# lvxianwei/DeepMerge

Measured on AMD Instinct MI355X. Metric: superpixel-pairs/sec (train step), higher is better.
Workload: dtype bf16; 1 GPU; ShfitScaleFormer_v3 depth [3, 2, 1], scales [32, 64, 128, 256] x 4ch (256x256x4 patches), 32 pairs/GPU/step, fwd+loss+bwd+allreduce+Adam (BASELINE configs[1]); pairs_per_gpu=32, global_batch=32, parallelism=dp1

## Files before the change

deepmerge_amd/_lib.py:

```python
from __future__ import annotations

import ctypes as C
import os
import re
import threading

HERE = os.path.dirname(os.path.abspath(__file__))
ROOT = os.path.dirname(HERE)
LIB_PATH = os.path.join(HERE, "libdeepmerge_hip.so")
HEADER_PATH = os.path.join(ROOT, "include", "deepmerge_hip.h")

DM_F32, DM_BF16 = 0, 1
DM_NT, DM_NN, DM_TN = 0, 1, 2
DM_BF16_PAIR = 2
DM_F64 = 3
DM_EPI_NONE, DM_EPI_GELU, DM_EPI_DGELU, DM_EPI_GELU_GRAD, DM_EPI_MUL = 0, 1, 2, 3, 4

_STATUS = {-1: "bad shape", -2: "bad dtype", -3: "bad alignment", -4: "workspace", -5: "HIP error", -6: "unsupported"}


class DeepMergeLibraryError(RuntimeError):
    pass


class DmGemmArgs(C.Structure):
    _fields_ = [
        ("layout", C.c_int32), ("ab_dtype", C.c_int32), ("c_dtype", C.c_int32), ("aux_dtype", C.c_int32),
        ("M", C.c_int32), ("N", C.c_int32), ("K", C.c_int32),
        ("epilogue", C.c_int32), ("accumulate", C.c_int32), ("split_k", C.c_int32),
        ("A", C.c_void_p), ("lda", C.c_int64),
        ("B", C.c_void_p), ("ldb", C.c_int64),
        ("C", C.c_void_p), ("ldc", C.c_int64),
        ("bias", C.c_void_p),
        ("residual", C.c_void_p), ("ldr", C.c_int64),
        ("aux", C.c_void_p), ("ldaux", C.c_int64),
        ("rows_per_group", C.c_int32), ("group_stride", C.c_int64),
        ("workspace", C.c_void_p), ("workspace_bytes", C.c_int64),
        ("colsum_a", C.c_void_p), ("colsum_accumulate", C.c_int32),
        ("k_fold", C.c_int32), ("a_fold", C.c_int64 * 3), ("b_fold", C.c_int64 * 3),
        ("c_plane", C.c_int64),
    ]


class DmReduceItem(C.Structure):
    _fields_ = [("partial", C.c_void_p), ("out0", C.c_void_p), ("out1", C.c_void_p),
                ("nrows", C.c_int32), ("width", C.c_int32), ("split", C.c_int32), ("accumulate", C.c_int32)]


class DmPairDraw(C.Structure):
    _fields_ = [("pairs", C.c_void_p), ("pair_flag", C.c_void_p), ("poly_off", C.c_void_p), ("poly_pts", C.c_void_p),
                ("pt_tile", C.c_void_p), ("pt_xy", C.c_void_p), ("pt_inner", C.c_void_p), ("pt_obj", C.c_void_p),
                ("pt_region", C.c_void_p),
                ("tile_id", C.c_void_p), ("xy", C.c_void_p), ("inner", C.c_void_p), ("obj", C.c_void_p),
                ("region", C.c_void_p), ("flag", C.c_void_p),
                ("point_id", C.c_void_p),
                ("seed", C.c_uint64),
                ("n_pairs", C.c_int32), ("n_poly", C.c_int32), ("n_poly_pts", C.c_int32), ("n_pts", C.c_int32),
                ("epoch", C.c_int32), ("batch", C.c_int32)]


class DmProfRow(C.Structure):
    _fields_ = [("name", C.c_char * 64), ("launches", C.c_int64), ("total_ms", C.c_double),
                ("total_flops", C.c_double), ("total_bytes", C.c_double)]


_P, _I, _L, _F, _D = C.c_void_p, C.c_int32, C.c_int64, C.c_float, C.c_double

SIGNATURES = {
    "dm_abi_version": (_I, []),
    "dm_last_error": (C.c_char_p, []),
    "dm_arch": (C.c_char_p, []),
    "dm_gemm": (_I, [C.POINTER(DmGemmArgs), _P]),
    "dm_gemm_workspace_bytes": (_L, [_I, _I, _I, _I]),
    "dm_gemm_grouped": (_I, [C.POINTER(DmGemmArgs), _I, _P, _L, _P]),
    "dm_gemm_grouped_workspace_bytes": (_L, [C.POINTER(DmGemmArgs), _I]),
    "dm_attention_fwd": (_I, [_P, _P, _P, _P, _I, _I, _I, _I, _F, _I, _P]),
    "dm_attention_relpos_inkernel": (_I, [_I, _I, _I, _I, _I, _I, _I, _I]),
    "dm_attention_fwd_relpos": (_I, [_P, _P, _I, _I, _I, _P, _P, _I, _I, _I, _I, _F, _I, _P]),
    "dm_attention_split_ok": (_I, [_I, _I, _I, _I, _I, _I, _I, _I]),
    "dm_attention_split_fwd": (_I, [_P, _P, _P, _P, _I, _I, _I, _P, _P, _I, _I, _I, _I, _F, _P]),
    "dm_attention_split_fwd_pair": (_I, [_P, _P, _P, _P, _I, _I, _I, _P, _P, _P, _I, _I, _I, _I, _F, _P]),
    "dm_attention_split_bwd_chunks": (_I, [_I, _I, _I]),
    "dm_attention_split_bwd": (_I, [_P, _P, _P, _I, _I, _I, _P, _P, _P, _P, _P, _P, _P, _P, _I, _I, _I, _I, _F, _P]),
    "dm_attention_split_bwd_pair": (_I, [_P, _P, _P, _I, _I, _I, _P, _P, _P, _P, _P, _P, _P, _P, _I, _I, _I, _I, _F, _P]),
    "dm_attention_bwd_relpos": (_I, [_P, _P, _I, _I, _I, _P, _P, _P, _P, _P, _P, _P, _P, _I, _I, _I, _I, _F, _I, _P]),
    "dm_attention_bwd": (_I, [_P, _P, _P, _P, _P, _P, _P, _P, _P, _I, _I, _I, _I, _F, _I, _P]),
    "dm_attention_bwd_batch_chunks": (_I, [_I, _I, _I, _I]),
    "dm_relpos_bias_gather": (_I, [_P, _P, _P, _P, _I, _I, _I, _P]),
    "dm_relpos_bias_reduce": (_I, [_P, _P, _P, _P, _I, _I, _I, _I, _I, _P]),
    "dm_layernorm_fwd": (_I, [_P, _P, _P, _P, _I, _P, _P, _I, _I, _F, _P]),
    "dm_layernorm_bwd": (_I, [_P, _I, _P, _P, _P, _P, _P, _P, _P, _P, _P, _I, _P, _I, _I, _P]),
    "dm_layernorm_bwd_partials": (_I, [_P, _I, _P, _P, _P, _P, _P, _P, _P, _P, _I, _I, C.POINTER(C.c_int32), _P]),
    "dm_layernorm_bwd_partials_pair": (_I, [_P, _I, _P, _P, _P, _P, _P, _P, _P, _P, _I, _I, C.POINTER(C.c_int32), _P]),
    "dm_partial_reduce_batch": (_I, [C.POINTER(DmReduceItem), _I, _P]),
    "dm_layernorm_bwd_partial_floats": (_L, [_I]),
    "dm_token_pool_fwd": (_I, [_P, _P, _I, _I, _I, _I, _P]),
    "dm_token_pool_bwd": (_I, [_P, _P, _I, _I, _I, _I, _P]),
    "dm_group_mean_fwd": (_I, [_P, _P, _I, _I, _I, _P]),
    "dm_group_mean_bwd": (_I, [_P, _P, _I, _I, _I, _P]),
    "dm_colsum": (_I, [_P, _I, _L, _P, _I, _I, _I, _P, _P]),
    "dm_colsum_partial_floats": (_L, [_I]),
    "dm_cast": (_I, [_P, _P, _I, _L, _P]),
    "dm_split_bf16": (_I, [_P, _L, _L, _L, _P, _I, _I, _P]),
    "dm_split_colsum_partial_floats": (_L, [_L, _L]),
    "dm_split_bf16_colsum": (_I, [_P, _L, _L, _L, _P, _I, _I, _P, _P, _P]),
    "dm_split_bf16_planes": (_I, [_P, _L, _L, _L, _P, _P, _P, _P]),
    "dm_patchify": (_I, [_P, _P, _I, _I, _I, _I, _I, _P]),
    "dm_contrastive_loss": (_I, [_P, _P, _P, _F, _F, _P, _P, _P, _I, _I, _P]),
    "dm_cross_entropy": (_I, [_P, _P, _P, _F, _P, _P, _I, _I, _P]),
    "dm_batchnorm_workspace_bytes": (_L, [_I, _I]),
    "dm_batchnorm_fwd": (_I, [_P, _P, _P, _P, _P, _P, _I, _P, _P, _P, _I, _I, _F, _F, _I, _I, _P, _P]),
    "dm_batchnorm_bwd": (_I, [_P, _P, _P, _P, _P, _I, _P, _P, _P, _P, _P, _I, _I, _I, _I, _I, _P, _P]),
    "dm_adam_step": (_I, [_P, _P, _P, _P, _P, _L, _I, _D, _D, _D, _D, _D, _P]),
    "dm_adam_hyper": (_I, [_I, _D, _D, _D, _P]),
    "dm_adam_step_dev": (_I, [_P, _P, _P, _P, _P, _L, _P, _D, _D, _D, _D, _P]),
    "dm_adam_step_dev_pair": (_I, [_P, _P, _P, _P, _P, _P, _L, _P, _D, _D, _D, _D, _P]),
    "dm_segment_mean": (_I, [_P, _P, _P, _P, _I, _I, _P]),
    "dm_edge_similarity": (_I, [_P, _P, _P, _P, _I, _I, _F, _P]),
    "dm_pairwise_distance": (_I, [_P, _P, _P, _I, _I, _I, _I, _P]),
    "dm_patch_pyramid": (_I, [_P, _I, _I, _I, _P, _P, _I, _I, _I, _I, _P, _P]),
    "dm_patch_pyramid_cols": (_I, [_P, _I, _I, _I, _P, _P, _I, _I, _I, _I, _I, _P, _I, _P]),
    "dm_pair_batch_gather": (_I, [_P, _I, _I, _I, _I, _P, _P, _P, _P, _I, _I, _I, _I, _I, _I, _P, _I, _P, _P, _P, _P]),
    "dm_pair_epoch_draw": (_I, [C.POINTER(DmPairDraw), _P]),
    "dm_contrastive_terms": (_I, [_P, _P, _P, _F, _P, _P, _I, _I, _P]),
    "dm_pair_eval_workspace_bytes": (_L, [_L, _I]),
    "dm_pair_eval_summary": (_I, [_P, _P, _P, _L, _P, _I, _P, _P, _P, _P, _P]),
    "dm_label_stats": (_I, [_P, _P, _I, _I, _I, _I, _P, _P, _P, _P, _P, _P]),
    "dm_label_features": (_I, [_P, _P, _P, _P, _P, _I, _I, _P, _P]),
    "dm_rag_edges": (_I, [_P, _I, _I, _I, _P, _P, _I, _P, _P, _I, _P, _P, _P]),
    "dm_merge_round": (_I, [_P, _P, _I, _I, _P, _P, _I, _P]),
    "dm_gru_cell_fwd": (_I, [_P, _L, _P, _P, _P, _P, _I, _I, _P]),
    "dm_gru_cell_bwd": (_I, [_P, _P, _P, _P, _P, _P, _I, _I, _P]),
    "dm_prof_enable": (_I, [_I]),
    "dm_prof_collect": (_I, [C.POINTER(DmProfRow), _I]),
}

_lock = threading.Lock()
_lib = None


def declared_symbols(header_path: str = HEADER_PATH):
    text = open(header_path).read()
    text = re.sub(r"/\*.*?\*/", "", text, flags=re.S)
    return sorted(set(re.findall(r"\b(dm_[a-z0-9_]+)\s*\(", text)))


def lib() -> C.CDLL:
    global _lib
    if _lib is not None:
        return _lib
    with _lock:
        if _lib is not None:
            return _lib
        if not os.path.exists(LIB_PATH):
            raise DeepMergeLibraryError(
                f"{LIB_PATH} not found: build the HIP kernels first "
                f"(`python -c 'import __graft_entry__ as g; g.build()'` or `make -C deepmerge_amd/csrc`). "
                f"deepmerge_amd has no CPU fallback.")
        try:
            handle = C.CDLL(LIB_PATH)
        except OSError as e:
            raise DeepMergeLibraryError(f"cannot load {LIB_PATH}: {e}") from e
        for name, (res, args) in SIGNATURES.items():
            try:
                fn = getattr(handle, name)
            except AttributeError as e:
                raise DeepMergeLibraryError(f"{LIB_PATH} does not export {name}") from e
            fn.restype = res
            fn.argtypes = args
        if handle.dm_abi_version() != 6:
            raise DeepMergeLibraryError(f"ABI version mismatch: library {handle.dm_abi_version()} != 6")
        _lib = handle
        return _lib


def check(rc: int, what: str):
    if rc == 0:
        return
    msg = lib().dm_last_error().decode("utf-8", "replace")
    text = f"{what} failed ({_STATUS.get(rc, rc)}): {msg}"
    if rc in (-1, -2, -3, -6):
        raise ValueError(text)
    raise RuntimeError(text)
```

deepmerge_amd/csrc/dm_attention.hip:

```cpp
#include "dm_common.h"
#include "dm_mfma.h"
#include "dm_attention_pipe.h"
#include "dm_attention_x3.h"
#include "dm_prof.h"

namespace {

constexpr int HD = 64;
constexpr int QB = 64;

template <typename T> struct AL {
  static constexpr int RB = HD * (int)sizeof(T);
  static constexpr int CPRW = RB / 16;
  static constexpr int KBD = RB / 64;
  static constexpr int EPC = 16 / (int)sizeof(T);
  static constexpr int TPB = (sizeof(T) == 2) ? 2 : 1;
};

template <typename T> __device__ __forceinline__ int swz(int row);
template <> __device__ __forceinline__ int swz<bf16_t>(int row) {
  const int t0 = (row >> 1) & 1, t1 = (row >> 2) & 1, t2 = (row >> 3) & 1;
  return ((t1 ^ t2) << 2) | (t0 << 1) | t1;
}
template <> __device__ __forceinline__ int swz<float>(int row) { return row & 15; }
// ... 314 lines not shown
#pragma unroll
        for (int r = 0; r < 4; ++r)
          if (key + r < N) srow[key + r] = hacc[kt][r];
      }
    }
  }
}

template <typename T, int NKT, bool FAST>
__global__ __launch_bounds__(256, 2) void attn_bwd_dkv_kernel(const AttnParams p) {
  using L = AL<T>;
  constexpr int NK = NKT * 16;
  constexpr int IMG = NK * L::RB;
  __shared__ __attribute__((aligned(16))) char smem[2 * IMG];
  char *qimg = smem, *doimg = smem + IMG;
  const int t = threadIdx.x, lane = t & 63, wave = t >> 6, g = lane >> 4, li = lane & 15;
  const int kblk = blockIdx.x, h = blockIdx.y, b = blockIdx.z;
  const int N = p.N, H = p.H;

  const long long tok_stride = 3LL * H * HD;
  const T *base = reinterpret_cast<const T *>(p.qkv) + (long long)b * N * tok_stride + (long long)h * HD;
  const long long o_stride = (long long)H * HD;
  const T *dOg = reinterpret_cast<const T *>(p.dout) + (long long)b * N * o_stride + (long long)h * HD;
  const int key = kblk * QB + wave * 16 + li;
  const bool kok = key < N;
  const T *krow = base + (long long)key * tok_stride + (long long)H * HD;
  const T *vrow = krow + (long long)H * HD;
  const float *lse = p.lse + ((long long)b * H + h) * N;
  const float *delta = p.delta + ((long long)b * H + h) * N;

  tile_to_lds<T>(qimg, base, tok_stride, N, NK, t);
  tile_to_lds<T>(doimg, dOg, o_stride, N, NK, t);
  u32x4 fk[L::KBD], fvv[L::KBD];
#pragma unroll
  for (int kb = 0; kb < L::KBD; ++kb) {
    fk[kb] = gl_frag<T>(krow, kok, kb, lane);
    fvv[kb] = gl_frag<T>(vrow, kok, kb, lane);
  }
  __syncthreads();

  constexpr int NB = NKT / L::TPB;
  u32x4 fpt[NB], fds[NB];
  const float *bsrc = FAST ? p.bias_t : p.bias;
  const float *brows = bsrc ? bsrc + (long long)h * N * N : nullptr;
  f32x4 bnext[L::TPB], lnext[L::TPB], dnext[L::TPB];
  auto fetch = [&](int m) {
#pragma unroll
    for (int u = 0; u < L::TPB; ++u) {
      const int qt = m * L::TPB + u;
      bnext[u] = bias_tile<FAST, !FAST>(brows, N, key, lane, qt);
      lnext[u] = load4_guard(lse, qt * 16 + 4 * g, N, FAST);
      dnext[u] = load4_guard(delta, qt * 16 + 4 * g, N, FAST);
    }
  };
  fetch(0);
#pragma unroll
  for (int m = 0; m < NB; ++m) {
    f32x4 bcur[L::TPB], lcur[L::TPB], dcur[L::TPB];
#pragma unroll
    for (int u = 0; u < L::TPB; ++u) { bcur[u] = bnext[u]; lcur[u] = lnext[u]; dcur[u] = dnext[u]; }
    if (m + 1 < NB) fetch(m + 1);
    f32x4 tp[L::TPB], td[L::TPB];
#pragma unroll
    for (int u = 0; u < L::TPB; ++u) {
      const int qt = m * L::TPB + u;
      const int q0 = qt * 16 + 4 * g;
      const f32x4 sc = score_tile<T>(fk, qimg, bcur[u], N, key, p.scale, lane, qt);
      f32x4 a = {0.f, 0.f, 0.f, 0.f};
#pragma unroll
      for (int kb = 0; kb < L::KBD; ++kb) mma<T>(a, fvv[kb], frag_row<T>(doimg, qt * 16 + li, kb, lane));
#pragma unroll
      for (int r = 0; r < 4; ++r) {
        const float pv = (q0 + r < N) ? fast_exp<T>(sc[r] - lcur[u][r]) : 0.f;
        tp[u][r] = pv;
        td[u][r] = pv * (a[r] - dcur[u][r]);
      }
    }
    fpt[m] = pack_tiles<T>(tp);
    fds[m] = pack_tiles<T>(td);
    asm volatile("" : "+v"(fpt[m]), "+v"(fds[m]));
    __builtin_amdgcn_sched_barrier(0);
  }
  f32x4 o[4];
  T *dk = reinterpret_cast<T *>(p.dqkv) + ((long long)b * N + key) * tok_stride + (long long)H * HD + (long long)h * HD;
  T *dvp = dk + (long long)H * HD;
#pragma unroll
  for (int dt = 0; dt < 4; ++dt) o[dt] = (f32x4){0.f, 0.f, 0.f, 0.f};
  contract_frags<T, NB>(o, fpt, doimg, lane);
  if (kok) {
#pragma unroll
    for (int dt = 0; dt < 4; ++dt) dm_store4(dvp + dt * 16 + 4 * g, o[dt]);
  }
#pragma unroll
  for (int dt = 0; dt < 4; ++dt) o[dt] = (f32x4){0.f, 0.f, 0.f, 0.f};
  contract_frags<T, NB>(o, fds, qimg, lane);
  if (kok) {
#pragma unroll
    for (int dt = 0; dt < 4; ++dt) dm_store4(dk + dt * 16 + 4 * g, o[dt] * p.scale);
  }
}

template <typename T, int NKT, bool FAST> void launch3(int which, const AttnParams &p, dim3 grid, hipStream_t s) {
  if (which == 0) hipLaunchKernelGGL((attn_fwd_kernel<T, NKT, FAST>), grid, dim3(256), 0, s, p);
  else if (which == 1) hipLaunchKernelGGL((attn_bwd_dq_kernel<T, NKT, FAST>), grid, dim3(256), 0, s, p);
  else hipLaunchKernelGGL((attn_bwd_dkv_kernel<T, NKT, FAST>), grid, dim3(256), 0, s, p);
}
template <typename T, bool FAST> void dispatch_nkt(int which, const AttnParams &p, hipStream_t s) {
  const dim3 grid((p.N + QB - 1) / QB, p.H, which == 1 ? (p.B + p.bchunk - 1) / p.bchunk : p.B);
  const int nkt = (p.N + 15) / 16;
  if (nkt <= 2) launch3<T, 2, FAST>(which, p, grid, s);
  else if (nkt <= 4) launch3<T, 4, FAST>(which, p, grid, s);
  else if (nkt <= 8) launch3<T, 8, FAST>(which, p, grid, s);
  else if (nkt <= 12) launch3<T, 12, FAST>(which, p, grid, s);
  else if (nkt <= 14) launch3<T, 14, FAST>(which, p, grid, s);
  else launch3<T, 16, FAST>(which, p, grid, s);
}
template <typename T> int dispatch(int which, const AttnParams &p, hipStream_t s) {
  const bool fast = (p.N % 4 == 0) && (which != 2 || p.bias == nullptr || p.bias_t != nullptr);
  if (fast) dispatch_nkt<T, true>(which, p, s);
  else dispatch_nkt<T, false>(which, p, s);
  return 0;
}

int check_common(const char *who, int B, int N, int H, int D, int dtype) {
  DM_REQUIRE(B > 0 && H > 0 && N > 0 && N <= 256, DM_ERR_BAD_SHAPE, "%s: need 0 < N <= 4096 tokens and head dim <= 256 (got N=%d, D=%d, B=%d, H=%d)", who, N, D, B, H);
  DM_REQUIRE(D == HD, DM_ERR_BAD_SHAPE, "%s: head dim must be in 1..256 (got %d)", who, D);
  DM_REQUIRE(dtype == DM_F32 || dtype == DM_BF16, DM_ERR_BAD_DTYPE, "%s: bad dtype %d", who, dtype);
  DM_REQUIRE(H <= 65535 && B <= 65535, DM_ERR_BAD_SHAPE, "%s: grid too large", who);
  return DM_OK;
}

}

static int batch_chunk(int B, int N, int H) {
  const int per_sample = ((N + QB - 1) / QB) * H;
  for (int c = 8; c > 1; c >>= 1)
    if ((long long)per_sample * ((B + c - 1) / c) >= 300) return c;
  return 1;
}

const AttnSwitches &attn_switches() {
  static const AttnSwitches sw = [] {
    AttnSwitches v;
    if (const char *e = getenv("DM_ATTN_PIPE")) v.pipe = atoi(e);
    if (const char *e = getenv("DM_ATTN_Q32")) v.q32 = atoi(e);
    if (const char *e = getenv("DM_ATTN_Q32_BWD")) v.q32_bwd = atoi(e);
    if (const char *e = getenv("DM_ATTN_Q32_TABKV")) v.q32_tabkv = atoi(e) != 0;
    if (const char *e = getenv("DM_ATTN_Q32_W8")) v.q32_w8 = atoi(e) != 0;
    if (const char *e = getenv("DM_ATTN_Q32_TABW")) v.q32_tabw = atoi(e);
    if (const char *e = getenv("DM_ATTN_PF")) v.pf = atoi(e) != 0;
    if (const char *e = getenv("DM_ATTN_XCD")) v.xcd = atoi(e) != 0;
    if (const char *e = getenv("DM_ATTN_X3")) v.x3 = atoi(e) != 0;
    if (const char *e = getenv("DM_ATTN_X3_W8")) v.x3_w8 = atoi(e) != 0;
    return v;
  }();
  return sw;
}

namespace {

bool tokens32(const AttnCall &c) { return c.N > 128 && c.N <= 256; }
bool cube_fits(const AttnCall &c) { return c.N == 64 * c.cube_s && (c.cube_s == 3 || c.cube_s == 4); }
bool persistent_gate(const AttnCall &c, int mode) {
  return mode != 0 && (long long)c.N * 3 * c.H * 64 * 2 < (1LL << 31) && (mode == 2 || c.B * c.H >= 96);
}

AttnPass pass32(const AttnCall &c, AttnFamily f, AttnBias bias, int waves, int rows) {
  AttnPass g{f, (c.N + 31) / 32, c.N % 32 != 0, bias, waves, 0, 0, 0};
  attn_chunks(c.B, c.N, c.H, rows, g.nblk, g.chunks, g.bchunk);
  return g;
}
bool ragged16(const AttnCall &c) { return !(c.N == 128 || c.N == 192 || c.N == 256); }
AttnPass pass_pipe16(const AttnCall &c, AttnBias bias) {
  const int nkt = (c.N + 15) / 16;
  AttnPass g{ATTN_PIPE16, ragged16(c) ? (nkt + 1) / 2 * 2 : nkt, ragged16(c), bias, 8, 0, 0, 0};
  attn_chunks(c.B, c.N, c.H, 128, g.nblk, g.chunks, g.bchunk);
  return g;
}
AttnPass pass_reg16(const AttnCall &c, int bchunk) {
  return AttnPass{ATTN_REG16, (c.N + 15) / 16, c.N % 16 != 0, c.dense ? ATTN_BIAS_DENSE : ATTN_BIAS_NONE, 4, (c.N + QB - 1) / QB, (c.B + bchunk - 1) / bchunk, bchunk};
}
int waves32(const AttnCall &c, const AttnSwitches &sw) { return (c.N + 31) / 32 <= 7 && sw.q32_w8 ? 8 : 4; }

bool split_shape(const AttnCall &c, const AttnSwitches &sw) {
  return sw.x3 && c.D == HD && tokens32(c) && c.B > 0 && c.H > 0 && persistent_gate(c, 2) && (!c.table || cube_fits(c));
}

}

AttnFwdPlan attn_plan_fwd(const AttnCall &c, const AttnSwitches &sw) {
  AttnFwdPlan pl{};
  pl.pf = sw.pf;
  pl.xcd = sw.xcd;
  if (c.split) {
    if (!split_shape(c, sw)) pl.refused = ATTN_SHAPE_NOT_TAKEN;
    else pl.pass = pass32(c, ATTN_X3, c.table ? ATTN_BIAS_TABLE : ATTN_BIAS_NONE, sw.x3_w8 ? 8 : 4, 128);
    return pl;
  }
  pl.pass = pass_reg16(c, 1);
  if (c.D != HD || c.N > 256) {
    pl.pass.family = ATTN_GENERIC;
  } else if (c.dtype == DM_BF16) {
    if (tokens32(c) && persistent_gate(c, sw.q32) && !(c.table && (c.dense || !cube_fits(c)))) {
      if (c.table) pl.pass = pass32(c, ATTN_Q32, ATTN_BIAS_TABLE, sw.q32_tabw == 4 ? 4 : 8, sw.q32_tabw == 4 ? 128 : 256);
      else if (c.dense) pl.pass = pass32(c, ATTN_Q32, ATTN_BIAS_DENSE, 4, 128);
      else pl.pass = pass32(c, ATTN_Q32, ATTN_BIAS_NONE, waves32(c, sw), 32 * waves32(c, sw));
    } else if (c.N >= 128 && persistent_gate(c, sw.pipe)) {
      pl.pass = pass_pipe16(c, c.dense ? ATTN_BIAS_DENSE : ATTN_BIAS_NONE);
    }
  }
  if (c.table && !c.dense && !(pl.pass.family == ATTN_Q32 && pl.pass.bias == ATTN_BIAS_TABLE)) pl.refused = ATTN_SHAPE_NOT_TAKEN;
  return pl;
}

AttnBwdPlan attn_plan_bwd(const AttnCall &c, const AttnSwitches &sw) {
  AttnBwdPlan pl{};
  pl.xcd = sw.xcd;
  if (c.split) {
    if (c.B > 0 && c.H > 0) {
      const AttnBias bias = c.table ? ATTN_BIAS_TABLE : ATTN_BIAS_NONE;
      pl.dq = pass32(c, ATTN_X3, bias, sw.x3_w8 ? 8 : 4, 128);
      pl.dkv = pass32(c, ATTN_X3, bias, 4, 128);
      pl.slab_chunks = pl.dkv.chunks;
    }
    if (!split_shape(c, sw)) pl.refused = ATTN_SHAPE_NOT_TAKEN;
    return pl;
  }
  pl.dq = pass_reg16(c, batch_chunk(c.B, c.N, c.H));
  pl.dkv = pass_reg16(c, 1);
  pl.slab_chunks = pl.dq.chunks;
  if (c.D != HD || c.N > 256) {
    pl.dq.family = pl.dkv.family = ATTN_GENERIC;
    return pl;
  }
  const bool table_only = c.table && !c.dense;
  if (c.dtype != DM_BF16) {
    if (table_only) pl.refused = ATTN_TABLE_NEEDS_BF16;
    return pl;
  }
  if (c.N >= 128 && persistent_gate(c, sw.pipe) && !(ragged16(c) && (c.dense || c.slab))) {
    pl.dq = pass_pipe16(c, c.dense ? ATTN_BIAS_DENSE : ATTN_BIAS_NONE);
    pl.dkv = pass_pipe16(c, c.dense || c.slab ? ATTN_BIAS_DENSE : ATTN_BIAS_NONE);
    if (tokens32(c) && persistent_gate(c, sw.q32_bwd) && !(c.table && !cube_fits(c))) {
      if (c.table) pl.dq = pass32(c, ATTN_Q32, ATTN_BIAS_TABLE, 8, 256);
      else if (c.dense) pl.dq = pass32(c, ATTN_Q32, ATTN_BIAS_DENSE, 4, 128);
      else pl.dq = pass32(c, ATTN_Q32, ATTN_BIAS_NONE, waves32(c, sw), 32 * waves32(c, sw));
      const int w = (c.N + 31) / 32 <= 7 ? 8 : 4;
      if (sw.q32_bwd != 3 && c.table && sw.q32_tabkv) pl.dkv = pass32(c, ATTN_Q32_TABKV, ATTN_BIAS_TABLE, 4, 128);
      else if (sw.q32_bwd != 3 && !c.dense && !c.slab) pl.dkv = pass32(c, ATTN_Q32, ATTN_BIAS_NONE, w, 32 * w);
    }
    pl.slab_chunks = pl.dkv.chunks;
  }
  if (table_only && pl.dkv.family != ATTN_Q32_TABKV) pl.refused = ATTN_TABLE_NOT_TAKEN;
  return pl;
}

extern "C" int32_t dm_attention_bwd_batch_chunks(int32_t B, int32_t N, int32_t H, int32_t dtype) {
  return attn_plan_bwd(AttnCall{B, N, H, HD, dtype == DM_BF16 ? DM_BF16 : DM_F32, true, false, 0, true, false}, attn_switches()).slab_chunks;
}

bool dm_attn_generic_shape(int N, int D);
int dm_attn_generic_fwd(const void *qkv, const float *bias, void *out, float *lse, int B, int N, int H, int D, float scale, int dtype, hipStream_t s);
int dm_attn_generic_bwd(const void *qkv, const float *bias, const void *out, const void *dout, const float *lse, void *dqkv, float *delta,
                        int B, int N, int H, int D, float scale, int dtype, hipStream_t s);

extern "C" int dm_attention_fwd(const void *qkv, const float *bias, void *out, float *lse, int32_t B, int32_t N, int32_t H,
                                int32_t D, float scale, int32_t dtype, void *stream) {
  if (dm_attn_generic_shape(N, D)) {
    DM_REQUIRE(B > 0 && H > 0 && H <= 65535 && B <= 65535 && (dtype == DM_F32 || dtype == DM_BF16) && qkv && out && lse, DM_ERR_BAD_SHAPE,
               "dm_attention_fwd: bad arguments (B=%d H=%d dtype=%d)", B, H, dtype);
    const int rc = dm_attn_generic_fwd(qkv, bias, out, lse, B, N, H, D, scale, dtype, reinterpret_cast<hipStream_t>(stream));
    DM_REQUIRE(rc == DM_OK, rc, "dm_attention_fwd: generic kernel could not be configured");
    DM_LAUNCH_CHECK("dm_attention_fwd(generic)");
    return DM_OK;
  }
  if (int rc = check_common("dm_attention_fwd", B, N, H, D, dtype)) return rc;
  DM_REQUIRE(qkv && out && lse, DM_ERR_BAD_SHAPE, "dm_attention_fwd: null pointer");
  DM_REQUIRE(dm_aligned16(qkv) && dm_aligned16(out) && dm_aligned16(bias), DM_ERR_BAD_ALIGN, "dm_attention_fwd: qkv/out/bias must be 16-byte aligned");
  const AttnFwdPlan pl = attn_plan_fwd(AttnCall{B, N, H, D, dtype, bias != nullptr, false, 0, false, false}, attn_switches());
  hipStream_t s = reinterpret_cast<hipStream_t>(stream);
  {
    const double esz = (dtype == DM_BF16) ? 2.0 : 4.0;
    DmProfScope prof(dtype == DM_BF16 ? "attn_fwd_bf16" : "attn_fwd_f32", s, 4.0 * B * H * (double)N * N * HD,
                     esz * 4.0 * B * H * (double)N * HD);
    const AttnPipeParams pp{qkv, bias, out, lse, B, N, H, scale};
    if (pl.pass.family == ATTN_Q32) {
      DM_REQUIRE(dm_attn_fwd_q32(pl, pp, s), DM_ERR_HIP, "dm_attention_fwd: kernel could not be configured");
    } else if (pl.pass.family == ATTN_PIPE16) {
      dm_attn_fwd_pipe(pl, pp, s);
    } else {
      AttnParams p{};
      p.qkv = qkv; p.bias = bias; p.out = out; p.lse = lse; p.B = B; p.N = N; p.H = H; p.scale = scale; p.bchunk = 1;
      if (dtype == DM_BF16) dispatch<bf16_t>(0, p, s); else dispatch<float>(0, p, s);
    }
  }
  DM_LAUNCH_CHECK("dm_attention_fwd");
  return DM_OK;
}

static AttnCall table_call(int32_t B, int32_t N, int32_t H, int32_t D, int32_t cube_s, int32_t cube_h, int32_t cube_w, int32_t dtype, bool split) {
  return AttnCall{B, N, H, D, dtype, false, true, cube_h == 8 && cube_w == 8 ? cube_s : 0, false, split};
}

extern "C" int32_t dm_attention_relpos_inkernel(int32_t B, int32_t N, int32_t H, int32_t D, int32_t cube_s, int32_t cube_h, int32_t cube_w,
                                                int32_t dtype) {
  if (B <= 0 || H <= 0) return 0;
  const AttnCall c = table_call(B, N, H, D, cube_s, cube_h, cube_w, dtype, false);
  return !attn_plan_fwd(c, attn_switches()).refused && !attn_plan_bwd(c, attn_switches()).refused ? 1 : 0;
}

extern "C" int dm_attention_fwd_relpos(const void *qkv, const float *table, int32_t cube_s, int32_t cube_h, int32_t cube_w, void *out,
                                       float *lse, int32_t B, int32_t N, int32_t H, int32_t D, float scale, int32_t dtype, void *stream) {
  DM_REQUIRE(dm_attention_relpos_inkernel(B, N, H, D, cube_s, cube_h, cube_w, dtype), DM_ERR_UNSUPPORTED,
             "dm_attention_fwd_relpos: shape not taken (B=%d N=%d H=%d D=%d cube=%dx%dx%d dtype=%d); gather the bias and call dm_attention_fwd",
             B, N, H, D, cube_s, cube_h, cube_w, dtype);
  DM_REQUIRE(qkv && table && out && lse, DM_ERR_BAD_SHAPE, "dm_attention_fwd_relpos: null pointer");
  DM_REQUIRE(dm_aligned16(qkv) && dm_aligned16(out), DM_ERR_BAD_ALIGN, "dm_attention_fwd_relpos: qkv/out must be 16-byte aligned");
  const AttnFwdPlan pl = attn_plan_fwd(table_call(B, N, H, D, cube_s, cube_h, cube_w, dtype, false), attn_switches());
  hipStream_t s = reinterpret_cast<hipStream_t>(stream);
  {
    DmProfScope prof("attn_fwd_bf16", s, 4.0 * B * H * (double)N * N * HD, 2.0 * 4.0 * B * H * (double)N * HD);
    AttnPipeParams pp{qkv, nullptr, out, lse, B, N, H, scale};
    pp.table = table;
    pp.cube_s = cube_s;
    DM_REQUIRE(dm_attn_fwd_q32(pl, pp, s), DM_ERR_UNSUPPORTED, "dm_attention_fwd_relpos: kernel could not be configured");
  }
  DM_LAUNCH_CHECK("dm_attention_fwd_relpos");
  return DM_OK;
}

static int attention_bwd(const void *qkv, const float *bias, const float *bias_t, const float *table, int32_t cube_s, const void *out,
                         const void *dout, const float *lse, void *dqkv, float *delta, float *dbias_slab, int32_t B, int32_t N, int32_t H,
                         int32_t D, float scale, int32_t dtype, void *stream) {
  if (dm_attn_generic_shape(N, D)) {
    DM_REQUIRE(B > 0 && H > 0 && H <= 65535 && B <= 65535 && (dtype == DM_F32 || dtype == DM_BF16) && qkv && out && dout && lse && dqkv && delta,
               DM_ERR_BAD_SHAPE, "dm_attention_bwd: bad arguments (B=%d H=%d dtype=%d)", B, H, dtype);
    DM_REQUIRE(dbias_slab == nullptr, DM_ERR_UNSUPPORTED, "dm_attention_bwd: the bias-table gradient needs head dim 64 and N <= 256 (got D=%d N=%d)", D, N);
    const int rc = dm_attn_generic_bwd(qkv, bias, out, dout, lse, dqkv, delta, B, N, H, D, scale, dtype, reinterpret_cast<hipStream_t>(stream));
    DM_REQUIRE(rc == DM_OK, rc, "dm_attention_bwd: generic kernel could not be configured");
    DM_LAUNCH_CHECK("dm_attention_bwd(generic)");
    return DM_OK;
  }
  if (int rc = check_common("dm_attention_bwd", B, N, H, D, dtype)) return rc;
  DM_REQUIRE(qkv && out && dout && lse && dqkv && delta, DM_ERR_BAD_SHAPE, "dm_attention_bwd: null pointer");
  DM_REQUIRE(dm_aligned16(qkv) && dm_aligned16(out) && dm_aligned16(dout) && dm_aligned16(dqkv) && dm_aligned16(bias) &&
             dm_aligned16(bias_t) && dm_aligned16(lse) && dm_aligned16(delta) && dm_aligned16(dbias_slab), DM_ERR_BAD_ALIGN,
             "dm_attention_bwd: tensors must be 16-byte aligned");
  const AttnBwdPlan pl = attn_plan_bwd(AttnCall{B, N, H, D, dtype, bias != nullptr, table != nullptr, cube_s, dbias_slab != nullptr, false}, attn_switches());
  DM_REQUIRE(pl.refused != ATTN_TABLE_NEEDS_BF16, DM_ERR_UNSUPPORTED, "dm_attention_bwd_relpos: the table-reading kernels are bf16 only");
  DM_REQUIRE(!pl.refused, DM_ERR_UNSUPPORTED,
             "dm_attention_bwd_relpos: the table-reading backward kernels do not take this call (B=%d N=%d H=%d, switches "
             "DM_ATTN_PIPE / DM_ATTN_Q32_BWD / DM_ATTN_Q32_TABKV) and no dense bias rows were given", B, N, H);
  hipStream_t s = reinterpret_cast<hipStream_t>(stream);
  {
    const double esz = (dtype == DM_BF16) ? 2.0 : 4.0;
    DmProfScope prof(dtype == DM_BF16 ? "attn_bwd_bf16" : "attn_bwd_f32", s, 10.0 * B * H * (double)N * N * HD,
                     esz * 8.0 * B * H * (double)N * HD);
    if (pl.dkv.family == ATTN_REG16) {
      AttnParams p{};
      p.qkv = qkv; p.bias = bias; p.bias_t = bias ? bias_t : nullptr; p.out = out; p.dout = dout; p.lse = const_cast<float *>(lse);
      p.delta = delta; p.dqkv = dqkv; p.slab = dbias_slab;
      p.B = B; p.N = N; p.H = H; p.scale = scale; p.bchunk = pl.dq.bchunk;
      if (dtype == DM_BF16) { dispatch<bf16_t>(1, p, s); dispatch<bf16_t>(2, p, s); }
      else { dispatch<float>(1, p, s); dispatch<float>(2, p, s); }
    } else {
      AttnPipeBwdParams pp{qkv, bias, out, dout, lse, delta, dqkv, dbias_slab, B, N, H, scale};
      pp.table = table;
      pp.cube_s = cube_s;
      DM_REQUIRE(pl.dq.family != ATTN_Q32 || dm_attn_bwd_dq_q32(pl, pp, s), DM_ERR_HIP, "dm_attention_bwd: the dQ kernel could not be configured");
      if (pl.dkv.family == ATTN_PIPE16) dm_attn_bwd_pipe(pl, pp, s);
      else DM_REQUIRE(dm_attn_bwd_dkv_q32(pl, pp, s), DM_ERR_HIP, "dm_attention_bwd: the dK / dV kernel could not be configured");
    }
  }
  DM_LAUNCH_CHECK("dm_attention_bwd");
  return DM_OK;
}

extern "C" int dm_attention_bwd(const void *qkv, const float *bias, const float *bias_t, const void *out, const void *dout,
                                const float *lse, void *dqkv, float *delta, float *dbias_slab, int32_t B, int32_t N, int32_t H, int32_t D, float scale, int32_t dtype,
                                void *stream) {
  return attention_bwd(qkv, bias, bias_t, nullptr, 0, out, dout, lse, dqkv, delta, dbias_slab, B, N, H, D, scale, dtype, stream);
}

extern "C" int dm_attention_bwd_relpos(const void *qkv, const float *table, int32_t cube_s, int32_t cube_h, int32_t cube_w, const float *bias,
                                       const float *bias_t, const void *out, const void *dout, const float *lse, void *dqkv, float *delta,
                                       float *dbias_slab, int32_t B, int32_t N, int32_t H, int32_t D, float scale, int32_t dtype, void *stream) {
  DM_REQUIRE(table, DM_ERR_BAD_SHAPE, "dm_attention_bwd_relpos: null table");
  DM_REQUIRE(bias || dm_attention_relpos_inkernel(B, N, H, D, cube_s, cube_h, cube_w, dtype), DM_ERR_UNSUPPORTED,
             "dm_attention_bwd_relpos: shape not taken (B=%d N=%d H=%d D=%d cube=%dx%dx%d dtype=%d); call dm_attention_bwd", B, N, H, D, cube_s,
             cube_h, cube_w, dtype);
  return attention_bwd(qkv, bias, bias_t, table, cube_s, out, dout, lse, dqkv, delta, dbias_slab, B, N, H, D, scale, dtype, stream);
}

static AttnCall split_call(int32_t B, int32_t N, int32_t H, int32_t D, bool has_table, int32_t cube_s, int32_t cube_h, int32_t cube_w, bool slab) {
  AttnCall c = table_call(B, N, H, D, cube_s, cube_h, cube_w, DM_F32, true);
  c.table = has_table;
  c.slab = slab;
  return c;
}

extern "C" int32_t dm_attention_split_ok(int32_t B, int32_t N, int32_t H, int32_t D, int32_t has_table, int32_t cube_s, int32_t cube_h,
                                         int32_t cube_w) {
  return attn_plan_fwd(split_call(B, N, H, D, has_table != 0, cube_s, cube_h, cube_w, false), attn_switches()).refused ? 0 : 1;
}

static int split_fwd_impl(const float *qkv, void *qkv_hi, void *qkv_lo, const float *table, int32_t cube_s, int32_t cube_h, int32_t cube_w, float *out,
                          void *out_pair, float *lse, int32_t B, int32_t N, int32_t H, int32_t D, float scale, void *stream);
extern "C" int dm_attention_split_fwd(const float *qkv, void *qkv_hi, void *qkv_lo, const float *table, int32_t cube_s, int32_t cube_h,
                                      int32_t cube_w, float *out, float *lse, int32_t B, int32_t N, int32_t H, int32_t D, float scale,
                                      void *stream) {
  return split_fwd_impl(qkv, qkv_hi, qkv_lo, table, cube_s, cube_h, cube_w, out, nullptr, lse, B, N, H, D, scale, stream);
}
extern "C" int dm_attention_split_fwd_pair(const float *qkv, void *qkv_hi, void *qkv_lo, const float *table, int32_t cube_s, int32_t cube_h,
                                           int32_t cube_w, float *out, void *out_pair, float *lse, int32_t B, int32_t N, int32_t H, int32_t D,
                                           float scale, void *stream) {
  DM_REQUIRE(out_pair && dm_aligned16(out_pair), DM_ERR_BAD_SHAPE, "dm_attention_split_fwd_pair: out_pair must be a 16-byte aligned pointer");
  return split_fwd_impl(qkv, qkv_hi, qkv_lo, table, cube_s, cube_h, cube_w, out, out_pair, lse, B, N, H, D, scale, stream);
}
static int split_fwd_impl(const float *qkv, void *qkv_hi, void *qkv_lo, const float *table, int32_t cube_s, int32_t cube_h, int32_t cube_w, float *out,
                          void *out_pair, float *lse, int32_t B, int32_t N, int32_t H, int32_t D, float scale, void *stream) {
  const AttnFwdPlan pl = attn_plan_fwd(split_call(B, N, H, D, table != nullptr, cube_s, cube_h, cube_w, false), attn_switches());
  DM_REQUIRE(!pl.refused, DM_ERR_UNSUPPORTED,
             "dm_attention_split_fwd: shape not taken (B=%d N=%d H=%d D=%d cube=%dx%dx%d); use dm_attention_fwd", B, N, H, D, cube_s, cube_h, cube_w);
  DM_REQUIRE(qkv_hi && qkv_lo && out && lse, DM_ERR_BAD_SHAPE, "dm_attention_split_fwd: null pointer");
  DM_REQUIRE(dm_aligned16(qkv) && dm_aligned16(qkv_hi) && dm_aligned16(qkv_lo) && dm_aligned16(out), DM_ERR_BAD_ALIGN,
             "dm_attention_split_fwd: tensors must be 16-byte aligned");
  hipStream_t s = reinterpret_cast<hipStream_t>(stream);
  {
    DmProfScope prof("attn_fwd_x3", s, 3.0 * 4.0 * B * H * (double)N * N * HD, 4.0 * 4.0 * B * H * (double)N * HD);
    if (qkv) dm_attn_x3_split(qkv, qkv_hi, qkv_lo, (long long)B * N * 3 * H * HD, s);
    AttnX3Params p{reinterpret_cast<const bf16_t *>(qkv_hi), reinterpret_cast<const bf16_t *>(qkv_lo), table, cube_s, out, lse, B, N, H, scale,
                   reinterpret_cast<bf16_t *>(out_pair)};
    DM_REQUIRE(dm_attn_fwd_x3(pl, p, s), DM_ERR_UNSUPPORTED, "dm_attention_split_fwd: kernel could not be configured");
  }
  DM_LAUNCH_CHECK("dm_attention_split_fwd");
  return DM_OK;
}

extern "C" int32_t dm_attention_split_bwd_chunks(int32_t B, int32_t N, int32_t H) {
  return attn_plan_bwd(split_call(B, N, H, HD, false, 0, 0, 0, false), attn_switches()).slab_chunks;
}

static int split_bwd_impl(const void *qkv_hi, const void *qkv_lo, const float *table, int32_t cube_s, int32_t cube_h, int32_t cube_w,
                          const float *out, const float *dout, void *dout_hi, void *dout_lo, const float *lse, float *dqkv, void *dqkv_pair,
                          float *delta, float *dbias_slab, int32_t B, int32_t N, int32_t H, int32_t D, float scale, void *stream);
extern "C" int dm_attention_split_bwd(const void *qkv_hi, const void *qkv_lo, const float *table, int32_t cube_s, int32_t cube_h, int32_t cube_w,
                                      const float *out, const float *dout, void *dout_hi, void *dout_lo, const float *lse, float *dqkv,
                                      float *delta, float *dbias_slab, int32_t B, int32_t N, int32_t H, int32_t D, float scale, void *stream) {
  DM_REQUIRE(dqkv, DM_ERR_BAD_SHAPE, "dm_attention_split_bwd: null pointer");
  return split_bwd_impl(qkv_hi, qkv_lo, table, cube_s, cube_h, cube_w, out, dout, dout_hi, dout_lo, lse, dqkv, nullptr, delta, dbias_slab, B, N, H, D, scale, stream);
}
extern "C" int dm_attention_split_bwd_pair(const void *qkv_hi, const void *qkv_lo, const float *table, int32_t cube_s, int32_t cube_h, int32_t cube_w,
                                           const float *out, const float *dout, void *dout_hi, void *dout_lo, const float *lse, void *dqkv_pair,
                                           float *delta, float *dbias_slab, int32_t B, int32_t N, int32_t H, int32_t D, float scale, void *stream) {
  DM_REQUIRE(dqkv_pair, DM_ERR_BAD_SHAPE, "dm_attention_split_bwd_pair: null pointer");
  return split_bwd_impl(qkv_hi, qkv_lo, table, cube_s, cube_h, cube_w, out, dout, dout_hi, dout_lo, lse, nullptr, dqkv_pair, delta, dbias_slab, B, N, H, D, scale, stream);
}
static int split_bwd_impl(const void *qkv_hi, const void *qkv_lo, const float *table, int32_t cube_s, int32_t cube_h, int32_t cube_w,
                          const float *out, const float *dout, void *dout_hi, void *dout_lo, const float *lse, float *dqkv, void *dqkv_pair,
                          float *delta, float *dbias_slab, int32_t B, int32_t N, int32_t H, int32_t D, float scale, void *stream) {
  const AttnBwdPlan pl = attn_plan_bwd(split_call(B, N, H, D, table != nullptr, cube_s, cube_h, cube_w, dbias_slab != nullptr), attn_switches());
  DM_REQUIRE(!pl.refused, DM_ERR_UNSUPPORTED,
             "dm_attention_split_bwd: shape not taken (B=%d N=%d H=%d D=%d cube=%dx%dx%d); use dm_attention_bwd", B, N, H, D, cube_s, cube_h, cube_w);
  DM_REQUIRE(qkv_hi && qkv_lo && out && dout && dout_hi && dout_lo && lse && (dqkv || dqkv_pair) && delta, DM_ERR_BAD_SHAPE, "dm_attention_split_bwd: null pointer");
  DM_REQUIRE(table || !dbias_slab, DM_ERR_BAD_SHAPE, "dm_attention_split_bwd: a bias-gradient slab needs the table");
  DM_REQUIRE(dm_aligned16(qkv_hi) && dm_aligned16(qkv_lo) && dm_aligned16(out) && dm_aligned16(dout) && dm_aligned16(dout_hi) &&
             dm_aligned16(dout_lo) && dm_aligned16(dqkv) && dm_aligned16(dqkv_pair) && dm_aligned16(dbias_slab), DM_ERR_BAD_ALIGN,
             "dm_attention_split_bwd: tensors must be 16-byte aligned");
  hipStream_t s = reinterpret_cast<hipStream_t>(stream);
  {
    DmProfScope prof("attn_bwd_x3", s, 3.0 * 10.0 * B * H * (double)N * N * HD, 4.0 * 8.0 * B * H * (double)N * HD);
    dm_attn_x3_split(dout, dout_hi, dout_lo, (long long)B * N * H * HD, s);
    AttnX3BwdParams p{reinterpret_cast<const bf16_t *>(qkv_hi), reinterpret_cast<const bf16_t *>(qkv_lo), reinterpret_cast<const bf16_t *>(dout_hi),
                      reinterpret_cast<const bf16_t *>(dout_lo), out, dout, lse, delta, dqkv, reinterpret_cast<bf16_t *>(dqkv_pair),
                      (long long)B * N * 3 * H * HD, dbias_slab, table, cube_s, B, N, H, scale};
    DM_REQUIRE(dm_attn_bwd_dq_x3(pl, p, s) && dm_attn_bwd_dkv_x3(pl, p, s), DM_ERR_UNSUPPORTED, "dm_attention_split_bwd: kernels could not be configured");
  }
  DM_LAUNCH_CHECK("dm_attention_split_bwd");
  return DM_OK;
}
```

deepmerge_amd/csrc/dm_attention_pipe.h:

```cpp
#pragma once
#include <hip/hip_runtime.h>

#include "dm_attention_plan.h"

struct AttnPipeParams {
  const void *qkv;
  const float *bias;
  void *out;
  float *lse;
  int B, N, H;
  float scale;
  const float *table = nullptr;
  int cube_s = 0;
};

void dm_attn_fwd_pipe(const AttnFwdPlan &pl, const AttnPipeParams &p, hipStream_t s);
bool dm_attn_fwd_q32(const AttnFwdPlan &pl, const AttnPipeParams &p, hipStream_t s);

struct AttnPipeBwdParams {
  const void *qkv;
  const float *bias;
  const void *out;
  const void *dout;
  const float *lse;
  float *delta;
  void *dqkv;
  float *slab;
  int B, N, H;
  float scale;
  const float *table = nullptr;
  int cube_s = 0;
};

void dm_attn_bwd_pipe(const AttnBwdPlan &pl, const AttnPipeBwdParams &p, hipStream_t s);
bool dm_attn_bwd_dq_q32(const AttnBwdPlan &pl, const AttnPipeBwdParams &p, hipStream_t s);
bool dm_attn_bwd_dkv_q32(const AttnBwdPlan &pl, const AttnPipeBwdParams &p, hipStream_t s);
```

deepmerge_amd/csrc/dm_attention_plan.h:

```cpp
#pragma once

struct AttnSwitches {
  int pipe = 1;
  int q32 = 1;
  int q32_bwd = 1;
  bool q32_tabkv = true;
  bool q32_w8 = true;
  int q32_tabw = 8;
  bool pf = true;
  bool xcd = true;
  bool x3 = true;
  bool x3_w8 = true;
};
const AttnSwitches &attn_switches();

struct AttnCall {
  int B, N, H, D, dtype;
  bool dense;
  bool table;
  int cube_s;
  bool slab;
  bool split;
};

enum AttnFamily {
  ATTN_GENERIC,
  ATTN_REG16,
  ATTN_PIPE16,
  ATTN_Q32,
  ATTN_Q32_TABKV,
  ATTN_X3,
};
enum AttnBias { ATTN_BIAS_NONE, ATTN_BIAS_DENSE, ATTN_BIAS_TABLE };
enum AttnRefusal { ATTN_TAKEN = 0, ATTN_SHAPE_NOT_TAKEN, ATTN_TABLE_NEEDS_BF16, ATTN_TABLE_NOT_TAKEN };

struct AttnPass {
  AttnFamily family;
  int nkt;
  bool ragged;
  AttnBias bias;
  int waves;
  int nblk, chunks, bchunk;
};
struct AttnFwdPlan {
  AttnRefusal refused;
  AttnPass pass;
  bool pf, xcd;
};
struct AttnBwdPlan {
  AttnRefusal refused;
  AttnPass dq, dkv;
  bool xcd;
  int slab_chunks;
};
AttnFwdPlan attn_plan_fwd(const AttnCall &c, const AttnSwitches &sw);
AttnBwdPlan attn_plan_bwd(const AttnCall &c, const AttnSwitches &sw);

inline void attn_chunks(int B, int N, int H, int rows, int &nblk, int &chunks, int &bchunk) {
  nblk = (N + rows - 1) / rows;
  chunks = 256 / (H * nblk);
  if (chunks < 1) chunks = 1;
  if (chunks > B) chunks = B;
  bchunk = (B + chunks - 1) / chunks;
  chunks = (B + bchunk - 1) / bchunk;
}
```

deepmerge_amd/csrc/dm_attention_q32_bwd.hip:

```cpp
#include "dm_attention_q32.h"

#ifndef DMQ_ABL
#define DMQ_ABL 0
#endif

namespace dmq32 {

__device__ __forceinline__ void qk_first_acc(f32x16 &d, const u32x4 &k, const u32x4 &q, const f32x16 &c) {
  asm volatile(DMQ_MFMA " %0, %1, %2, %3" : "=&a"(d) : "v"(k), "a"(q), "a"(c));
}
__device__ __forceinline__ void qk_acc_acc(f32x16 &d, const u32x4 &k, const u32x4 &q) {
  asm volatile(DMQ_MFMA " %0, %1, %2, %0" : "+a"(d) : "v"(k), "a"(q));
}
__device__ __forceinline__ void park_acc16(f32x16 &v) { asm volatile("" : "+a"(v)); }
__device__ __forceinline__ float dot2(unsigned a, unsigned b, float c) {
  return __builtin_amdgcn_fdot2_f32_bf16(__builtin_bit_cast(bf16x2, a), __builtin_bit_cast(bf16x2, b), c, false);
}

template <int NKT, bool RAGGED, int BM, int NW>
__global__ __launch_bounds__(64 * NW, NW / 4) void attn_bwd_dq_q32_kernel(const AttnPipeBwdParams p, int bchunk, int nblk, int chunks) {
  constexpr bool BIAS = BM == 1, TAB = BM == 2;
  constexpr bool DIRECT = TAB && NW == 8;
  constexpr bool RUNS = NW == 8;
  static_assert(!TAB || (!RAGGED && NKT % 2 == 0 && NW == 8), "table form: N = 64 x scales, 8 waves");
// ... 761 lines not shown
      };
      auto read_bias = [&](int jt, f32x16 &d) {
#pragma unroll
        for (int c = 0; c < 4; ++c)
#pragma unroll
          for (int e = 0; e < 4; ++e) d[4 * c + e] = tabl[TAB_PITCH * (15 * (jt >> 1) + 4 * (jt & 1) + c) + e];
      };
      auto read_stat = [&](int jt, int which, f32x16 &d) {
#pragma unroll
        for (int c = 0; c < 4; ++c) {
          const f32x4 a = *reinterpret_cast<const f32x4 *>(stat + (which * NP + 32 * jt + 8 * c + 4 * hh) * 4);
#pragma unroll
          for (int e = 0; e < 4; ++e) d[4 * c + e] = a[e];
        }
      };
      auto s_piece = [&](int ks, f32x16 &d) { qk_acc<true, false>(d, qf[ks], kfr[ks]); };
      auto dp_piece = [&](int ks, f32x16 &d) { qk_acc<true, false>(d, df[ks], vfr[ks]); };
      auto tfrag = [&](const u32x2 (&f)[8], int sx, int dt) { return (u32x4){f[4 * sx + 2 * dt][0], f[4 * sx + 2 * dt][1], f[4 * sx + 2 * dt + 1][0], f[4 * sx + 2 * dt + 1][1]}; };
      auto dv_piece = [&](int jt, int g, const u32x4 (&pb)[2]) {
        const int sx = g >> 1, dt = g & 1;
        f32x16 &o = dt ? dv1 : dv0;
        if (jt == 0 && sx == 0) pv_first<false>(o, tfrag(dtf, 0, dt), pb[0]); else pv_acc<false>(o, tfrag(dtf, sx, dt), pb[sx]);
      };
      auto dk_piece = [&](int jt, int g, const u32x4 (&dsb)[2]) {
        const int sx = g >> 1, dt = g & 1;
        f32x16 &o = dt ? dk1 : dk0;
        if (jt == 0 && sx == 0) pv_first<false>(o, tfrag(qt, 0, dt), dsb[0]); else pv_acc<false>(o, tfrag(qt, sx, dt), dsb[sx]);
      };
      float fa[8][2], ex[8][2];
      auto stage_a = [&](const f32x16 &sc, int k) {
        fa[k][0] = __builtin_fmaf(sc[2 * k], scale2, nl[2 * k]);
        fa[k][1] = __builtin_fmaf(sc[2 * k + 1], scale2, nl[2 * k + 1]);
        asm volatile("" :: "v"(fa[k][0]), "v"(fa[k][1]));
      };
      auto stage_b = [&](int k) {
        ex[k][0] = __builtin_amdgcn_exp2f(fa[k][0]);
        ex[k][1] = __builtin_amdgcn_exp2f(fa[k][1]);
        asm volatile("" :: "v"(ex[k][0]), "v"(ex[k][1]));
      };
      auto stage_c = [&](const f32x16 &dp, int k, u32x4 (&pb)[2], u32x4 (&dsb)[2]) {
        const unsigned wp = pk_bf16(ex[k][0], ex[k][1]);
        const unsigned wd = pk_bf16(ex[k][0] * dp[2 * k], ex[k][1] * dp[2 * k + 1]);
        pb[k >> 2][k & 3] = wp;
        dsb[k >> 2][k & 3] = wd;
        asm volatile("" :: "v"(wp), "v"(wd));
      };

      read_a(0);
      read_bias(0, s0);
      read_stat(0, 1, dp0);
      read_stat(0, 0, nl);
      asm volatile("s_nop 1");
#pragma unroll
      for (int ks = 0; ks < 4; ++ks) s_piece(ks, s0);
#pragma unroll
      for (int ks = 0; ks < 4; ++ks) dp_piece(ks, dp0);
      asm volatile("" :: "v"(qf[0]), "v"(qf[1]), "v"(qf[2]), "v"(qf[3]), "v"(df[0]), "v"(df[1]), "v"(df[2]), "v"(df[3]));
      if (NKT > 1) { read_a(1); read_bias(1, s1); read_stat(1, 1, dp1); }
      asm volatile("s_nop 15\n\ts_nop 7" : "+v"(s0), "+v"(dp0));
#pragma unroll
      for (int j = 0; j < NKT; ++j) {
        f32x16 &sc = (j & 1) ? s1 : s0;
        f32x16 &sn = (j & 1) ? s0 : s1;
        f32x16 &dpc = (j & 1) ? dp1 : dp0;
        f32x16 &dpn = (j & 1) ? dp0 : dp1;
        u32x4 (&pbc)[2] = (j & 1) ? pb1 : pb0;
        u32x4 (&pbp)[2] = (j & 1) ? pb0 : pb1;
        u32x4 (&dsc)[2] = (j & 1) ? dsb1 : dsb0;
        u32x4 (&dsp)[2] = (j & 1) ? dsb0 : dsb1;
        asm volatile("" : "+v"(sc), "+v"(dpc));
        if (j > 0) read_t(j - 1);
        __builtin_amdgcn_sched_barrier(0);
#pragma unroll
        for (int g = 0; g < 18; ++g) {
          if (g < 4) {
            if (j + 1 < NKT) s_piece(g, sn);
          } else if (g < 8) {
            if (j + 1 < NKT) dp_piece(g - 4, dpn);
          } else if (g < 12) {
            if (j > 0) dv_piece(j - 1, g - 8, pbp);
          } else if (g < 16) {
            if (j > 0) dk_piece(j - 1, g - 12, dsp);
          } else {
            if (j > 0) pv_acc<false>(hacc[j > 0 ? j - 1 : 0], esel[g - 16], dsp[g - 16]);
          }
          __builtin_amdgcn_sched_barrier(0);
          if (g < 8) stage_a(sc, g);
          if (g >= 1 && g < 9) stage_b(g - 1);
          if (g >= 2 && g < 10) stage_c(dpc, g - 2, pbc, dsc);
          if (g == 8 && j + 2 < NKT) { read_a(j + 2); read_bias(j + 2, sc); }
          if (g == 10 && j + 2 < NKT) read_stat(j + 2, 1, dpc);
          if (g == 10 && j + 1 < NKT) read_stat(j + 1, 0, nl);
          if (g == 13 && more) {
            if (j < NKT - 1) stage_piece(rq_next, rd_next, buf ^ 1, j);
            if (j == 0) stage_piece(rq_next, rd_next, buf ^ 1, NKT - 1);
          }
          if (g == 14 && more && j == NKT - 1) load_rows(b + 1, kld, vld, lse_ld, dl_ld);
          if (g < 4) {
            if (j + 1 < NKT) asm volatile("" :: "v"(qf[g]));
          } else if (g < 8) {
            if (j + 1 < NKT) asm volatile("" :: "v"(df[g - 4]));
          } else if (g < 12) {
            if (j > 0) asm volatile("" :: "v"(dtf[2 * (g - 8)]), "v"(dtf[2 * (g - 8) + 1]), "v"(pbp[(g - 8) >> 1]));
          } else if (g < 16) {
            if (j > 0) asm volatile("" :: "v"(qt[2 * (g - 12)]), "v"(qt[2 * (g - 12) + 1]), "v"(dsp[(g - 12) >> 1]));
          } else {
            if (j > 0) asm volatile("" :: "v"(esel[g - 16]), "v"(dsp[g - 16]));
          }
          __builtin_amdgcn_sched_barrier(0);
        }
      }
      read_t(NKT - 1);
      {
        u32x4 (&pbl)[2] = ((NKT - 1) & 1) ? pb1 : pb0;
        u32x4 (&dsl)[2] = ((NKT - 1) & 1) ? dsb1 : dsb0;
        asm volatile("s_nop 1");
#pragma unroll
        for (int g = 0; g < 4; ++g) dv_piece(NKT - 1, g, pbl);
#pragma unroll
        for (int g = 0; g < 4; ++g) dk_piece(NKT - 1, g, dsl);
        pv_acc<false>(hacc[NKT - 1], esel[0], dsl[0]);
        pv_acc<false>(hacc[NKT - 1], esel[1], dsl[1]);
        asm volatile("s_nop 15\n\ts_nop 7" : "+a"(dk0), "+a"(dk1), "+a"(dv0), "+a"(dv1)
                     : "v"(pbl[0]), "v"(pbl[1]), "v"(dsl[0]), "v"(dsl[1]), "v"(esel[0]), "v"(esel[1]),
                       "v"(qt[0]), "v"(qt[1]), "v"(qt[2]), "v"(qt[3]), "v"(qt[4]), "v"(qt[5]), "v"(qt[6]), "v"(qt[7]),
                       "v"(dtf[0]), "v"(dtf[1]), "v"(dtf[2]), "v"(dtf[3]), "v"(dtf[4]), "v"(dtf[5]), "v"(dtf[6]), "v"(dtf[7]));
      }
      const int rr = lane >> 3, cc = lane & 7;
#pragma unroll
      for (int which = 0; which < 2; ++which) {
        const f32x16 &a0 = which ? dv0 : dk0;
        const f32x16 &a1 = which ? dv1 : dk1;
        const float f = which ? 1.f : p.scale;
#pragma unroll
        for (int c = 0; c < 4; ++c) {
          const u32x2 w0 = {pk_bf16(a0[4 * c] * f, a0[4 * c + 1] * f), pk_bf16(a0[4 * c + 2] * f, a0[4 * c + 3] * f)};
          const u32x2 w1 = {pk_bf16(a1[4 * c] * f, a1[4 * c + 1] * f), pk_bf16(a1[4 * c + 2] * f, a1[4 * c + 3] * f)};
          *reinterpret_cast<u32x2 *>(wb + r * WB_PITCH + (8 * c + 4 * hh) * 2) = w0;
          *reinterpret_cast<u32x2 *>(wb + r * WB_PITCH + (32 + 8 * c + 4 * hh) * 2) = w1;
        }
        bf16_t *drow0 = reinterpret_cast<bf16_t *>(p.dqkv) + ((long long)b * N + k_wave) * tok_stride + (long long)((1 + which) * H + h) * HD;
#pragma unroll
        for (int k = 0; k < 4; ++k) {
          const u32x4 v = *reinterpret_cast<const u32x4 *>(wb + (rr + 8 * k) * WB_PITCH + cc * 16);
          *reinterpret_cast<u32x4 *>(drow0 + (long long)(rr + 8 * k) * tok_stride + cc * 8) = v;
        }
      }
    } else if (more) {
#pragma unroll
      for (int j = 0; j < NKT; ++j) stage_piece(rq_next, rd_next, buf ^ 1, j);
      load_rows(b + 1, kld, vld, lse_ld, dl_ld);
    }
  }
  if (wave_live && p.slab) {
    float *sl = p.slab + ((long long)(chunk * H + h) * N) * N + key;
#pragma unroll
    for (int j = 0; j < NKT; ++j) {
      asm volatile("s_nop 15\n\ts_nop 7" : "+a"(hacc[j]));
#pragma unroll
      for (int i = 0; i < 16; ++i) sl[(long long)(32 * j + 8 * (i >> 2) + 4 * hh + (i & 3)) * N] = hacc[j][i];
    }
  }
}

template <int NKT, bool RAGGED, int BM, int NW> bool launch_dq(const AttnPass &g, const AttnPipeBwdParams &p, hipStream_t s) {
  constexpr int LDS = 4 * NKT * 32 * 128 + (BM == 2 ? 0 : NW * WB_WAVE) + (BM == 2 ? (NKT - 1) * 15 * TAB_PITCH * 4 : 0);
  static_assert(LDS <= 160 * 1024, "LDS budget");
  static const bool ok = hipFuncSetAttribute(reinterpret_cast<const void *>(attn_bwd_dq_q32_kernel<NKT, RAGGED, BM, NW>),
                                             hipFuncAttributeMaxDynamicSharedMemorySize, LDS) == hipSuccess;
  if (!ok) return false;
  const int wgs = NW == 8 ? (p.B * p.H < 256 ? p.B * p.H : 256) : grid_size(g.nblk, p.H, g.chunks);
  hipLaunchKernelGGL((attn_bwd_dq_q32_kernel<NKT, RAGGED, BM, NW>), dim3(wgs), dim3(64 * NW), LDS, s, p, g.bchunk, g.nblk, g.chunks);
  return true;
}

template <int NKT> bool launch_dq_n(const AttnPass &g, const AttnPipeBwdParams &p, hipStream_t s) {
  if constexpr (NKT % 2 == 0) {
    if (g.bias == ATTN_BIAS_TABLE) return launch_dq<NKT, false, 2, 8>(g, p, s);
  }
  if (g.bias == ATTN_BIAS_DENSE) return g.ragged ? launch_dq<NKT, true, 1, 4>(g, p, s) : launch_dq<NKT, false, 1, 4>(g, p, s);
  if constexpr (NKT <= 7) {
    if (g.waves == 8) return g.ragged ? launch_dq<NKT, true, 0, 8>(g, p, s) : launch_dq<NKT, false, 0, 8>(g, p, s);
  }
  return g.ragged ? launch_dq<NKT, true, 0, 4>(g, p, s) : launch_dq<NKT, false, 0, 4>(g, p, s);
}

template <int NKT, bool RAGGED, int NW> bool launch_dkv(const AttnPass &g, const AttnPipeBwdParams &p, hipStream_t s) {
  constexpr int LDS = 4 * NKT * 32 * 128 + 2 * (2 * NKT * 32 * 4) + NW * WB_WAVE;
  static_assert(LDS <= 160 * 1024, "LDS budget");
  static const bool ok = hipFuncSetAttribute(reinterpret_cast<const void *>(attn_bwd_dkv_q32_kernel<NKT, RAGGED, NW>),
                                             hipFuncAttributeMaxDynamicSharedMemorySize, LDS) == hipSuccess;
  if (!ok) return false;
  hipLaunchKernelGGL((attn_bwd_dkv_q32_kernel<NKT, RAGGED, NW>), dim3(grid_size(g.nblk, p.H, g.chunks)), dim3(64 * NW), LDS, s, p, g.bchunk, g.nblk, g.chunks);
  return true;
}

template <int NKT> bool launch_dkv_tab(const AttnPass &g, const AttnPipeBwdParams &p, hipStream_t s) {
  constexpr int LDS = 4 * NKT * 32 * 128 + 2 * (2 * NKT * 32 * 4) + 4 * WB_WAVE + (NKT - 1) * 15 * TAB_PITCH * 4;
  static_assert(LDS <= 160 * 1024, "LDS budget");
  static const bool ok = hipFuncSetAttribute(reinterpret_cast<const void *>(attn_bwd_dkv_tab_kernel<NKT>),
                                             hipFuncAttributeMaxDynamicSharedMemorySize, LDS) == hipSuccess;
  if (!ok) return false;
  hipLaunchKernelGGL((attn_bwd_dkv_tab_kernel<NKT>), dim3(grid_size(g.nblk, p.H, g.chunks)), dim3(256), LDS, s, p, g.bchunk, g.nblk, g.chunks);
  return true;
}

template <int NKT> bool launch_dkv_n(const AttnPass &g, const AttnPipeBwdParams &p, hipStream_t s) {
  if constexpr (NKT <= 7) return g.ragged ? launch_dkv<NKT, true, 8>(g, p, s) : launch_dkv<NKT, false, 8>(g, p, s);
  else return g.ragged ? launch_dkv<NKT, true, 4>(g, p, s) : launch_dkv<NKT, false, 4>(g, p, s);
}

}

bool dm_attn_bwd_dkv_q32(const AttnBwdPlan &pl, const AttnPipeBwdParams &p, hipStream_t s) {
  if (pl.dkv.family == ATTN_Q32_TABKV) return pl.dkv.nkt == 6 ? dmq32::launch_dkv_tab<6>(pl.dkv, p, s) : dmq32::launch_dkv_tab<8>(pl.dkv, p, s);
  return dmq32::with_tiles32(pl.dkv.nkt, [&](auto nkt) { return dmq32::launch_dkv_n<nkt.value>(pl.dkv, p, s); });
}

bool dm_attn_bwd_dq_q32(const AttnBwdPlan &pl, const AttnPipeBwdParams &p, hipStream_t s) {
  return dmq32::with_tiles32(pl.dq.nkt, [&](auto nkt) { return dmq32::launch_dq_n<nkt.value>(pl.dq, p, s); });
}
```

deepmerge_amd/csrc/dm_rows.hip:

```cpp
#include <cstdlib>

#include "dm_common.h"

int dm_layernorm_wide_fwd(const float *x, const float *gamma, const float *beta, void *y, int y_dtype, float *mean, float *rstd, int rows,
                          int cols, float eps, hipStream_t s);
int dm_layernorm_wide_bwd(const void *dy, int dy_dtype, const float *x, const float *gamma, const float *mean, const float *rstd,
                          const float *dres, float *dx, void *dx_lp, float *partial, int max_slices, int *slices, int rows, int cols,
                          hipStream_t s);
int dm_patchify_any(const float *x, void *cols, int dtype, int B, int C, int side, int p, hipStream_t s);

namespace {

constexpr int MAXCH = 4;
constexpr int LN_WIDE_MAX = 8192;
static int ln_max_wg() {
  static const int v = [] { const char *e = getenv("DM_LN_WG"); return e ? atoi(e) : 768; }();
  return v;
}
constexpr int CS_MAX_SLICES = 64;

template <typename TY, bool PAIR = false>
__global__ __launch_bounds__(256) void layernorm_fwd_kernel(const float *__restrict__ x, const float *__restrict__ gamma,
                                                            const float *__restrict__ beta, TY *__restrict__ y,
                                                            float *__restrict__ mean_out, float *__restrict__ rstd_out,
// ... 31 lines not shown
    TY *yr = y + (long long)row * cols;
#pragma unroll
    for (int i = 0; i < MAXCH; ++i) {
      const int c = lane + 64 * i;
      if (c < nch) {
        const f32x4 g = dm_load4(gamma + 4 * c), b = dm_load4(beta + 4 * c);
        f32x4 o;
#pragma unroll
        for (int e = 0; e < 4; ++e) o[e] = (v[i][e] - mean) * rstd * g[e] + b[e];
        if constexpr (PAIR) {
          bf16x4 h, l;
#pragma unroll
          for (int e = 0; e < 4; ++e) {
            h[e] = (bf16_t)o[e];
            l[e] = (bf16_t)(o[e] - (float)h[e]);
          }
          *reinterpret_cast<bf16x4 *>(yr + 4 * c) = h;
          *reinterpret_cast<bf16x4 *>(yr + (long long)rows * cols + 4 * c) = l;
        } else {
          dm_store4(yr + 4 * c, o);
        }
      }
    }
  }
}

template <typename TDY, int CH>
__global__ __launch_bounds__(256) void layernorm_bwd_kernel(const TDY *__restrict__ dy, const float *__restrict__ x,
                                                            const float *__restrict__ gamma, const float *__restrict__ mean,
                                                            const float *__restrict__ rstd, const float *__restrict__ dres,
                                                            float *__restrict__ dx, bf16_t *__restrict__ dx_lp,
                                                            float *__restrict__ partial, int rows, int cols, long long lp_plane) {
  __shared__ float red[4][2][CH * 256];
  const int lane = threadIdx.x & 63, wave = threadIdx.x >> 6;
  const int nch = cols >> 2;
  f32x4 dg[CH], db[CH], gam[CH];
#pragma unroll
  for (int i = 0; i < CH; ++i) {
    dg[i] = db[i] = (f32x4){0.f, 0.f, 0.f, 0.f};
    const int c = lane + 64 * i;
    gam[i] = (c < nch) ? dm_load4(gamma + 4 * c) : (f32x4){0.f, 0.f, 0.f, 0.f};
  }
  for (int row = blockIdx.x * 4 + wave; row < rows; row += gridDim.x * 4) {
    const long long off = (long long)row * cols;
    const float mu = mean[row], rs = rstd[row];
    f32x4 xh[CH], g[CH], dr[CH];
    float s1 = 0.f, s2 = 0.f;
#pragma unroll
    for (int i = 0; i < CH; ++i) {
      const int c = lane + 64 * i;
      dr[i] = (dres && c < nch) ? dm_load4(dres + off + 4 * c) : (f32x4){0.f, 0.f, 0.f, 0.f};
    }
#pragma unroll
    for (int i = 0; i < CH; ++i) {
      const int c = lane + 64 * i;
      if (c < nch) {
        const f32x4 xv = dm_load4(x + off + 4 * c);
        const f32x4 d = dm_load4(dy + off + 4 * c);
#pragma unroll
        for (int e = 0; e < 4; ++e) {
          xh[i][e] = (xv[e] - mu) * rs;
          g[i][e] = d[e] * gam[i][e];
          s1 += g[i][e];
          s2 += g[i][e] * xh[i][e];
          dg[i][e] += d[e] * xh[i][e];
          db[i][e] += d[e];
        }
      } else {
        xh[i] = g[i] = (f32x4){0.f, 0.f, 0.f, 0.f};
      }
    }
    const float c1 = dm_wave_sum(s1) / (float)cols, c2 = dm_wave_sum(s2) / (float)cols;
#pragma unroll
    for (int i = 0; i < CH; ++i) {
      const int c = lane + 64 * i;
      if (c < nch) {
        f32x4 o;
#pragma unroll
        for (int e = 0; e < 4; ++e) o[e] = rs * (g[i][e] - c1 - xh[i][e] * c2);
        if (dres) o += dr[i];
        dm_store4(dx + off + 4 * c, o);
        if (dx_lp) {
          if (lp_plane > 0) {
            bf16x4 h, l;
#pragma unroll
            for (int e = 0; e < 4; ++e) {
              h[e] = (bf16_t)o[e];
              l[e] = (bf16_t)(o[e] - (float)h[e]);
            }
            *reinterpret_cast<bf16x4 *>(dx_lp + off + 4 * c) = h;
            *reinterpret_cast<bf16x4 *>(dx_lp + lp_plane + off + 4 * c) = l;
          } else {
            dm_store4(dx_lp + off + 4 * c, o);
          }
        }
      }
    }
  }
#pragma unroll
  for (int i = 0; i < CH; ++i) {
#pragma unroll
    for (int e = 0; e < 4; ++e) {
      red[wave][0][(lane + 64 * i) * 4 + e] = dg[i][e];
      red[wave][1][(lane + 64 * i) * 4 + e] = db[i][e];
    }
  }
  __syncthreads();
  float *prow = partial + (long long)blockIdx.x * 2 * cols;
  for (int c = threadIdx.x; c < 2 * cols; c += 256) {
    const int which = c / cols, col = c % cols;
    prow[c] = (red[0][which][col] + red[1][which][col]) + (red[2][which][col] + red[3][which][col]);
  }
}

__global__ __launch_bounds__(256) void partial_reduce_kernel(const float *__restrict__ partial, float *__restrict__ out0,
                                                             float *__restrict__ out1, int nrows, int width, int split,
                                                             int accumulate) {
  __shared__ float red[16][17];
  const int tx = threadIdx.x & 15, ty = threadIdx.x >> 4;
  const int j = blockIdx.x * 16 + tx;
  float s = 0.f;
  if (j < width) {
    float s0 = 0.f, s1 = 0.f, s2 = 0.f, s3 = 0.f;
    int r = ty;
    for (; r + 48 < nrows; r += 64) {
      s0 += partial[(long long)r * width + j];
      s1 += partial[(long long)(r + 16) * width + j];
      s2 += partial[(long long)(r + 32) * width + j];
      s3 += partial[(long long)(r + 48) * width + j];
    }
    for (; r < nrows; r += 16) s0 += partial[(long long)r * width + j];
    s = (s0 + s1) + (s2 + s3);
  }
  red[ty][tx] = s;
  __syncthreads();
  if (ty == 0 && j < width) {
    float t[16];
#pragma unroll
    for (int k = 0; k < 16; ++k) t[k] = red[k][tx];
#pragma unroll
    for (int w = 8; w > 0; w >>= 1)
#pragma unroll
      for (int k = 0; k < w; ++k) t[k] = t[2 * k] + t[2 * k + 1];
    s = t[0];
    float *o = (j < split) ? out0 + j : out1 + (j - split);
    *o = accumulate ? *o + s : s;
  }
}

struct ReduceBatch {
  DmReduceItem it[32];
  int start[33];
  int n;
};
__global__ __launch_bounds__(256) void partial_reduce_batch_kernel(const ReduceBatch rb) {
  __shared__ float red[16][17];
  int job = 0;
  while (job + 1 < rb.n && (int)blockIdx.x >= rb.start[job + 1]) ++job;
  const DmReduceItem &it = rb.it[job];
  const float *__restrict__ partial = it.partial;
  const int nrows = it.nrows, width = it.width;
  const int tx = threadIdx.x & 15, ty = threadIdx.x >> 4;
  const int j = ((int)blockIdx.x - rb.start[job]) * 16 + tx;
  float s = 0.f;
  if (j < width) {
    float s0 = 0.f, s1 = 0.f, s2 = 0.f, s3 = 0.f;
    int r = ty;
    for (; r + 48 < nrows; r += 64) {
      s0 += partial[(long long)r * width + j];
      s1 += partial[(long long)(r + 16) * width + j];
      s2 += partial[(long long)(r + 32) * width + j];
      s3 += partial[(long long)(r + 48) * width + j];
    }
    for (; r < nrows; r += 16) s0 += partial[(long long)r * width + j];
    s = (s0 + s1) + (s2 + s3);
  }
  red[ty][tx] = s;
  __syncthreads();
  if (ty == 0 && j < width) {
    float t[16];
#pragma unroll
    for (int k = 0; k < 16; ++k) t[k] = red[k][tx];
#pragma unroll
    for (int w = 8; w > 0; w >>= 1)
#pragma unroll
      for (int k = 0; k < w; ++k) t[k] = t[2 * k] + t[2 * k + 1];
    s = t[0];
    float *o = (j < it.split) ? it.out0 + j : it.out1 + (j - it.split);
    *o = it.accumulate ? *o + s : s;
  }
}

__global__ void token_pool_fwd_kernel(const float *__restrict__ x, float *__restrict__ y, int B, int S, int side, int C) {
  const int half = side >> 1, c4 = C >> 2;
  const long long total = (long long)B * S * half * half * c4;
  for (long long i = (long long)blockIdx.x * blockDim.x + threadIdx.x; i < total; i += (long long)gridDim.x * blockDim.x) {
    const int c = (int)(i % c4);
    long long r = i / c4;
    const int px = (int)(r % half); r /= half;
    const int py = (int)(r % half); r /= half;
    const float *src = x + ((r * side + 2 * py) * side + 2 * px) * (long long)C + 4 * c;
    const f32x4 a = dm_load4(src), b = dm_load4(src + C), d = dm_load4(src + (long long)side * C), e = dm_load4(src + (long long)side * C + C);
    dm_store4(y + ((r * half + py) * half + px) * (long long)C + 4 * c, ((a + b) + (d + e)) * 0.25f);
  }
}
__global__ void token_pool_bwd_kernel(const float *__restrict__ dy, float *__restrict__ dx, int B, int S, int side, int C) {
  const int half = side >> 1, c4 = C >> 2;
  const long long total = (long long)B * S * side * side * c4;
  for (long long i = (long long)blockIdx.x * blockDim.x + threadIdx.x; i < total; i += (long long)gridDim.x * blockDim.x) {
    const int c = (int)(i % c4);
    long long r = i / c4;
    const int xx = (int)(r % side); r /= side;
    const int yy = (int)(r % side); r /= side;
    const f32x4 g = dm_load4(dy + ((r * half + (yy >> 1)) * half + (xx >> 1)) * (long long)C + 4 * c);
    dm_store4(dx + ((r * side + yy) * side + xx) * (long long)C + 4 * c, g * 0.25f);
  }
}
__global__ void group_mean_fwd_kernel(const float *__restrict__ x, float *__restrict__ y, int rows, int g, int C) {
  const int c4 = C >> 2;
  const long long total = (long long)rows * c4;
  const float inv = 1.0f / (float)g;
  for (long long i = (long long)blockIdx.x * blockDim.x + threadIdx.x; i < total; i += (long long)gridDim.x * blockDim.x) {
    const int c = (int)(i % c4);
    const long long r = i / c4;
    f32x4 s = {0.f, 0.f, 0.f, 0.f};
    for (int k = 0; k < g; ++k) s += dm_load4(x + (r * g + k) * C + 4 * c);
    dm_store4(y + r * C + 4 * c, s * inv);
  }
}
__global__ void group_mean_bwd_kernel(const float *__restrict__ dy, float *__restrict__ dx, int rows, int g, int C) {
  const int c4 = C >> 2;
  const long long total = (long long)rows * g * c4;
  const float inv = 1.0f / (float)g;
  for (long long i = (long long)blockIdx.x * blockDim.x + threadIdx.x; i < total; i += (long long)gridDim.x * blockDim.x) {
    const int c = (int)(i % c4);
    const long long r = i / c4;
    dm_store4(dx + r * C + 4 * c, dm_load4(dy + (r / g) * C + 4 * c) * inv);
  }
}

template <typename T>
__global__ __launch_bounds__(256) void colsum_kernel(const T *__restrict__ X, long long ldx, float *__restrict__ partial,
                                                     int M, int N, int rows_per_slice, int direct) {
  __shared__ f32x4 red[16][16];
  const int tx = threadIdx.x & 15, ty = threadIdx.x >> 4;
  const int n = blockIdx.x * 64 + tx * 4;
  const int r0 = blockIdx.y * rows_per_slice, r1 = min(M, r0 + rows_per_slice);
  f32x4 s = {0.f, 0.f, 0.f, 0.f};
  if (n < N)
    for (int r = r0 + ty; r < r1; r += 16) s += dm_load4(X + (long long)r * ldx + n);
  red[ty][tx] = s;
  __syncthreads();
  if (ty == 0 && n < N) {
    f32x4 a = red[0][tx];
#pragma unroll
    for (int k = 1; k < 16; ++k) a += red[k][tx];
    if (direct == 1) a = dm_load4(partial + n) + a;
    dm_store4(partial + (long long)blockIdx.y * N + n, a);
  }
}

template <typename T>
__global__ __launch_bounds__(256) void colsum_generic_kernel(const T *__restrict__ X, long long ldx, float *__restrict__ partial,
                                                             int M, int N, int rows_per_slice) {
  const int n = blockIdx.x * 256 + threadIdx.x;
  if (n >= N) return;
  const int r0 = blockIdx.y * rows_per_slice, r1 = min(M, r0 + rows_per_slice);
  float s = 0.f;
  for (int r = r0; r < r1; ++r) s += (float)X[(long long)r * ldx + n];
  partial[(long long)blockIdx.y * N + n] = s;
}

__global__ void cast_bf16_kernel(const float *__restrict__ src, bf16_t *__restrict__ dst, long long n) {
  const long long n8 = n >> 3;
  for (long long i = (long long)blockIdx.x * blockDim.x + threadIdx.x; i < n8; i += (long long)gridDim.x * blockDim.x) {
    const f32x4 a = dm_load4(src + 8 * i), b = dm_load4(src + 8 * i + 4);
    bf16x8 o = {(bf16_t)a[0], (bf16_t)a[1], (bf16_t)a[2], (bf16_t)a[3], (bf16_t)b[0], (bf16_t)b[1], (bf16_t)b[2], (bf16_t)b[3]};
    *reinterpret_cast<bf16x8 *>(dst + 8 * i) = o;
  }
  if (blockIdx.x == 0 && threadIdx.x < (n & 7)) dst[(n8 << 3) + threadIdx.x] = (bf16_t)src[(n8 << 3) + threadIdx.x];
}
__global__ void split_bf16_kernel(const float *__restrict__ src, long long ld, long long rows, long long cols, bf16_t *__restrict__ dst,
                                  int stack, int pattern) {
  const long long c4 = cols >> 2, total = rows * c4;
  const long long piece = stack ? rows * cols : cols, ldd = stack ? cols : 3 * cols;
  for (long long i = (long long)blockIdx.x * blockDim.x + threadIdx.x; i < total; i += (long long)gridDim.x * blockDim.x) {
    const long long r = i / c4, c = (i - r * c4) << 2;
    const f32x4 x = dm_load4(src + r * ld + c);
    bf16x4 hi, lo;
#pragma unroll
    for (int j = 0; j < 4; ++j) {
      hi[j] = (bf16_t)x[j];
      lo[j] = (bf16_t)(x[j] - (float)hi[j]);
    }
    bf16_t *d = dst + r * ldd + c;
#pragma unroll
    for (int j = 0; j < 3; ++j) *reinterpret_cast<bf16x4 *>(d + j * piece) = ((pattern >> j) & 1) ? lo : hi;
  }
}
template <bool CS>
__global__ __launch_bounds__(256) void split_bf16_rows_kernel(const float *__restrict__ src, long long ld, int rows, int cols,
                                                              bf16_t *__restrict__ dst, int stack, int pattern, float *__restrict__ partial, int pieces) {
  __shared__ float red[CS ? 8 : 1][CS ? 264 : 1];
  const int c = (blockIdx.x * 32 + threadIdx.x) * 8;
  const bool live = c < cols;
  if (!CS && !live) return;
  const long long piece = stack ? (long long)rows * cols : cols, ldd = stack ? cols : 3LL * cols;
  float cs[8] = {0.f, 0.f, 0.f, 0.f, 0.f, 0.f, 0.f, 0.f};
  for (int r = blockIdx.y * 8 + threadIdx.y; live && r < rows; r += gridDim.y * 8) {
// ... 164 lines not shown
    const long long i = (n4 << 2) + threadIdx.x;
    const float g = grad[i] * grad_scale;
    const float mm = m[i] * beta1 + g * omb1;
    const float vv = v[i] * beta2 + (g * g) * omb2;
    const float p = param[i] - step_size * (mm / (sqrtf(vv) / bc2_sqrt + eps));
    param[i] = p; m[i] = mm; v[i] = vv;
    if (lp) lp[i] = (bf16_t)p;
    if (lo) lo[i] = (bf16_t)(p - (float)(bf16_t)p);
  }
}

__global__ void relpos_gather_kernel(const float *__restrict__ table, const int *__restrict__ index,
                                     float *__restrict__ bias, float *__restrict__ bias_t, int N, int H, int n_bins) {
  const int NN = N * N;
  for (int ij = blockIdx.x * blockDim.x + threadIdx.x; ij < NN; ij += gridDim.x * blockDim.x) {
    int bin = index[ij];
    bin = min(max(bin, 0), n_bins - 1);
    for (int h = 0; h < H; ++h) bias[(long long)h * NN + ij] = table[bin * H + h];
    if (bias_t) {
      const int i = ij / N, j = ij % N;
      int bt = index[j * N + i];
      bt = min(max(bt, 0), n_bins - 1);
      for (int h = 0; h < H; ++h) bias_t[(long long)h * NN + ij] = table[bt * H + h];
    }
  }
}
__global__ void chunk_sum_kernel(float *__restrict__ slab, long long plane4, int chunks) {
  for (long long i = (long long)blockIdx.x * blockDim.x + threadIdx.x; i < plane4; i += (long long)gridDim.x * blockDim.x) {
    f32x4 v = dm_load4(slab + 4 * i);
    for (int c = 1; c < chunks; ++c) v += dm_load4(slab + ((long long)c * plane4 + i) * 4);
    dm_store4(slab + 4 * i, v);
  }
}

__global__ __launch_bounds__(256) void relpos_reduce_kernel(const float *__restrict__ slab, const int *__restrict__ pos,
                                                            const int *__restrict__ off, float *__restrict__ dtable, int chunks,
                                                            int H, int N, int n_bins, int accumulate) {
  const int lane = threadIdx.x & 63, wave = threadIdx.x >> 6;
  const int bin = blockIdx.x, h = blockIdx.y * 4 + wave;
  if (h >= H) return;
  const int beg = off[bin], cnt = off[bin + 1] - beg;
  const long long plane = (long long)N * N;
  float acc = 0.f;
  for (int c = 0; c < chunks; ++c) {
    const float *pl = slab + ((long long)c * H + h) * plane;
#pragma unroll 4
    for (int j = lane; j < cnt; j += 64) acc += pl[pos[beg + j]];
  }
  acc = dm_wave_sum(acc);
  if (lane == 0) {
    float *o = dtable + (long long)bin * H + h;
    *o = accumulate ? *o + acc : acc;
  }
}

inline int grid_for(long long work_items, int block = 256, int cap = 4096) {
  long long g = (work_items + block - 1) / block;
  if (g < 1) g = 1;
  if (g > cap) g = cap;
  return (int)g;
}

static int adam_grid(long long n) {
  static const int cap = [] { const char *e = getenv("DM_ADAM_GRID"); return e ? atoi(e) : 16384; }();
  return grid_for(n / 4 + 1, 256, cap);
}

}

extern "C" int dm_layernorm_fwd(const float *x, const float *gamma, const float *beta, void *y, int32_t y_dtype,
                                float *mean, float *rstd, int32_t rows, int32_t cols, float eps, void *stream) {
  DM_REQUIRE(rows > 0 && cols > 0 && cols % 4 == 0 && cols <= LN_WIDE_MAX, DM_ERR_BAD_SHAPE,
             "dm_layernorm_fwd: rows=%d cols=%d (cols must be a multiple of 4, <= %d)", rows, cols, LN_WIDE_MAX);
  DM_REQUIRE(x && gamma && beta && y && mean && rstd, DM_ERR_BAD_SHAPE, "dm_layernorm_fwd: null pointer");
  hipStream_t s = reinterpret_cast<hipStream_t>(stream);
  if (cols > MAXCH * 256) {
    DM_REQUIRE(y_dtype != DM_BF16_PAIR, DM_ERR_UNSUPPORTED, "dm_layernorm_fwd: a plane-pair result needs cols <= %d", MAXCH * 256);
    const int rc = dm_layernorm_wide_fwd(x, gamma, beta, y, y_dtype, mean, rstd, rows, cols, eps, s);
    DM_REQUIRE(rc == DM_OK, rc, "dm_layernorm_fwd: bad y_dtype %d", y_dtype);
    DM_LAUNCH_CHECK("dm_layernorm_fwd(wide)");
    return DM_OK;
  }
  const int grid = grid_for((long long)rows, 4, 2048);
  if (y_dtype == DM_F32)
    hipLaunchKernelGGL(layernorm_fwd_kernel<float>, dim3(grid), dim3(256), 0, s, x, gamma, beta, (float *)y, mean, rstd, rows, cols, eps);
  else if (y_dtype == DM_BF16)
    hipLaunchKernelGGL(layernorm_fwd_kernel<bf16_t>, dim3(grid), dim3(256), 0, s, x, gamma, beta, (bf16_t *)y, mean, rstd, rows, cols, eps);
  else if (y_dtype == DM_BF16_PAIR)
    hipLaunchKernelGGL((layernorm_fwd_kernel<bf16_t, true>), dim3(grid), dim3(256), 0, s, x, gamma, beta, (bf16_t *)y, mean, rstd, rows, cols, eps);
  else DM_REQUIRE(false, DM_ERR_BAD_DTYPE, "dm_layernorm_fwd: bad y_dtype %d", y_dtype);
  DM_LAUNCH_CHECK("dm_layernorm_fwd");
  return DM_OK;
}

extern "C" int64_t dm_layernorm_bwd_partial_floats(int32_t cols) { return (int64_t)ln_max_wg() * 2 * cols; }

static int ln_bwd_main(const void *dy, int32_t dy_dtype, const float *x, const float *gamma, const float *mean, const float *rstd,
                       const float *dres, float *dx, void *dx_lp, float *partial, int32_t rows, int32_t cols, int32_t *n_partial, hipStream_t s,
                       const char *who, bool lp_pair = false) {
  const long long lp_plane = lp_pair ? (long long)rows * cols : 0;
  DM_REQUIRE(!lp_pair || (dx_lp && cols <= MAXCH * 256), DM_ERR_UNSUPPORTED, "%s: the plane-pair copy needs dx_lp and cols <= %d", who, MAXCH * 256);
  DM_REQUIRE(rows > 0 && cols > 0 && cols % 4 == 0 && cols <= LN_WIDE_MAX, DM_ERR_BAD_SHAPE, "%s: rows=%d cols=%d", who, rows, cols);
  DM_REQUIRE(dy && x && gamma && mean && rstd && dx && partial && n_partial, DM_ERR_BAD_SHAPE, "%s: null pointer", who);
  if (cols > MAXCH * 256) {
    int slices = 0;
    const int rc = dm_layernorm_wide_bwd(dy, dy_dtype, x, gamma, mean, rstd, dres, dx, dx_lp, partial, ln_max_wg(), &slices, rows, cols, s);
    DM_REQUIRE(rc == DM_OK, rc, "%s: bad dy_dtype %d", who, dy_dtype);
    DM_LAUNCH_CHECK("dm_layernorm_bwd(wide)");
    *n_partial = slices;
    return DM_OK;
  }
  const int grid = grid_for((long long)rows, 4, ln_max_wg());
  DM_REQUIRE(dy_dtype == DM_F32 || dy_dtype == DM_BF16, DM_ERR_BAD_DTYPE, "%s: bad dy_dtype %d", who, dy_dtype);
  const bool narrow = cols <= 768;
  if (dy_dtype == DM_F32 && narrow)
    hipLaunchKernelGGL((layernorm_bwd_kernel<float, 3>), dim3(grid), dim3(256), 0, s, (const float *)dy, x, gamma, mean, rstd, dres, dx, (bf16_t *)dx_lp, partial, rows, cols, lp_plane);
  else if (dy_dtype == DM_F32)
    hipLaunchKernelGGL((layernorm_bwd_kernel<float, MAXCH>), dim3(grid), dim3(256), 0, s, (const float *)dy, x, gamma, mean, rstd, dres, dx, (bf16_t *)dx_lp, partial, rows, cols, lp_plane);
  else if (narrow)
    hipLaunchKernelGGL((layernorm_bwd_kernel<bf16_t, 3>), dim3(grid), dim3(256), 0, s, (const bf16_t *)dy, x, gamma, mean, rstd, dres, dx, (bf16_t *)dx_lp, partial, rows, cols, lp_plane);
  else
    hipLaunchKernelGGL((layernorm_bwd_kernel<bf16_t, MAXCH>), dim3(grid), dim3(256), 0, s, (const bf16_t *)dy, x, gamma, mean, rstd, dres, dx, (bf16_t *)dx_lp, partial, rows, cols, lp_plane);
  DM_LAUNCH_CHECK("dm_layernorm_bwd");
  *n_partial = grid;
  return DM_OK;
}

extern "C" int dm_layernorm_bwd(const void *dy, int32_t dy_dtype, const float *x, const float *gamma, const float *mean,
                                const float *rstd, const float *dres, float *dx, void *dx_lp, float *dgamma, float *dbeta,
                                int32_t accumulate_params, float *partial, int32_t rows, int32_t cols, void *stream) {
  DM_REQUIRE(dgamma && dbeta, DM_ERR_BAD_SHAPE, "dm_layernorm_bwd: null pointer");
  hipStream_t s = reinterpret_cast<hipStream_t>(stream);
  int32_t slices = 0;
  if (const int rc = ln_bwd_main(dy, dy_dtype, x, gamma, mean, rstd, dres, dx, dx_lp, partial, rows, cols, &slices, s, "dm_layernorm_bwd")) return rc;
  hipLaunchKernelGGL(partial_reduce_kernel, dim3((2 * cols + 15) / 16), dim3(256), 0, s, partial, dgamma, dbeta, slices, 2 * cols, cols, accumulate_params);
  DM_LAUNCH_CHECK("dm_layernorm_bwd(reduce)");
  return DM_OK;
}

extern "C" int dm_layernorm_bwd_partials(const void *dy, int32_t dy_dtype, const float *x, const float *gamma, const float *mean,
                                         const float *rstd, const float *dres, float *dx, void *dx_lp, float *partial, int32_t rows,
                                         int32_t cols, int32_t *n_partial, void *stream) {
  return ln_bwd_main(dy, dy_dtype, x, gamma, mean, rstd, dres, dx, dx_lp, partial, rows, cols, n_partial, reinterpret_cast<hipStream_t>(stream),
                     "dm_layernorm_bwd_partials");
}

extern "C" int dm_layernorm_bwd_partials_pair(const void *dy, int32_t dy_dtype, const float *x, const float *gamma, const float *mean,
                                              const float *rstd, const float *dres, float *dx, void *dx_pair, float *partial, int32_t rows,
                                              int32_t cols, int32_t *n_partial, void *stream) {
  return ln_bwd_main(dy, dy_dtype, x, gamma, mean, rstd, dres, dx, dx_pair, partial, rows, cols, n_partial, reinterpret_cast<hipStream_t>(stream),
                     "dm_layernorm_bwd_partials_pair", true);
}

extern "C" int dm_partial_reduce_batch(const DmReduceItem *items, int32_t n, void *stream) {
  DM_REQUIRE(items && n > 0, DM_ERR_BAD_SHAPE, "dm_partial_reduce_batch: no items");
  hipStream_t s = reinterpret_cast<hipStream_t>(stream);
  for (int32_t base = 0; base < n; base += 32) {
    ReduceBatch rb;
    rb.n = (n - base < 32) ? n - base : 32;
    int total = 0;
    for (int i = 0; i < rb.n; ++i) {
      const DmReduceItem &it = items[base + i];
      DM_REQUIRE(it.partial && it.out0 && it.out1 && it.nrows > 0 && it.width > 0 && it.split >= 0 && it.split <= it.width, DM_ERR_BAD_SHAPE,
                 "dm_partial_reduce_batch: item %d: nrows=%d width=%d split=%d", base + i, it.nrows, it.width, it.split);
      rb.it[i] = it;
      rb.start[i] = total;
      total += (it.width + 15) / 16;
    }
    for (int i = rb.n; i <= 32; ++i) rb.start[i] = total;
    hipLaunchKernelGGL(partial_reduce_batch_kernel, dim3(total), dim3(256), 0, s, rb);
    DM_LAUNCH_CHECK("dm_partial_reduce_batch");
  }
  return DM_OK;
}

extern "C" int dm_token_pool_fwd(const float *x, float *y, int32_t B, int32_t S, int32_t side, int32_t C, void *stream) {
  DM_REQUIRE(B > 0 && S > 0 && side >= 2 && side % 2 == 0 && C % 4 == 0, DM_ERR_BAD_SHAPE, "dm_token_pool_fwd: B=%d S=%d side=%d C=%d", B, S, side, C);
  const long long total = (long long)B * S * (side / 2) * (side / 2) * (C / 4);
  hipLaunchKernelGGL(token_pool_fwd_kernel, dim3(grid_for(total)), dim3(256), 0, reinterpret_cast<hipStream_t>(stream), x, y, B, S, side, C);
  DM_LAUNCH_CHECK("dm_token_pool_fwd");
  return DM_OK;
}
extern "C" int dm_token_pool_bwd(const float *dy, float *dx, int32_t B, int32_t S, int32_t side, int32_t C, void *stream) {
  DM_REQUIRE(B > 0 && S > 0 && side >= 2 && side % 2 == 0 && C % 4 == 0, DM_ERR_BAD_SHAPE, "dm_token_pool_bwd: B=%d S=%d side=%d C=%d", B, S, side, C);
  const long long total = (long long)B * S * side * side * (C / 4);
  hipLaunchKernelGGL(token_pool_bwd_kernel, dim3(grid_for(total)), dim3(256), 0, reinterpret_cast<hipStream_t>(stream), dy, dx, B, S, side, C);
  DM_LAUNCH_CHECK("dm_token_pool_bwd");
  return DM_OK;
}
extern "C" int dm_group_mean_fwd(const float *x, float *y, int32_t rows, int32_t g, int32_t C, void *stream) {
  DM_REQUIRE(rows > 0 && g > 0 && C % 4 == 0, DM_ERR_BAD_SHAPE, "dm_group_mean_fwd: rows=%d g=%d C=%d", rows, g, C);
  hipLaunchKernelGGL(group_mean_fwd_kernel, dim3(grid_for((long long)rows * (C / 4))), dim3(256), 0, reinterpret_cast<hipStream_t>(stream), x, y, rows, g, C);
  DM_LAUNCH_CHECK("dm_group_mean_fwd");
  return DM_OK;
}
extern "C" int dm_group_mean_bwd(const float *dy, float *dx, int32_t rows, int32_t g, int32_t C, void *stream) {
  DM_REQUIRE(rows > 0 && g > 0 && C % 4 == 0, DM_ERR_BAD_SHAPE, "dm_group_mean_bwd: rows=%d g=%d C=%d", rows, g, C);
  hipLaunchKernelGGL(group_mean_bwd_kernel, dim3(grid_for((long long)rows * g * (C / 4))), dim3(256), 0, reinterpret_cast<hipStream_t>(stream), dy, dx, rows, g, C);
  DM_LAUNCH_CHECK("dm_group_mean_bwd");
  return DM_OK;
}

extern "C" int64_t dm_colsum_partial_floats(int32_t N) { return (int64_t)CS_MAX_SLICES * N; }

extern "C" int dm_colsum(const void *X, int32_t dtype, int64_t ldx, float *out, int32_t M, int32_t N, int32_t accumulate,
                         float *partial, void *stream) {
  DM_REQUIRE(M > 0 && N > 0 && ldx >= N, DM_ERR_BAD_SHAPE, "dm_colsum: M=%d N=%d ldx=%lld", M, N, (long long)ldx);
  const bool vec = (N % 4 == 0) && (ldx % 4 == 0) && dm_aligned16(X);
  DM_REQUIRE(X && out && partial, DM_ERR_BAD_SHAPE, "dm_colsum: null pointer");
  hipStream_t s = reinterpret_cast<hipStream_t>(stream);
  int slices = (M + 255) / 256;
  if (slices > CS_MAX_SLICES) slices = CS_MAX_SLICES;
  const int rps = (M + slices - 1) / slices;
  slices = (M + rps - 1) / rps;
  dim3 grid((N + 63) / 64, slices), ggrid((N + 255) / 256, slices);
  const bool direct = slices == 1 && vec && dm_aligned16(out);
  float *dst = direct ? out : partial;
  const int dflag = direct ? (accumulate ? 1 : 0) : -1;
  if (dtype == DM_F32) {
    if (vec) hipLaunchKernelGGL(colsum_kernel<float>, grid, dim3(256), 0, s, (const float *)X, (long long)ldx, dst, M, N, rps, dflag);
    else hipLaunchKernelGGL(colsum_generic_kernel<float>, ggrid, dim3(256), 0, s, (const float *)X, (long long)ldx, partial, M, N, rps);
  } else if (dtype == DM_BF16) {
    if (vec) hipLaunchKernelGGL(colsum_kernel<bf16_t>, grid, dim3(256), 0, s, (const bf16_t *)X, (long long)ldx, dst, M, N, rps, dflag);
    else hipLaunchKernelGGL(colsum_generic_kernel<bf16_t>, ggrid, dim3(256), 0, s, (const bf16_t *)X, (long long)ldx, partial, M, N, rps);
  } else DM_REQUIRE(false, DM_ERR_BAD_DTYPE, "dm_colsum: bad dtype %d", dtype);
  DM_LAUNCH_CHECK("dm_colsum");
  if (direct) return DM_OK;
  hipLaunchKernelGGL(partial_reduce_kernel, dim3((N + 15) / 16), dim3(256), 0, s, partial, out, out, slices, N, N, accumulate);
  DM_LAUNCH_CHECK("dm_colsum(reduce)");
  return DM_OK;
}

extern "C" int dm_cast(const float *src, void *dst, int32_t dst_dtype, int64_t n, void *stream) {
  DM_REQUIRE(src && dst && n > 0, DM_ERR_BAD_SHAPE, "dm_cast: bad arguments");
  hipStream_t s = reinterpret_cast<hipStream_t>(stream);
  if (dst_dtype == DM_BF16) hipLaunchKernelGGL(cast_bf16_kernel, dim3(grid_for(n / 8 + 1)), dim3(256), 0, s, src, (bf16_t *)dst, (long long)n);
  else if (dst_dtype == DM_F32) hipLaunchKernelGGL(copy_f32_kernel, dim3(grid_for(n / 4 + 1)), dim3(256), 0, s, src, (float *)dst, (long long)n);
  else DM_REQUIRE(false, DM_ERR_BAD_DTYPE, "dm_cast: bad dtype %d", dst_dtype);
  DM_LAUNCH_CHECK("dm_cast");
  return DM_OK;
}

static bool split_rows_ok(const float *src, int64_t ld, int64_t rows, int64_t cols, const void *dst, int32_t stack) {
  return cols % 8 == 0 && rows < (1LL << 31) && cols < (1LL << 31) && dm_aligned16(src) && dm_aligned16(dst) && ld % 4 == 0 &&
         (stack ? (rows * cols) % 8 == 0 : true);
}
static void split_rows_grid(int64_t rows, int64_t cols, int &gx, int &gy, bool colsum = false) {
  gx = (int)((cols / 8 + 31) / 32);
  long long y = (rows + 7) / 8;
  const int blocks = colsum ? 2048 : 8192;
  const long long cap = blocks / gx > 0 ? blocks / gx : 1;
  gy = (int)(y > cap ? cap : y);
}

extern "C" int64_t dm_split_colsum_partial_floats(int64_t rows, int64_t cols) {
  if (rows <= 0 || cols <= 0 || cols % 8) return 0;
  int gx, gy;
  split_rows_grid(rows, cols, gx, gy, true);
  return (int64_t)gy * cols;
}

extern "C" int dm_split_bf16_colsum(const float *src, int64_t ld, int64_t rows, int64_t cols, void *dst, int32_t stack, int32_t pattern,
                                    float *partial, int32_t *n_partial, void *stream) {
  DM_REQUIRE(src && dst && partial && n_partial && rows > 0 && cols > 0 && ld >= cols && pattern >= 0 && pattern < 8, DM_ERR_BAD_SHAPE,
             "dm_split_bf16_colsum: bad arguments (rows=%lld cols=%lld ld=%lld)", (long long)rows, (long long)cols, (long long)ld);
  DM_REQUIRE(split_rows_ok(src, ld, rows, cols, dst, stack), DM_ERR_UNSUPPORTED,
             "dm_split_bf16_colsum: needs cols %% 8 == 0, ld %% 4 == 0 and 16-byte aligned tensors (cols=%lld ld=%lld)", (long long)cols, (long long)ld);
  int gx, gy;
  split_rows_grid(rows, cols, gx, gy, true);
  hipLaunchKernelGGL(split_bf16_rows_kernel<true>, dim3(gx, (unsigned)gy), dim3(32, 8), 0, reinterpret_cast<hipStream_t>(stream), src, (long long)ld,
                     (int)rows, (int)cols, (bf16_t *)dst, stack ? 1 : 0, pattern, partial, 3);
  DM_LAUNCH_CHECK("dm_split_bf16_colsum");
  *n_partial = gy;
  return DM_OK;
}

extern "C" int dm_split_bf16_planes(const float *src, int64_t ld, int64_t rows, int64_t cols, void *dst, float *partial, int32_t *n_partial,
                                    void *stream) {
  DM_REQUIRE(src && dst && rows > 0 && cols > 0 && ld >= cols && ((partial == nullptr) == (n_partial == nullptr)), DM_ERR_BAD_SHAPE,
             "dm_split_bf16_planes: bad arguments (rows=%lld cols=%lld ld=%lld)", (long long)rows, (long long)cols, (long long)ld);
  DM_REQUIRE(split_rows_ok(src, ld, rows, cols, dst, 1), DM_ERR_UNSUPPORTED,
             "dm_split_bf16_planes: needs cols %% 8 == 0, ld %% 4 == 0 and 16-byte aligned tensors (cols=%lld ld=%lld)", (long long)cols, (long long)ld);
  int gx, gy;
  split_rows_grid(rows, cols, gx, gy, partial != nullptr);
  hipStream_t s = reinterpret_cast<hipStream_t>(stream);
  if (partial)
    hipLaunchKernelGGL(split_bf16_rows_kernel<true>, dim3(gx, (unsigned)gy), dim3(32, 8), 0, s, src, (long long)ld, (int)rows, (int)cols, (bf16_t *)dst, 1, 0b10, partial, 2);
  else
    hipLaunchKernelGGL(split_bf16_rows_kernel<false>, dim3(gx, (unsigned)gy), dim3(32, 8), 0, s, src, (long long)ld, (int)rows, (int)cols, (bf16_t *)dst, 1, 0b10,
                       (float *)nullptr, 2);
  DM_LAUNCH_CHECK("dm_split_bf16_planes");
  if (n_partial) *n_partial = gy;
  return DM_OK;
}

extern "C" int dm_split_bf16(const float *src, int64_t ld, int64_t rows, int64_t cols, void *dst, int32_t stack, int32_t pattern,
                             void *stream) {
  DM_REQUIRE(src && dst && rows > 0 && cols > 0 && cols % 4 == 0 && ld >= cols && ld % 4 == 0, DM_ERR_BAD_SHAPE,
             "dm_split_bf16: rows=%lld cols=%lld ld=%lld (cols and ld must be multiples of 4)", (long long)rows, (long long)cols, (long long)ld);
  DM_REQUIRE(pattern >= 0 && pattern < 8, DM_ERR_BAD_SHAPE, "dm_split_bf16: pattern %d", pattern);
  hipStream_t s = reinterpret_cast<hipStream_t>(stream);
  if (split_rows_ok(src, ld, rows, cols, dst, stack)) {
    int gx, gy;
    split_rows_grid(rows, cols, gx, gy);
    hipLaunchKernelGGL(split_bf16_rows_kernel<false>, dim3(gx, (unsigned)gy), dim3(32, 8), 0, s, src, (long long)ld, (int)rows, (int)cols,
                       (bf16_t *)dst, stack ? 1 : 0, pattern, (float *)nullptr, 3);
  } else {
    hipLaunchKernelGGL(split_bf16_kernel, dim3(grid_for(rows * (cols / 4))), dim3(256), 0, s, src, (long long)ld, (long long)rows,
                       (long long)cols, (bf16_t *)dst, stack ? 1 : 0, pattern);
  }
  DM_LAUNCH_CHECK("dm_split_bf16");
  return DM_OK;
}

extern "C" int dm_patchify(const float *x, void *cols, int32_t dtype, int32_t B, int32_t C, int32_t side, int32_t p, void *stream) {
  DM_REQUIRE(B > 0 && C > 0 && p > 0 && side % p == 0, DM_ERR_BAD_SHAPE,
             "dm_patchify: B=%d C=%d side=%d patch=%d (patch must divide side)", B, C, side, p);
  hipStream_t s = reinterpret_cast<hipStream_t>(stream);
  if (p % 4 != 0) {
    const int rc = dm_patchify_any(x, cols, dtype, B, C, side, p, s);
    DM_REQUIRE(rc == DM_OK, rc, "dm_patchify: bad dtype %d", dtype);
    DM_LAUNCH_CHECK("dm_patchify(any)");
    return DM_OK;
  }
  const long long total = (long long)B * (side / p) * (side / p) * ((long long)C * p * p / 4);
  if (dtype == DM_F32) hipLaunchKernelGGL(patchify_kernel<float>, dim3(grid_for(total)), dim3(256), 0, s, x, (float *)cols, B, C, side, p);
// ... 95 lines not shown
```

deepmerge_amd/ops.py:

```python
from __future__ import annotations

import os

import ctypes as C
from typing import Optional

import torch

from . import _lib
from ._lib import DM_BF16, DM_EPI_DGELU, DM_EPI_GELU, DM_EPI_GELU_GRAD, DM_EPI_MUL, DM_EPI_NONE, DM_F32, DM_NN, DM_NT, DM_TN, DmGemmArgs, check

_NUMERICS = "bf16"


NUMERICS_MODES = ("bf16", "fp32", "bf16x3")
_FP32_PRODUCTS = "mfma_f32"
_SPLIT_MIN_WORK = 1 << 24
_PAIR_LN_MAX_COLS = 1024


def set_numerics(mode: str) -> None:
    global _NUMERICS
    _NUMERICS = check_numerics(mode)

# ... 187 lines not shown
    if A.dtype != B.dtype:
        raise ValueError(f"A/B dtype mismatch: {A.dtype} vs {B.dtype}")
    if lda is None:
        lda = A.stride(-2) if A.dim() >= 2 else K
    if ldb is None:
        ldb = B.stride(-2) if B.dim() >= 2 else K
    if (_FP32_PRODUCTS == "bf16x3" and A.dtype == torch.float32 and M * N * K >= _SPLIT_MIN_WORK
            and M % 8 == 0 and N % 8 == 0 and K % 8 == 0 and lda % 4 == 0 and ldb % 4 == 0):
        a_rows, a_cols = (M, K) if layout != DM_TN else (K, M)
        b_rows, b_cols = (N, K) if layout == DM_NT else (K, N)
        a_stack, b_stack = int(layout == DM_TN), int(layout != DM_NT)
        A3 = workspace(6 * a_rows * a_cols, A.device, ws_slot + ".split_a").view(torch.bfloat16)
        B3 = workspace(6 * b_rows * b_cols, A.device, ws_slot + ".split_b").view(torch.bfloat16)
        fused_ok = colsum_out is not None and a_cols % 8 == 0 and A.data_ptr() % 16 == 0 and (a_rows * a_cols) % 8 == 0
        n_part = _lib.lib().dm_split_colsum_partial_floats(a_rows, a_cols) if fused_ok else 0
        if n_part > 0:
            part = workspace(4 * n_part, A.device, ws_slot + ".partial").view(torch.float32)
            rows_out = C.c_int32(0)
            check(_lib.lib().dm_split_bf16_colsum(A.data_ptr(), lda, a_rows, a_cols, A3.data_ptr(), a_stack, 0b100, part.data_ptr(),
                                                  C.byref(rows_out), _stream()), "dm_split_bf16_colsum")
            item = (_lib.DmReduceItem * 1)()
            item[0].partial, item[0].out0, item[0].out1 = part.data_ptr(), colsum_out.data_ptr(), colsum_out.data_ptr()
            item[0].nrows, item[0].width, item[0].split, item[0].accumulate = rows_out.value, a_cols, a_cols, int(bool(colsum_accumulate))
            check(_lib.lib().dm_partial_reduce_batch(item, 1, _stream()), "dm_partial_reduce_batch")
        else:
            check(_lib.lib().dm_split_bf16(A.data_ptr(), lda, a_rows, a_cols, A3.data_ptr(), a_stack, 0b100, _stream()), "dm_split_bf16")
            if colsum_out is not None:
                colsum(torch.as_strided(A, (a_rows, a_cols), (lda, 1)), colsum_out, accumulate=colsum_accumulate, ws_slot=ws_slot + ".partial")
        check(_lib.lib().dm_split_bf16(B.data_ptr(), ldb, b_rows, b_cols, B3.data_ptr(), b_stack, 0b010, _stream()), "dm_split_bf16")
        return gemm(layout, A3, B3, C_out, M, N, 3 * K, lda=(a_cols if a_stack else 3 * a_cols), ldb=(b_cols if b_stack else 3 * b_cols),
                    ldc=ldc, bias=bias, residual=residual, ldr=ldr, epilogue=epilogue, aux=aux, ldaux=ldaux, accumulate=accumulate,
                    split_k=split_k, rows_per_group=rows_per_group, group_stride=group_stride, ws_slot=ws_slot)
    a = _gemm_args(layout, A, B, C_out, M, N, K, lda, ldb, ldc, bias, residual, ldr, epilogue, aux, ldaux, accumulate, split_k,
                   rows_per_group, group_stride, colsum_out, colsum_accumulate, ws_slot, c_pair, fold)
    check(_lib.lib().dm_gemm(C.byref(a), _stream()), "dm_gemm")
    return c_pair if c_pair is not None else C_out


def _gemm_args(layout, A, B, C_out, M, N, K, lda, ldb, ldc, bias, residual, ldr, epilogue, aux, ldaux, accumulate, split_k,
               rows_per_group, group_stride, colsum_out, colsum_accumulate, ws_slot, c_pair=None, fold=None, min_slabs: int = 0) -> DmGemmArgs:
    a = DmGemmArgs()
    a.layout, a.ab_dtype, a.c_dtype = layout, _dt(A), _dt(C_out)
    if c_pair is not None:
        if _dt(A) != DM_BF16:
            raise ValueError("a plane-pair result goes with bf16 / folded operands")
        a.c_dtype, a.c_plane = _lib.DM_BF16_PAIR, M * N
    a.aux_dtype = _dt(aux) if aux is not None else DM_F32
    a.M, a.N, a.K = M, N, K
    a.epilogue, a.accumulate, a.split_k = epilogue, int(accumulate), split_k
    a.A, a.lda = A.data_ptr(), lda
    a.B, a.ldb = B.data_ptr(), ldb
    a.C, a.ldc = C_out.data_ptr(), (ldc if ldc is not None else N)
    a.bias = _ptr(bias)
    if bias is not None and (bias.dtype != torch.float32 or bias.numel() < N):
        raise ValueError("bias must be fp32 with >= N elements")
    a.residual, a.ldr = _ptr(residual), (ldr if ldr is not None else N)
    if residual is not None and residual.dtype != torch.float32:
        raise ValueError("residual must be fp32")
    a.aux, a.ldaux = _ptr(aux), (ldaux if ldaux is not None else N)
    a.rows_per_group, a.group_stride = rows_per_group, group_stride
    if colsum_out is not None:
        if colsum_out.dtype != torch.float32 or colsum_out.numel() < M or not colsum_out.is_contiguous():
            raise ValueError("colsum_out must be a contiguous fp32 tensor with >= M elements")
        a.colsum_a, a.colsum_accumulate = colsum_out.data_ptr(), int(colsum_accumulate)
    if fold is not None:
        a.k_fold = fold[0]
        a.a_fold[0], a.a_fold[1], a.a_fold[2] = 0, 0, fold[1]
        a.b_fold[0], a.b_fold[1], a.b_fold[2] = 0, fold[2], 0
    ws_bytes = _lib.lib().dm_gemm_workspace_bytes(layout, M, N, K) if (split_k != 1 or colsum_out is not None) else 0
    if split_k > 1:
        ws_bytes = max(ws_bytes, _lib.lib().dm_gemm_workspace_bytes(layout, M, N, K) + split_k * M * N * 4)
    if min_slabs > 0:
        ws_bytes = max(ws_bytes, _lib.lib().dm_gemm_workspace_bytes(layout, M, N, K) + min_slabs * M * N * 4)
    if ws_bytes > 0:
        ws = workspace(ws_bytes, A.device, ws_slot)
        a.workspace, a.workspace_bytes = ws.data_ptr(), ws.numel()
    return a


def gemm_grouped(calls) -> None:
    if not calls:
        return
    plain = len(calls) > 1
    for args, kw in calls:
        A, B = args[1], args[2]
        pair = isinstance(A, Planes) and isinstance(B, Planes)
        plain = plain and not isinstance(args[3], Planes) and (pair or (not isinstance(A, Planes) and not isinstance(B, Planes) and A.dtype == torch.bfloat16))
    if not plain:
        for args, kw in calls:
            gemm(*args, **kw)
        return
    arr = (DmGemmArgs * len(calls))()
    for i, (args, kw) in enumerate(calls):
        layout, A, B, C_out, M, N, K = args
        lda, ldb, fold = kw.get("lda"), kw.get("ldb"), None
        if isinstance(A, Planes):
            a_rows, a_cols = (M, K) if layout != DM_TN else (K, M)
            b_rows, b_cols = (N, K) if layout == DM_NT else (K, N)
            if (A.rows, A.cols) != (a_rows, a_cols) or (B.rows, B.cols) != (b_rows, b_cols):
                raise ValueError(f"plane pair shapes {(A.rows, A.cols)} / {(B.rows, B.cols)} do not match the product {(a_rows, a_cols)} / {(b_rows, b_cols)}")
            fold = (K, A.t.stride(0), B.t.stride(0))
            A, B, lda, ldb, K = A.t, B.t, a_cols, b_cols, 3 * K
        _need_cuda(A, B, C_out, kw.get("colsum_out"))
        if A.dtype != B.dtype:
            raise ValueError(f"A/B dtype mismatch: {A.dtype} vs {B.dtype}")
        lda = lda if lda is not None else (A.stride(-2) if A.dim() >= 2 else K)
        ldb = ldb if ldb is not None else (B.stride(-2) if B.dim() >= 2 else K)
        arr[i] = _gemm_args(layout, A, B, C_out, M, N, K, lda, ldb, kw.get("ldc"), kw.get("bias"), kw.get("residual"), kw.get("ldr"),
                            kw.get("epilogue", DM_EPI_NONE), kw.get("aux"), kw.get("ldaux"), kw.get("accumulate", False), kw.get("split_k", 0),
                            kw.get("rows_per_group", 0), kw.get("group_stride", 0), kw.get("colsum_out"), kw.get("colsum_accumulate", False),
                            f"{kw.get('ws_slot', 'gemm')}.g{i}", None, fold, min_slabs=16 if layout == DM_TN else 0)
    ws_bytes = _lib.lib().dm_gemm_grouped_workspace_bytes(arr, len(calls))
    ws = workspace(ws_bytes, calls[0][0][1].t.device if isinstance(calls[0][0][1], Planes) else calls[0][0][1].device, "gemm_grouped") if ws_bytes > 0 else None
    check(_lib.lib().dm_gemm_grouped(arr, len(calls), None if ws is None else ws.data_ptr(), 0 if ws is None else ws.numel(), _stream()), "dm_gemm_grouped")


def cast(src: torch.Tensor, dtype: torch.dtype) -> torch.Tensor:
    if src.dtype == dtype:
        return src
    _need_cuda(src)
    if src.dtype != torch.float32:
        raise ValueError("dm_cast source must be fp32")
    src = src.contiguous()
    dst = torch.empty(src.shape, dtype=dtype, device=src.device)
    check(_lib.lib().dm_cast(src.data_ptr(), dst.data_ptr(), _dt(dst), src.numel(), _stream()), "dm_cast")
    return dst


def colsum(X: torch.Tensor, out: torch.Tensor, accumulate: bool = False, ws_slot: str = "partial") -> torch.Tensor:
    _need_cuda(X, out)
    M, N = X.shape
    part = workspace(_lib.lib().dm_colsum_partial_floats(N) * 4, X.device, ws_slot)
    check(_lib.lib().dm_colsum(X.data_ptr(), _dt(X), X.stride(0), out.data_ptr(), M, N, int(accumulate), part.data_ptr(), _stream()), "dm_colsum")
    return out


def layernorm_fwd(x: torch.Tensor, gamma, beta, eps: float, out_dtype: torch.dtype, pair: bool = False):
    _need_cuda(x, gamma, beta)
    rows, cols = x.numel() // x.shape[-1], x.shape[-1]
    mean = torch.empty(rows, dtype=torch.float32, device=x.device)
    rstd = torch.empty(rows, dtype=torch.float32, device=x.device)
    if pair:
        yp = torch.empty((2, rows, cols), dtype=torch.bfloat16, device=x.device)
        check(_lib.lib().dm_layernorm_fwd(x.data_ptr(), gamma.data_ptr(), beta.data_ptr(), yp.data_ptr(), _lib.DM_BF16_PAIR, mean.data_ptr(),
                                          rstd.data_ptr(), rows, cols, eps, _stream()), "dm_layernorm_fwd")
        return Planes(yp), mean, rstd
    y = torch.empty(x.shape, dtype=out_dtype, device=x.device)
    check(_lib.lib().dm_layernorm_fwd(x.data_ptr(), gamma.data_ptr(), beta.data_ptr(), y.data_ptr(), _dt(y), mean.data_ptr(),
                                      rstd.data_ptr(), rows, cols, eps, _stream()), "dm_layernorm_fwd")
    return y, mean, rstd


_pending_reduce = []
_pending_out = set()
_flush_queued = False
_flush_task = -1


def _in_backward() -> bool:
    return torch._C._current_graph_task_id() != -1


def flush_reductions() -> None:
    global _flush_queued
    _flush_queued = False
    if not _pending_reduce:
        return
    items = (_lib.DmReduceItem * len(_pending_reduce))()
    for i, (f, _keep) in enumerate(_pending_reduce):
        items[i].partial, items[i].out0, items[i].out1, items[i].nrows, items[i].width, items[i].split, items[i].accumulate = f
    n = len(_pending_reduce)
    keep = list(_pending_reduce)
    _pending_reduce.clear()
    _pending_out.clear()
    check(_lib.lib().dm_partial_reduce_batch(items, n, _stream()), "dm_partial_reduce_batch")
    del keep


def _queue_reduce(part, out0, out1, nrows, width, split, accumulate) -> None:
    global _flush_queued, _flush_task
    task = torch._C._current_graph_task_id()
    if task != _flush_task:
        _pending_reduce.clear()
        _pending_out.clear()
        _flush_queued = False
        _flush_task = task
    keys = (out0.data_ptr(), out1.data_ptr())
    if keys[0] in _pending_out or keys[1] in _pending_out:
        flush_reductions()
    _pending_reduce.append(((part.data_ptr(), keys[0], keys[1], int(nrows), int(width), int(split), int(bool(accumulate))), (part, out0, out1)))
    _pending_out.update(keys)
    if not _flush_queued:
        torch.autograd.Variable._execution_engine.queue_callback(flush_reductions)
        _flush_queued = True


def layernorm_bwd(dy, x, gamma, mean, rstd, dres=None, dgamma=None, dbeta=None, accumulate=False, want_lp=False, defer=False, want_pair=False):
    _need_cuda(dy, x)
    if not (dy.is_contiguous() and x.is_contiguous()) or dy.numel() != x.numel():
        raise ValueError("layernorm_bwd: dy and x must be contiguous and of the same size (an expanded gradient has no rows to read)")
    rows, cols = x.numel() // x.shape[-1], x.shape[-1]
    dx = torch.empty(x.shape, dtype=torch.float32, device=x.device)
    dx_lp = torch.empty(x.shape, dtype=torch.bfloat16, device=x.device) if want_lp else None
    if dgamma is None:
        dgamma = torch.empty(cols, dtype=torch.float32, device=x.device)
        dbeta = torch.empty(cols, dtype=torch.float32, device=x.device)
        accumulate = False
        defer = False
    if want_pair:
        pair = torch.empty((2, rows, cols), dtype=torch.bfloat16, device=x.device)
        deferred = defer and _DEFER_REDUCTIONS and _in_backward()
        part = (torch.empty(_lib.lib().dm_layernorm_bwd_partial_floats(cols), dtype=torch.float32, device=x.device) if deferred
                else workspace(_lib.lib().dm_layernorm_bwd_partial_floats(cols) * 4, x.device, "partial").view(torch.float32))
        n_part = C.c_int32(0)
        check(_lib.lib().dm_layernorm_bwd_partials_pair(dy.data_ptr(), _dt(dy), x.data_ptr(), gamma.data_ptr(), mean.data_ptr(), rstd.data_ptr(),
                                                        _ptr(dres), dx.data_ptr(), pair.data_ptr(), part.data_ptr(), rows, cols, C.byref(n_part),
                                                        _stream()), "dm_layernorm_bwd_partials_pair")
        if deferred:
            _queue_reduce(part, dgamma, dbeta, n_part.value, 2 * cols, cols, accumulate)
        else:
            item = (_lib.DmReduceItem * 1)()
            item[0].partial, item[0].out0, item[0].out1 = part.data_ptr(), dgamma.data_ptr(), dbeta.data_ptr()
            item[0].nrows, item[0].width, item[0].split, item[0].accumulate = n_part.value, 2 * cols, cols, int(bool(accumulate))
            check(_lib.lib().dm_partial_reduce_batch(item, 1, _stream()), "dm_partial_reduce_batch")
        return dx, Planes(pair), dgamma, dbeta
    if defer and _DEFER_REDUCTIONS and _in_backward():
        part = torch.empty(_lib.lib().dm_layernorm_bwd_partial_floats(cols), dtype=torch.float32, device=x.device)
        n_part = C.c_int32(0)
        check(_lib.lib().dm_layernorm_bwd_partials(dy.data_ptr(), _dt(dy), x.data_ptr(), gamma.data_ptr(), mean.data_ptr(), rstd.data_ptr(),
                                                   _ptr(dres), dx.data_ptr(), _ptr(dx_lp), part.data_ptr(), rows, cols, C.byref(n_part),
                                                   _stream()), "dm_layernorm_bwd_partials")
        _queue_reduce(part, dgamma, dbeta, n_part.value, 2 * cols, cols, accumulate)
        return (dx, dx_lp, dgamma, dbeta) if want_lp else (dx, dgamma, dbeta)
    part = workspace(_lib.lib().dm_layernorm_bwd_partial_floats(cols) * 4, x.device, "partial")
    check(_lib.lib().dm_layernorm_bwd(dy.data_ptr(), _dt(dy), x.data_ptr(), gamma.data_ptr(), mean.data_ptr(), rstd.data_ptr(),
                                      _ptr(dres), dx.data_ptr(), _ptr(dx_lp), dgamma.data_ptr(), dbeta.data_ptr(), int(accumulate),
                                      part.data_ptr(), rows, cols, _stream()), "dm_layernorm_bwd")
    return (dx, dx_lp, dgamma, dbeta) if want_lp else (dx, dgamma, dbeta)


_DEFER_REDUCTIONS = os.environ.get("DM_DEFER_REDUCTIONS", "1") != "0"


def relpos_bias_gather(table: torch.Tensor, index32: torch.Tensor, N: int, transposed: bool = False):
    _need_cuda(table, index32)
    n_bins, H = table.shape
    bias = torch.empty((H, N, N), dtype=torch.float32, device=table.device)
    bias_t = torch.empty_like(bias) if transposed else None
    check(_lib.lib().dm_relpos_bias_gather(table.data_ptr(), index32.data_ptr(), bias.data_ptr(), _ptr(bias_t), N, H, n_bins, _stream()),
          "dm_relpos_bias_gather")
    return (bias, bias_t) if transposed else bias


def attention_fwd(qkv: torch.Tensor, bias: Optional[torch.Tensor], B: int, N: int, H: int, D: int, scale: float):
    _need_cuda(qkv, bias)
    out = torch.empty((B, N, H * D), dtype=qkv.dtype, device=qkv.device)
    lse = torch.empty((B, H, N), dtype=torch.float32, device=qkv.device)
    check(_lib.lib().dm_attention_fwd(qkv.data_ptr(), _ptr(bias), out.data_ptr(), lse.data_ptr(), B, N, H, D, scale, _dt(qkv), _stream()),
          "dm_attention_fwd")
    return out, lse


def _split_attention(table, index32, qkv, B, N, H, D):
    if (qkv if isinstance(qkv, torch.dtype) else qkv.dtype) != torch.float32 or _FP32_PRODUCTS != "bf16x3" or not _SPLIT_ATTENTION:
        return False, None
    cube = None if table is None else getattr(index32, "_dm_cube", None)
    if table is not None and cube is None:
        return False, None
    return attention_split_ok(B, N, H, D, cube), cube


_SPLIT_ATTENTION = os.environ.get("DM_ATTN_X3", "1") != "0"


def _inkernel_cube(table, index32, B, N, H, D, dtype):
    cube = None if table is None else getattr(index32, "_dm_cube", None)
    if cube is None or _INKERNEL_TABLE is False or not relpos_inkernel(B, N, H, D, cube, dtype):
        return None
    return cube


_INKERNEL_TABLE = os.environ.get("DM_ATTN_TABLE_IN_KERNEL", "1") != "0"


def relpos_inkernel(B: int, N: int, H: int, D: int, cube, dtype: torch.dtype) -> bool:
    if cube is None or len(cube) != 3:
        return False
    return bool(_lib.lib().dm_attention_relpos_inkernel(B, N, H, D, int(cube[0]), int(cube[1]), int(cube[2]),
                                                        DM_BF16 if dtype == torch.bfloat16 else DM_F32))


def attention_fwd_relpos(qkv: torch.Tensor, table: torch.Tensor, cube, B: int, N: int, H: int, D: int, scale: float):
    _need_cuda(qkv, table)
    if table.dtype != torch.float32 or not table.is_contiguous() or tuple(table.shape) != ((2 * cube[0] - 1) * (2 * cube[1] - 1) * (2 * cube[2] - 1), H):
        raise ValueError(f"attention_fwd_relpos: table must be contiguous fp32 [(2s-1)(2h-1)(2w-1), H], got {tuple(table.shape)} {table.dtype}")
    out = torch.empty((B, N, H * D), dtype=qkv.dtype, device=qkv.device)
    lse = torch.empty((B, H, N), dtype=torch.float32, device=qkv.device)
    check(_lib.lib().dm_attention_fwd_relpos(qkv.data_ptr(), table.data_ptr(), int(cube[0]), int(cube[1]), int(cube[2]), out.data_ptr(),
                                             lse.data_ptr(), B, N, H, D, scale, _dt(qkv), _stream()), "dm_attention_fwd_relpos")
    return out, lse


def attention_split_ok(B: int, N: int, H: int, D: int, cube=None) -> bool:
    c = (0, 0, 0) if cube is None else tuple(int(v) for v in cube)
    return bool(_lib.lib().dm_attention_split_ok(B, N, H, D, int(cube is not None), c[0], c[1], c[2]))


def attention_fwd_split(qkv: torch.Tensor, table: Optional[torch.Tensor], cube, B: int, N: int, H: int, D: int, scale: float, out_pair: bool = False):
    if table is not None and (table.dtype != torch.float32 or not table.is_contiguous()):
        raise ValueError("attention_fwd_split: table must be contiguous fp32")
    if isinstance(qkv, Planes):
        _need_cuda(qkv.t, table)
        hi, lo, src, dev = qkv.t[0], qkv.t[1], None, qkv.t.device
    else:
        _need_cuda(qkv, table)
        if qkv.dtype != torch.float32 or not qkv.is_contiguous():
            raise ValueError("attention_fwd_split: qkv must be a contiguous fp32 tensor")
        hi = torch.empty(qkv.shape, dtype=torch.bfloat16, device=qkv.device)
        lo = torch.empty(qkv.shape, dtype=torch.bfloat16, device=qkv.device)
        src, dev = qkv.data_ptr(), qkv.device
    out = torch.empty((B, N, H * D), dtype=torch.float32, device=dev)
    lse = torch.empty((B, H, N), dtype=torch.float32, device=dev)
    c = (0, 0, 0) if cube is None else tuple(int(v) for v in cube)
    if out_pair:
        op = torch.empty((2, B * N, H * D), dtype=torch.bfloat16, device=dev)
        check(_lib.lib().dm_attention_split_fwd_pair(src, hi.data_ptr(), lo.data_ptr(), _ptr(table), c[0], c[1], c[2], out.data_ptr(), op.data_ptr(),
                                                     lse.data_ptr(), B, N, H, D, scale, _stream()), "dm_attention_split_fwd_pair")
        return out, lse, hi, lo, Planes(op)
    check(_lib.lib().dm_attention_split_fwd(src, hi.data_ptr(), lo.data_ptr(), _ptr(table), c[0], c[1], c[2], out.data_ptr(),
                                            lse.data_ptr(), B, N, H, D, scale, _stream()), "dm_attention_split_fwd")
    return out, lse, hi, lo


def attention_bwd_split(hi, lo, table, cube, out, dout, lse, B, N, H, D, scale, index32=None, n_bins=0, pair=False):
    _need_cuda(hi, lo, table, out, dout, lse, index32)
    if out.dtype != torch.float32 or dout.dtype != torch.float32 or not (out.is_contiguous() and dout.is_contiguous()):
        raise ValueError("attention_bwd_split: out / dout must be contiguous fp32")
    dqkv = (torch.empty((2, B * N, 3 * H * D), dtype=torch.bfloat16, device=hi.device) if pair
            else torch.empty(hi.shape, dtype=torch.float32, device=hi.device))
    delta = torch.empty((B, H, N), dtype=torch.float32, device=hi.device)
    dhi = torch.empty(dout.shape, dtype=torch.bfloat16, device=hi.device)
    dlo = torch.empty(dout.shape, dtype=torch.bfloat16, device=hi.device)
    slab, info = None, None
    if index32 is not None and table is not None:
        chunks = _lib.lib().dm_attention_split_bwd_chunks(B, N, H)
        slab = torch.empty((chunks, H, N, N), dtype=torch.float32, device=hi.device)
        info = (chunks, N, relpos_index_csr(index32, n_bins))
    c = (0, 0, 0) if cube is None else tuple(int(v) for v in cube)
    fn = _lib.lib().dm_attention_split_bwd_pair if pair else _lib.lib().dm_attention_split_bwd
    check(fn(hi.data_ptr(), lo.data_ptr(), _ptr(table), c[0], c[1], c[2], out.data_ptr(), dout.data_ptr(),
             dhi.data_ptr(), dlo.data_ptr(), lse.data_ptr(), dqkv.data_ptr(), delta.data_ptr(), _ptr(slab),
             B, N, H, D, scale, _stream()), "dm_attention_split_bwd")
    return (Planes(dqkv) if pair else dqkv), slab, info


def relpos_index_csr(index32: torch.Tensor, n_bins: int):
    key = (index32._version, n_bins)
    hit = getattr(index32, "_dm_csr", None)
    if hit is None or hit[0] != key:
        flat = index32.reshape(-1).to(torch.int64)
        ok = (flat >= 0) & (flat < n_bins)
        where = torch.nonzero(ok).reshape(-1)
        order = torch.argsort(flat[where], stable=True)
        positions = where[order].to(torch.int32).contiguous()
        counts = torch.bincount(flat[where], minlength=n_bins)
        offsets = torch.zeros(n_bins + 1, dtype=torch.int64, device=index32.device)
        offsets[1:] = torch.cumsum(counts, 0)
        hit = index32._dm_csr = (key, positions, offsets.to(torch.int32).contiguous())
    return hit[1], hit[2]


def attention_bwd(qkv, bias, out, dout, lse, B, N, H, D, scale, index32=None, n_bins=0, bias_t=None, table=None, cube=None):
    _need_cuda(qkv, bias, out, dout, lse, index32, bias_t, table)
    dqkv = torch.empty_like(qkv)
    delta = torch.empty((B, H, N), dtype=torch.float32, device=qkv.device)
    slab, info = None, None
    if index32 is not None:
        if D != 64 or N > 256:
            raise ValueError(f"the relative-position bias gradient needs head dim 64 and N <= 256 (got D={D}, N={N})")
        chunks = _lib.lib().dm_attention_bwd_batch_chunks(B, N, H, _dt(qkv))
        slab = torch.empty((chunks, H, N, N), dtype=torch.float32, device=qkv.device)
        info = (chunks, N, relpos_index_csr(index32, n_bins))
    if table is not None and cube is not None:
        check(_lib.lib().dm_attention_bwd_relpos(qkv.data_ptr(), table.data_ptr(), int(cube[0]), int(cube[1]), int(cube[2]), _ptr(bias),
                                                 _ptr(bias_t), out.data_ptr(), dout.data_ptr(), lse.data_ptr(), dqkv.data_ptr(),
                                                 delta.data_ptr(), _ptr(slab), B, N, H, D, scale, _dt(qkv), _stream()),
              "dm_attention_bwd_relpos")
        return dqkv, slab, info
    check(_lib.lib().dm_attention_bwd(qkv.data_ptr(), _ptr(bias), _ptr(bias_t), out.data_ptr(), dout.data_ptr(), lse.data_ptr(), dqkv.data_ptr(),
                                      delta.data_ptr(), _ptr(slab), B, N, H, D, scale, _dt(qkv), _stream()),
          "dm_attention_bwd")
    return dqkv, slab, info


def relpos_bias_scatter(slab, dtable, B, H, info, n_bins, accumulate=False):
    _need_cuda(slab, dtable)
    chunks, N, (positions, offsets) = info
    check(_lib.lib().dm_relpos_bias_reduce(slab.data_ptr(), positions.data_ptr(), offsets.data_ptr(), dtable.data_ptr(), chunks, H, N,
                                           n_bins, int(accumulate), _stream()), "dm_relpos_bias_reduce")
    return dtable


def patchify(x: torch.Tensor, patch: int, dtype: torch.dtype) -> torch.Tensor:
    _need_cuda(x)
    B, Cc, H, W = x.shape
    if H != W:
        raise ValueError("square images only")
    x = x.contiguous()
    g = H // patch
    cols = torch.empty((B * g * g, Cc * patch * patch), dtype=dtype, device=x.device)
    check(_lib.lib().dm_patchify(x.data_ptr(), cols.data_ptr(), _dt(cols), B, Cc, H, patch, _stream()), "dm_patchify")
    return cols


RESIZE_RULES = {"opencv": 0, "exact_area": 1}


def _resize_rule(resize: str) -> int:
    if resize not in RESIZE_RULES:
        raise ValueError(f"resize must be one of {tuple(RESIZE_RULES)}, got {resize!r}")
    return RESIZE_RULES[resize]


def patch_pyramid(tile: torch.Tensor, xy: torch.Tensor, windows: torch.Tensor, target: int, max_window: Optional[int] = None,
                  resize: str = "opencv") -> torch.Tensor:
    _need_cuda(tile, xy, windows)
    if tile.dtype != torch.uint8:
        raise ValueError("tile must be uint8")
    bands, H, W = tile.shape
    P = xy.shape[0]
    if max_window is None:
        max_window = int(windows.max().item())
    out = torch.empty((P, bands, target, target), dtype=torch.float32, device=tile.device)
    check(_lib.lib().dm_patch_pyramid(tile.contiguous().data_ptr(), bands, H, W, xy.to(torch.int32).contiguous().data_ptr(),
                                      windows.to(torch.int32).contiguous().data_ptr(), max_window, P, target, _resize_rule(resize),
                                      out.data_ptr(), _stream()), "dm_patch_pyramid")
    return out


class PatchCols:

    def __init__(self, cols: torch.Tensor, batch: int, side: int, patch: int, bands: int):
        self.cols, self.batch, self.side, self.patch, self.bands = cols, batch, side, patch, bands

    @property
    def shape(self):
        return (self.batch, self.bands, self.side, self.side)

    def __getitem__(self, sl):
        g2 = (self.side // self.patch) ** 2
        if not isinstance(sl, slice) or sl.step not in (None, 1):
            raise TypeError("PatchCols supports contiguous batch slices only")
        a, b, _ = sl.indices(self.batch)
        return PatchCols(self.cols[a * g2:b * g2], b - a, self.side, self.patch, self.bands)

    def to(self, *_a, **_k):
        return self

    @staticmethod
    def cat(a: "PatchCols", b: "PatchCols") -> "PatchCols":
        if (a.side, a.patch, a.bands, a.cols.dtype) != (b.side, b.patch, b.bands, b.cols.dtype):
            raise ValueError("PatchCols.cat: the two sides were built for different scales / dtypes")
        ca, cb = a.cols, b.cols
        if (ca.is_contiguous() and cb.is_contiguous() and ca.untyped_storage().data_ptr() == cb.untyped_storage().data_ptr()
                and cb.data_ptr() == ca.data_ptr() + ca.numel() * ca.element_size()):
            both = ca.as_strided((ca.shape[0] + cb.shape[0], ca.shape[1]), (ca.shape[1], 1), ca.storage_offset())
        else:
            both = torch.cat((ca, cb), 0)
        return PatchCols(both, a.batch + b.batch, a.side, a.patch, a.bands)


def cat_batch(a, b):
    if isinstance(a, PatchCols) or isinstance(b, PatchCols):
        return PatchCols.cat(a, b)
    return torch.cat((a, b), 0)


def pair_batch_gather(tiles: torch.Tensor, tile_id: Optional[torch.Tensor], xy: torch.Tensor, inner: torch.Tensor, obj: torch.Tensor,
                      scale_index: int, target: int, max_window: int, out: torch.Tensor, grid: int = 0, resize: str = "opencv",
                      region_features: Optional[torch.Tensor] = None, designed: Optional[torch.Tensor] = None,
                      error_flag: Optional[torch.Tensor] = None) -> None:
    _need_cuda(tiles, tile_id, xy, inner, obj, out, region_features, designed, error_flag)
    if tiles.dtype != torch.uint8 or tiles.dim() != 4 or not tiles.is_contiguous():
        raise ValueError("tiles must be a contiguous uint8 [T, bands, H, W] tensor")
    for name, t in (("tile_id", tile_id), ("xy", xy), ("inner", inner), ("obj", obj), ("error_flag", error_flag)):
        if t is not None and (t.dtype != torch.int32 or not t.is_contiguous()):
            raise ValueError(f"{name} must be a contiguous int32 tensor (a per-step cast would be a launch of its own)")
    T, bands, H, W = tiles.shape
    P = xy.shape[0]
    if not out.is_contiguous() or out.numel() != P * bands * target * target:
        raise ValueError(f"out must be contiguous with {P * bands * target * target} elements, got {tuple(out.shape)}")
    if (region_features is None) != (designed is None):
        raise ValueError("designed rows need the region features (and vice versa)")
    if designed is not None and (designed.dtype != torch.float32 or designed.numel() != P * 19 or not designed.is_contiguous()
                                 or region_features.dtype != torch.float32 or region_features.numel() != P * 15 or not region_features.is_contiguous()):
        raise ValueError("region_features must be contiguous float32 [P, 15] and designed contiguous float32 [P, 1, 19]")
    check(_lib.lib().dm_pair_batch_gather(tiles.data_ptr(), T, bands, H, W, _ptr(tile_id), xy.data_ptr(), inner.data_ptr(), obj.data_ptr(),
                                          scale_index, max_window, P, target, grid, _resize_rule(resize), out.data_ptr(), _dt(out),
                                          _ptr(region_features), _ptr(designed), _ptr(error_flag), _stream()), "dm_pair_batch_gather")


def pair_epoch_draw(pairs: torch.Tensor, pair_flag: torch.Tensor, poly_off: torch.Tensor, poly_pts: torch.Tensor, pt_tile: torch.Tensor,
                    pt_xy: torch.Tensor, pt_inner: torch.Tensor, pt_obj: torch.Tensor, pt_region: torch.Tensor, seed: int, epoch: int, batch: int,
                    tile_id: torch.Tensor, xy: torch.Tensor, inner: torch.Tensor, obj: torch.Tensor, region: torch.Tensor, flag: torch.Tensor,
                    point_id: Optional[torch.Tensor] = None) -> None:
    if pairs.dim() != 2 or pairs.shape[1] != 2:
        raise ValueError(f"pair_epoch_draw: pairs must be [N, 2], got {tuple(pairs.shape)}")
    N, n_pts = pairs.shape[0], pt_tile.numel()
    cols = {"pairs": (pairs, torch.int32, 2 * N), "pair_flag": (pair_flag, torch.int32, N), "poly_off": (poly_off, torch.int32, poly_off.numel()),
            "poly_pts": (poly_pts, torch.int32, poly_pts.numel()), "pt_tile": (pt_tile, torch.int32, n_pts), "pt_xy": (pt_xy, torch.int32, 2 * n_pts),
            "pt_inner": (pt_inner, torch.int32, n_pts), "pt_obj": (pt_obj, torch.int32, n_pts), "pt_region": (pt_region, torch.float32, 15 * n_pts),
            "tile_id": (tile_id, torch.int32, 2 * N), "xy": (xy, torch.int32, 4 * N), "inner": (inner, torch.int32, 2 * N),
            "obj": (obj, torch.int32, 2 * N), "region": (region, torch.float32, 30 * N), "flag": (flag, torch.float32, N),
            "point_id": (point_id, torch.int32, 2 * N)}
    _need_cuda(*(t for t, _, _ in cols.values()))
    for name, (t, dtype, numel) in cols.items():
        if t is not None and (t.dtype != dtype or not t.is_contiguous() or t.numel() != numel):
            raise ValueError(f"pair_epoch_draw: {name} must be a contiguous {dtype} tensor of {numel} elements, got {t.dtype} {tuple(t.shape)}")
    a = _lib.DmPairDraw()
    for name, (t, _, _) in cols.items():
        setattr(a, name, _ptr(t))
    a.seed = int(seed) & 0xFFFFFFFFFFFFFFFF
    a.n_pairs, a.n_poly, a.n_poly_pts, a.n_pts = N, poly_off.numel() - 1, poly_pts.numel(), n_pts
    a.epoch, a.batch = int(epoch), int(batch)
    with torch.cuda.device(pairs.device):
        check(_lib.lib().dm_pair_epoch_draw(C.byref(a), _stream()), "dm_pair_epoch_draw")


def patch_pyramid_cols(tile: torch.Tensor, xy: torch.Tensor, windows: torch.Tensor, target: int, grid: int = 8,
                       dtype: torch.dtype = torch.bfloat16, max_window: Optional[int] = None, resize: str = "opencv") -> PatchCols:
    _need_cuda(tile, xy, windows)
    if tile.dtype != torch.uint8:
        raise ValueError("tile must be uint8")
    bands, H, W = tile.shape
    P = xy.shape[0]
    if target % grid:
        raise ValueError(f"target {target} is not a multiple of the token grid {grid}")
    ps = target // grid
    if max_window is None:
        max_window = int(windows.max().item())
    cols = torch.empty((P * grid * grid, bands * ps * ps), dtype=dtype, device=tile.device)
    check(_lib.lib().dm_patch_pyramid_cols(tile.contiguous().data_ptr(), bands, H, W, xy.to(torch.int32).contiguous().data_ptr(),
                                           windows.to(torch.int32).contiguous().data_ptr(), max_window, P, target, grid, _resize_rule(resize),
                                           cols.data_ptr(), _dt(cols), _stream()), "dm_patch_pyramid_cols")
    return PatchCols(cols, P, target, ps, bands)
# ... 638 lines not shown

class BlockFn(torch.autograd.Function):

    @staticmethod
    def forward(ctx, x, n1w, n1b, table, index32, qkv_w, qkv_b, proj_w, proj_b, n2w, n2b, fc1_w, fc1_b, fc2_w, fc2_b,
                heads, eps, scale, dtype):
        _save_products(ctx)
        x = x.contiguous()
        B, N, Cc = x.shape
        M, Hd, D = B * N, fc1_w.shape[0], Cc // heads
        dev = x.device
        wq, wp = lp_weight(qkv_w, dtype, (3 * Cc, Cc)), lp_weight(proj_w, dtype, (Cc, Cc))
        w1, w2 = lp_weight(fc1_w, dtype, (Hd, Cc)), lp_weight(fc2_w, dtype, (Cc, Hd))
        x2d = x.view(M, Cc)
        planes = (dtype == torch.float32 and _FP32_PRODUCTS == "bf16x3" and planes_ok(M, Cc) and planes_ok(M, Hd) and planes_ok(Hd, Cc)
                  and Cc <= _PAIR_LN_MAX_COLS and M * Cc * Cc >= _SPLIT_MIN_WORK)
        if planes:
            wq, wp, w1, w2 = (pair_weight(P, w) for P, w in ((qkv_w, wq), (proj_w, wp), (fc1_w, w1), (fc2_w, w2)))
        y1, mean1, rstd1 = layernorm_fwd(x2d, n1w, n1b, eps, dtype, pair=planes)
        split, scube = _split_attention(table, index32, dtype, B, N, heads, D)
        qkv = (Planes(torch.empty((2, M, 3 * Cc), dtype=torch.bfloat16, device=dev)) if (planes and split)
               else torch.empty((M, 3 * Cc), dtype=dtype, device=dev))
        gemm(DM_NT, y1, wq, qkv, M, 3 * Cc, Cc, lda=Cc, ldb=Cc, ldc=3 * Cc, bias=qkv_b)
        bias = bias_t = None
        cube = _inkernel_cube(table, index32, B, N, heads, D, dtype)
        split_imgs = None
        if split:
            o_op = None
            if planes:
                o, lse, hi, lo, o_op = attention_fwd_split(qkv, None if table is None else table.contiguous(), scube, B, N, heads, D, scale, out_pair=True)
            else:
                o, lse, hi, lo = attention_fwd_split(qkv, None if table is None else table.contiguous(), scube, B, N, heads, D, scale)
            split_imgs = (hi, lo, scube)
        elif cube is not None:
            o, lse = attention_fwd_relpos(qkv, table.contiguous(), cube, B, N, heads, D, scale)
        else:
            if table is not None:
                bias, bias_t = relpos_bias_gather(table.contiguous(), index32, N, transposed=True)
            o, lse = attention_fwd(qkv, bias, B, N, heads, D, scale)
        x1 = torch.empty((M, Cc), dtype=torch.float32, device=dev)
        if not (planes and split):
            o_op = split_planes(o.view(M, Cc)) if planes else o.view(M, Cc)
        gemm(DM_NT, o_op, wp, x1, M, Cc, Cc, lda=Cc, ldb=Cc, ldc=Cc, bias=proj_b, residual=x2d)
        y2, mean2, rstd2 = layernorm_fwd(x1, n2w, n2b, eps, dtype, pair=planes)
        h = Planes(torch.empty((2, M, Hd), dtype=torch.bfloat16, device=dev)) if planes else torch.empty((M, Hd), dtype=dtype, device=dev)
        if any(ctx.needs_input_grad):
            pre = torch.empty((M, Hd), dtype=dtype, device=dev)
            gemm(DM_NT, y2, w1, h, M, Hd, Cc, lda=Cc, ldb=Cc, ldc=Hd, bias=fc1_b, epilogue=DM_EPI_GELU_GRAD, aux=pre, ldaux=Hd)
        else:
            pre = None
            gemm(DM_NT, y2, w1, h, M, Hd, Cc, lda=Cc, ldb=Cc, ldc=Hd, bias=fc1_b, epilogue=DM_EPI_GELU)
        x2 = torch.empty((M, Cc), dtype=torch.float32, device=dev)
        gemm(DM_NT, h, w2, x2, M, Cc, Hd, lda=Hd, ldb=Hd, ldc=Cc, bias=fc2_b, residual=x1)
        if planes:
            y1, y2, h, wq, wp, w1, w2, o_op = y1.t, y2.t, h.t, wq.t, wp.t, w1.t, w2.t, o_op.t
            if isinstance(qkv, Planes):
                qkv = qkv.t
        ctx.planes = planes
        ctx.save_for_backward(x2d, mean1, rstd1, y1, qkv, o, lse, bias, bias_t, index32, x1, mean2, rstd2, y2, pre, h,
                              wq, wp, w1, w2, n1w, n2w, o_op if planes else None)
        ctx.dims = (B, N, Cc, heads, D, Hd, scale, None if table is None else table.shape[0])
        ctx.table_in_kernel = cube is not None
        ctx.split_imgs = split_imgs
        ctx.params = (n1w, n1b, table, qkv_w, qkv_b, proj_w, proj_b, n2w, n2b, fc1_w, fc1_b, fc2_w, fc2_b)
        return x2.view(B, N, Cc)

    @staticmethod
    @_replay_products
    def backward(ctx, dx2):
        (x, mean1, rstd1, y1, qkv, o, lse, bias, bias_t, index32, x1, mean2, rstd2, y2, pre, h,
         wq, wp, w1, w2, n1w, n2w, o_op) = ctx.saved_tensors
        planes = ctx.planes
        if planes:
            y1, y2, h, wq, wp, w1, w2, o_op = (Planes(t_) for t_ in (y1, y2, h, wq, wp, w1, w2, o_op))
        (P_n1w, P_n1b, P_table, P_qkv_w, P_qkv_b, P_proj_w, P_proj_b, P_n2w, P_n2b, P_fc1_w, P_fc1_b, P_fc2_w, P_fc2_b) = ctx.params
        B, N, Cc, heads, D, Hd, scale, n_bins = ctx.dims
        M = B * N
        dtype, dev = (torch.float32 if planes else y1.dtype), x.device
        lp = dtype != torch.float32
        lp_copy = getattr(dx2, "_dm_lp_copy", None)
        dy_pair = getattr(dx2, "_dm_planes", None)
        if dy_pair is not None and dy_pair[1] != (dx2.data_ptr(), dx2._version):
            dy_pair = None
        elif dy_pair is not None:
            dy_pair = dy_pair[0]
        dx2 = dx2.contiguous().view(M, Cc)
        if lp_copy is not None:
            dx2._dm_lp_copy = lp_copy
        dy = _operand_grad(dx2, dtype)
        if planes and isinstance(dy_pair, Planes) and (dy_pair.rows, dy_pair.cols) == (M, Cc):
            dy = dy_pair
        dw2, k_w2 = _grad_out(P_fc2_w, (Cc, Hd), dev)
        db2, k_b2 = _grad_out(P_fc2_b, (Cc,), dev)
        side = _side_stream(dev) if 0 < M <= _WGRAD_SIDE_TOKENS else None

        pending = [] if (side is None and (lp or planes) and 0 < M <= _WGRAD_GROUP_TOKENS) else None
        late = [] if (pending is None and side is None and (lp or planes) and _WGRAD_PAIR) else None

        def wgrad(*a, pair=False, **kw):
            if pending is not None:
                pending.append((a, kw))
                return None
            if late is not None and pair:
                late.append((a, kw))
                return None
            if side is None:
                return gemm(*a, **kw)
            side.wait_stream(torch.cuda.current_stream())
            with torch.cuda.stream(side):
                return gemm(*a, ws_slot="gemm_side", **kw)

        def bias_grad(g2d, db, acc_b, direct):
            if planes and not isinstance(g2d, Planes):
                g2d = split_planes(g2d)
            return g2d, dict(colsum_out=db, colsum_accumulate=acc_b)
        dy, cs = bias_grad(dy, db2, _acc(P_fc2_b, k_b2), k_b2)
        wgrad(DM_TN, dy, h, dw2, Cc, Hd, M, lda=Cc, ldb=Hd, ldc=Hd, accumulate=_acc(P_fc2_w, k_w2), **cs)
        dpre = Planes(torch.empty((2, M, Hd), dtype=torch.bfloat16, device=dev)) if planes else torch.empty((M, Hd), dtype=dtype, device=dev)
        gemm(DM_NN, dy, w2, dpre, M, Hd, Cc, lda=Cc, ldb=Hd, ldc=None if planes else Hd, epilogue=DM_EPI_MUL, aux=pre, ldaux=Hd)
        dw1, k_w1 = _grad_out(P_fc1_w, (Hd, Cc), dev)
        db1, k_b1 = _grad_out(P_fc1_b, (Hd,), dev)
        dpre, cs = bias_grad(dpre, db1, _acc(P_fc1_b, k_b1), k_b1)
        wgrad(DM_TN, dpre, y2, dw1, Hd, Cc, M, lda=Hd, ldb=Cc, ldc=Cc, accumulate=_acc(P_fc1_w, k_w1), **cs)
        dy2 = torch.empty((M, Cc), dtype=dtype, device=dev)
        gemm(DM_NN, dpre, w1, dy2, M, Cc, Hd, lda=Hd, ldb=Cc, ldc=Cc)
        dg2, k_n2 = _grad_out(P_n2w, (Cc,), dev)
        dbt2, k_n2b = _grad_out(P_n2b, (Cc,), dev)
        if k_n2 != k_n2b:
            dg2, dbt2, k_n2, k_n2b = torch.empty(Cc, device=dev), torch.empty(Cc, device=dev), False, False
        a_n2 = _acc(P_n2w, k_n2)
        _acc(P_n2b, k_n2b)
        r = layernorm_bwd(dy2, x1, n2w, mean2, rstd2, dres=dx2, dgamma=dg2, dbeta=dbt2, accumulate=a_n2, want_lp=lp, defer=bool(k_n2 and k_n2b),
                          want_pair=planes)
        dx1, dx1_lp = (r[0], r[1]) if (lp or planes) else (r[0], r[0])
        dwp, k_wp = _grad_out(P_proj_w, (Cc, Cc), dev)
        dbp, k_bp = _grad_out(P_proj_b, (Cc,), dev)
        dx1_op, cs = bias_grad(dx1_lp, dbp, _acc(P_proj_b, k_bp), k_bp)
        wgrad(DM_TN, dx1_op, o_op if planes else o.view(M, Cc), dwp, Cc, Cc, M, lda=Cc, ldb=Cc, ldc=Cc, accumulate=_acc(P_proj_w, k_wp), pair=True, **cs)
        do = torch.empty((M, Cc), dtype=dtype, device=dev)
        gemm(DM_NN, dx1_op, wp, do, M, Cc, Cc, lda=Cc, ldb=Cc, ldc=Cc)
        tab, cube = None, None
        if ctx.split_imgs is not None:
            hi, lo, scube = ctx.split_imgs
            ctx.split_imgs = None
            want_table = P_table is not None
            dqkv, slab, rows = attention_bwd_split(hi, lo, None if P_table is None else P_table.detach().contiguous(), scube, o.view(B, N, Cc),
                                                   do.view(B, N, Cc), lse, B, N, heads, D, scale, index32 if want_table else None, n_bins or 0,
                                                   pair=planes)
        else:
            if ctx.table_in_kernel:
                tab, cube = P_table.detach().contiguous(), index32._dm_cube
            want_table = bias is not None or tab is not None
            dqkv, slab, rows = attention_bwd(qkv, bias, o, do, lse, B, N, heads, D, scale,
                                             index32 if want_table else None, n_bins or 0, bias_t=bias_t, table=tab, cube=cube)
        dtable, k_t = None, False
        if want_table:
            dtable, k_t = _grad_out(P_table, (n_bins, heads), dev)
            relpos_bias_scatter(slab, dtable, B, heads, rows, n_bins, accumulate=_acc(P_table, k_t))
        dqkv2 = dqkv if isinstance(dqkv, Planes) else dqkv.view(M, 3 * Cc)
        dwq, k_wq = _grad_out(P_qkv_w, (3 * Cc, Cc), dev)
        dbq, k_bq = _grad_out(P_qkv_b, (3 * Cc,), dev)
        dqkv_op, cs = bias_grad(dqkv2, dbq, _acc(P_qkv_b, k_bq), k_bq)
        wgrad(DM_TN, dqkv_op, y1, dwq, 3 * Cc, Cc, M, lda=3 * Cc, ldb=Cc, ldc=Cc, accumulate=_acc(P_qkv_w, k_wq), pair=True, **cs)
        dy1 = torch.empty((M, Cc), dtype=dtype, device=dev)
        gemm(DM_NN, dqkv_op, wq, dy1, M, Cc, 3 * Cc, lda=3 * Cc, ldb=Cc, ldc=Cc)
        dg1, k_n1 = _grad_out(P_n1w, (Cc,), dev)
        dbt1, k_n1b = _grad_out(P_n1b, (Cc,), dev)
        if k_n1 != k_n1b:
            dg1, dbt1, k_n1, k_n1b = torch.empty(Cc, device=dev), torch.empty(Cc, device=dev), False, False
        a_n1 = _acc(P_n1w, k_n1)
        _acc(P_n1b, k_n1b)
        r = layernorm_bwd(dy1, x, n1w, mean1, rstd1, dres=dx1, dgamma=dg1, dbeta=dbt1, accumulate=a_n1, want_lp=lp, defer=bool(k_n1 and k_n1b),
                          want_pair=planes)
        if side is not None:
            torch.cuda.current_stream().wait_stream(side)
        if pending:
            gemm_grouped(pending)
        if late:
            gemm_grouped(late)
        dx = r[0].view(B, N, Cc)
        if lp:
            dx._dm_lp_copy = r[1]
        if planes:
            dx._dm_planes = (r[1], (dx.data_ptr(), dx._version))
        return (dx, _grad_done(P_n1w, dg1, k_n1), _grad_done(P_n1b, dbt1, k_n1b),
                _grad_done(P_table, dtable, k_t) if want_table else None, None,
                _grad_done(P_qkv_w, dwq, k_wq), _grad_done(P_qkv_b, dbq, k_bq),
                _grad_done(P_proj_w, dwp, k_wp), _grad_done(P_proj_b, dbp, k_bp),
                _grad_done(P_n2w, dg2, k_n2), _grad_done(P_n2b, dbt2, k_n2b),
                _grad_done(P_fc1_w, dw1, k_w1), _grad_done(P_fc1_b, db1, k_b1),
                _grad_done(P_fc2_w, dw2, k_w2), _grad_done(P_fc2_b, db2, k_b2), None, None, None, None)
```

include/deepmerge_hip.h:

```cpp
#ifndef DEEPMERGE_HIP_H
#define DEEPMERGE_HIP_H

#include <stdint.h>

#ifdef __cplusplus
extern "C" {
#endif

typedef enum { DM_F32 = 0, DM_BF16 = 1,
               DM_BF16_PAIR = 2,
               DM_F64 = 3
} DmDtype;

typedef enum {
  DM_OK = 0,
  DM_ERR_BAD_SHAPE = -1,
  DM_ERR_BAD_DTYPE = -2,
  DM_ERR_BAD_ALIGN = -3,
  DM_ERR_WORKSPACE = -4,
  DM_ERR_HIP = -5,
  DM_ERR_UNSUPPORTED = -6
} DmStatus;

int dm_abi_version(void);
const char *dm_last_error(void);
const char *dm_arch(void);

typedef enum { DM_NT = 0, DM_NN = 1, DM_TN = 2 } DmGemmLayout;
typedef enum { DM_EPI_NONE = 0, DM_EPI_GELU = 1, DM_EPI_DGELU = 2, DM_EPI_GELU_GRAD = 3, DM_EPI_MUL = 4 } DmEpilogue;

typedef struct {
  int32_t layout;
  int32_t ab_dtype;
  int32_t c_dtype;
  int32_t aux_dtype;
  int32_t M, N, K;
  int32_t epilogue;
  int32_t accumulate;
  int32_t split_k;
  const void *A; int64_t lda;
  const void *B; int64_t ldb;
  void *C; int64_t ldc;
  const float *bias;
  const float *residual; int64_t ldr;
  void *aux; int64_t ldaux;
  int32_t rows_per_group; int64_t group_stride;
  void *workspace; int64_t workspace_bytes;
  float *colsum_a; int32_t colsum_accumulate;
  int32_t k_fold;
  int64_t a_fold[3], b_fold[3];
  int64_t c_plane;
} DmGemmArgs;

int dm_gemm(const DmGemmArgs *args, void *stream);
int64_t dm_gemm_workspace_bytes(int32_t layout, int32_t M, int32_t N, int32_t K);
int64_t dm_gemm_grouped_workspace_bytes(const DmGemmArgs *args, int32_t n);
int dm_gemm_grouped(const DmGemmArgs *args, int32_t n, void *workspace, int64_t workspace_bytes, void *stream);

int dm_attention_fwd(const void *qkv, const float *bias, void *out, float *lse,
                     int32_t B, int32_t N, int32_t H, int32_t D, float scale, int32_t dtype, void *stream);
int32_t dm_attention_relpos_inkernel(int32_t B, int32_t N, int32_t H, int32_t D, int32_t cube_s, int32_t cube_h,
                                     int32_t cube_w, int32_t dtype);
int dm_attention_fwd_relpos(const void *qkv, const float *table, int32_t cube_s, int32_t cube_h, int32_t cube_w,
                            void *out, float *lse, int32_t B, int32_t N, int32_t H, int32_t D, float scale,
                            int32_t dtype, void *stream);
int dm_attention_bwd(const void *qkv, const float *bias, const float *bias_t, const void *out, const void *dout,
                     const float *lse, void *dqkv, float *delta, float *dbias_slab, int32_t B, int32_t N, int32_t H,
                     int32_t D, float scale, int32_t dtype, void *stream);
int dm_attention_bwd_relpos(const void *qkv, const float *table, int32_t cube_s, int32_t cube_h, int32_t cube_w,
                            const float *bias, const float *bias_t, const void *out, const void *dout, const float *lse,
                            void *dqkv, float *delta, float *dbias_slab, int32_t B, int32_t N, int32_t H, int32_t D,
                            float scale, int32_t dtype, void *stream);
int32_t dm_attention_split_ok(int32_t B, int32_t N, int32_t H, int32_t D, int32_t has_table, int32_t cube_s, int32_t cube_h,
                              int32_t cube_w);
int dm_attention_split_fwd(const float *qkv, void *qkv_hi, void *qkv_lo, const float *table, int32_t cube_s, int32_t cube_h,
                           int32_t cube_w, float *out, float *lse, int32_t B, int32_t N, int32_t H, int32_t D, float scale,
                           void *stream);
int dm_attention_split_fwd_pair(const float *qkv, void *qkv_hi, void *qkv_lo, const float *table, int32_t cube_s, int32_t cube_h,
                                int32_t cube_w, float *out, void *out_pair, float *lse, int32_t B, int32_t N, int32_t H, int32_t D,
                                float scale, void *stream);
int32_t dm_attention_split_bwd_chunks(int32_t B, int32_t N, int32_t H);
int dm_attention_split_bwd(const void *qkv_hi, const void *qkv_lo, const float *table, int32_t cube_s, int32_t cube_h,
                           int32_t cube_w, const float *out, const float *dout, void *dout_hi, void *dout_lo,
                           const float *lse, float *dqkv, float *delta, float *dbias_slab, int32_t B, int32_t N,
                           int32_t H, int32_t D, float scale, void *stream);
int dm_attention_split_bwd_pair(const void *qkv_hi, const void *qkv_lo, const float *table, int32_t cube_s, int32_t cube_h,
                                int32_t cube_w, const float *out, const float *dout, void *dout_hi, void *dout_lo,
                                const float *lse, void *dqkv_pair, float *delta, float *dbias_slab, int32_t B, int32_t N,
                                int32_t H, int32_t D, float scale, void *stream);
int32_t dm_attention_bwd_batch_chunks(int32_t B, int32_t N, int32_t H, int32_t dtype);

int dm_relpos_bias_gather(const float *table, const int32_t *index, float *bias, float *bias_t,
                          int32_t N, int32_t H, int32_t n_bins, void *stream);
int dm_relpos_bias_reduce(float *dbias_slab, const int32_t *positions, const int32_t *offsets, float *dtable,
                          int32_t chunks, int32_t H, int32_t N, int32_t n_bins, int32_t accumulate, void *stream);

int dm_layernorm_fwd(const float *x, const float *gamma, const float *beta, void *y, int32_t y_dtype,
                     float *mean, float *rstd, int32_t rows, int32_t cols, float eps, void *stream);
int dm_layernorm_bwd(const void *dy, int32_t dy_dtype, const float *x, const float *gamma,
                     const float *mean, const float *rstd, const float *dres, float *dx, void *dx_lp,
                     float *dgamma, float *dbeta, int32_t accumulate_params, float *partial,
                     int32_t rows, int32_t cols, void *stream);
int64_t dm_layernorm_bwd_partial_floats(int32_t cols);
int dm_layernorm_bwd_partials(const void *dy, int32_t dy_dtype, const float *x, const float *gamma,
                              const float *mean, const float *rstd, const float *dres, float *dx, void *dx_lp,
                              float *partial, int32_t rows, int32_t cols, int32_t *n_partial, void *stream);
int dm_layernorm_bwd_partials_pair(const void *dy, int32_t dy_dtype, const float *x, const float *gamma,
                                   const float *mean, const float *rstd, const float *dres, float *dx, void *dx_pair, float *partial,
                                   int32_t rows, int32_t cols, int32_t *n_partial, void *stream);
typedef struct DmReduceItem {
  const float *partial;
  float *out0, *out1;
  int32_t nrows, width, split, accumulate;
} DmReduceItem;
int dm_partial_reduce_batch(const DmReduceItem *items, int32_t n, void *stream);

int dm_token_pool_fwd(const float *x, float *y, int32_t B, int32_t S, int32_t side, int32_t C, void *stream);
int dm_token_pool_bwd(const float *dy, float *dx, int32_t B, int32_t S, int32_t side, int32_t C, void *stream);
int dm_group_mean_fwd(const float *x, float *y, int32_t rows, int32_t g, int32_t C, void *stream);
int dm_group_mean_bwd(const float *dy, float *dx, int32_t rows, int32_t g, int32_t C, void *stream);

int dm_colsum(const void *X, int32_t dtype, int64_t ldx, float *out, int32_t M, int32_t N,
              int32_t accumulate, float *partial, void *stream);
int64_t dm_colsum_partial_floats(int32_t N);

int dm_cast(const float *src, void *dst, int32_t dst_dtype, int64_t n, void *stream);

int dm_split_bf16(const float *src, int64_t ld, int64_t rows, int64_t cols, void *dst, int32_t stack, int32_t pattern, void *stream);
int64_t dm_split_colsum_partial_floats(int64_t rows, int64_t cols);
int dm_split_bf16_planes(const float *src, int64_t ld, int64_t rows, int64_t cols, void *dst, float *partial, int32_t *n_partial, void *stream);
int dm_split_bf16_colsum(const float *src, int64_t ld, int64_t rows, int64_t cols, void *dst, int32_t stack, int32_t pattern,
                         float *partial, int32_t *n_partial, void *stream);

int dm_patchify(const float *x, void *cols, int32_t dtype, int32_t B, int32_t C, int32_t side, int32_t p, void *stream);

int dm_contrastive_loss(const float *a, const float *b, const float *flag, float margin, float upstream,
                        float *loss, float *da, float *db, int32_t B, int32_t D, void *stream);

int dm_cross_entropy(const float *logits, const int64_t *target_index, const float *target_prob, float upstream,
                     float *loss, float *dlogits, int32_t B, int32_t K, void *stream);

int dm_adam_step(float *param, const float *grad, float *m, float *v, void *param_lp, int64_t n,
                 int32_t step, double lr, double beta1, double beta2, double eps, double grad_scale, void *stream);

int dm_adam_hyper(int32_t step, double lr, double beta1, double beta2, float *hyper_host);
int dm_adam_step_dev(float *param, const float *grad, float *m, float *v, void *param_lp, int64_t n, const float *hyper_dev,
                     double beta1, double beta2, double eps, double grad_scale, void *stream);
int dm_adam_step_dev_pair(float *param, const float *grad, float *m, float *v, void *param_hi, void *param_lo, int64_t n,
                          const float *hyper_dev, double beta1, double beta2, double eps, double grad_scale, void *stream);

int dm_segment_mean(const float *F, const int32_t *ptr, const int32_t *idx, float *pooled,
                    int32_t S, int32_t D, void *stream);
int dm_edge_similarity(const float *pooled, const int32_t *edges, float *simi, uint8_t *merge,
                       int32_t E, int32_t D, float margin, void *stream);
int dm_pairwise_distance(const void *X, const void *Y, void *D, int32_t n, int32_t m, int32_t p, int32_t dtype, void *stream);

#define DM_RESIZE_OPENCV 0
#define DM_RESIZE_EXACT_AREA 1
int dm_patch_pyramid(const uint8_t *tile, int32_t bands, int32_t H, int32_t W, const int32_t *xy, const int32_t *windows,
                     int32_t max_window, int32_t P, int32_t target, int32_t resize_rule, float *out, void *stream);
int dm_patch_pyramid_cols(const uint8_t *tile, int32_t bands, int32_t H, int32_t W, const int32_t *xy, const int32_t *windows,
                          int32_t max_window, int32_t P, int32_t target, int32_t grid, int32_t resize_rule, void *cols, int32_t dtype,
                          void *stream);

int dm_pair_batch_gather(const uint8_t *tiles, int32_t n_tiles, int32_t bands, int32_t H, int32_t W, const int32_t *tile_id,
                         const int32_t *xy, const int32_t *inner, const int32_t *obj, int32_t scale_index, int32_t max_window,
                         int32_t P, int32_t target, int32_t grid, int32_t resize_rule, void *out, int32_t dtype,
                         const float *region_features, float *designed, int32_t *error_flag, void *stream);

typedef struct {
  const int32_t *pairs, *pair_flag, *poly_off, *poly_pts;
  const int32_t *pt_tile, *pt_xy, *pt_inner, *pt_obj;
  const float *pt_region;
  int32_t *tile_id, *xy, *inner, *obj;
  float *region, *flag;
  int32_t *point_id;
  uint64_t seed;
  int32_t n_pairs, n_poly, n_poly_pts, n_pts, epoch, batch;
} DmPairDraw;
int dm_pair_epoch_draw(const DmPairDraw *args, void *stream);

int dm_contrastive_terms(const float *a, const float *b, const float *flag, float margin, float *d2, float *term, int32_t B, int32_t D,
                         void *stream);
int64_t dm_pair_eval_workspace_bytes(int64_t N, int32_t T);
int dm_pair_eval_summary(const float *term, const float *simi, const float *flag, int64_t N, const float *thresholds, int32_t T,
                         void *workspace, double *loss_sum, int64_t *merged, int64_t *n_pos, void *stream);

int dm_label_stats(const int32_t *labels, const uint8_t *tile, int32_t bands, int32_t H, int32_t W, int32_t S,
                   int64_t *count, int64_t *sum, int64_t *sumsq, int32_t *bbox, int64_t *peri, void *stream);
int dm_label_features(const int64_t *count, const int64_t *sum, const int64_t *sumsq, const int32_t *bbox, const int64_t *peri,
                      int32_t S, int32_t bands, float *features, void *stream);
int dm_rag_edges(const int32_t *labels, int32_t H, int32_t W, int32_t S, int64_t *table_keys, int32_t *table_counts,
                 int32_t capacity_log2, int64_t *edge_keys, int32_t *edge_counts, int32_t max_edges, int32_t *n_edges,
                 int32_t *overflow, void *stream);

int dm_merge_round(const int32_t *edges, const uint8_t *merge, int32_t E, int32_t S, int32_t *parent, int32_t *changed,
                   int32_t init, void *stream);

int64_t dm_batchnorm_workspace_bytes(int32_t M, int32_t C);
int dm_batchnorm_fwd(const float *x, const float *gamma, const float *beta, float *running_mean, float *running_var,
                     const float *mask, int32_t rows_per_sample, float *y, float *save_mean, float *save_rstd, int32_t M,
                     int32_t C, float eps, float momentum, int32_t training, int32_t relu, void *workspace, void *stream);
int dm_batchnorm_bwd(const float *dy, const float *x, const float *y, const float *gamma, const float *mask, int32_t rows_per_sample,
                     const float *save_mean, const float *save_rstd, float *dx, float *dgamma, float *dbeta, int32_t accumulate,
                     int32_t M, int32_t C, int32_t training, int32_t relu, void *workspace, void *stream);

int dm_gru_cell_fwd(const float *gi, int64_t gi_stride, const float *gh, const float *h, float *h_new, float *saved,
                    int32_t B, int32_t H, void *stream);
int dm_gru_cell_bwd(const float *dh_new, const float *saved, const float *h, float *dgi, float *dgh, float *dh, int32_t B,
                    int32_t H, void *stream);

typedef struct {
  char name[64];
  int64_t launches;
  double total_ms;
  double total_flops;
  double total_bytes;
} DmProfRow;
int dm_prof_enable(int32_t on);
int32_t dm_prof_collect(DmProfRow *rows, int32_t max_rows);

#ifdef __cplusplus
}
#endif
#endif
```

Before: 6252 pairs/s.

## Bin relative-position bias gradients inside the dK/dV kernel and batch slab reductions

The Q32 table-reading dK/dV backward kernel now folds its per-block bias-gradient accumulators into relative-position bins in shared memory and writes per-block partial table rows. It does not write a full N×N fp32 slab per chunk that a separate scatter kernel then reads back. These partial rows, and the remaining slab-to-table scatters, are queued into the deferred batched reduction launch. The aim is to cut the slab's memory traffic and the extra kernel launches, at the cost of more shared-memory work and syncs at the end of the attention backward kernel.

```diff
diff --git a/deepmerge_amd/_lib.py b/deepmerge_amd/_lib.py
--- a/deepmerge_amd/_lib.py
+++ b/deepmerge_amd/_lib.py
@@ -47,6 +47,11 @@
                 ("nrows", C.c_int32), ("width", C.c_int32), ("split", C.c_int32), ("accumulate", C.c_int32)]
 
 
+class DmRelposItem(C.Structure):
+    _fields_ = [("slab", C.c_void_p), ("positions", C.c_void_p), ("offsets", C.c_void_p), ("dtable", C.c_void_p),
+                ("chunks", C.c_int32), ("H", C.c_int32), ("N", C.c_int32), ("n_bins", C.c_int32), ("accumulate", C.c_int32)]
+
+
 class DmPairDraw(C.Structure):
     _fields_ = [("pairs", C.c_void_p), ("pair_flag", C.c_void_p), ("poly_off", C.c_void_p), ("poly_pts", C.c_void_p),
                 ("pt_tile", C.c_void_p), ("pt_xy", C.c_void_p), ("pt_inner", C.c_void_p), ("pt_obj", C.c_void_p),
@@ -86,6 +91,8 @@
     "dm_attention_bwd_relpos": (_I, [_P, _P, _I, _I, _I, _P, _P, _P, _P, _P, _P, _P, _P, _I, _I, _I, _I, _F, _I, _P]),
     "dm_attention_bwd": (_I, [_P, _P, _P, _P, _P, _P, _P, _P, _P, _I, _I, _I, _I, _F, _I, _P]),
     "dm_attention_bwd_batch_chunks": (_I, [_I, _I, _I, _I]),
+    "dm_attention_bwd_bin_rows": (_I, [_I, _I, _I, _I, _I, _I, _I, _I]),
+    "dm_attention_bwd_relpos_binned": (_I, [_P, _P, _I, _I, _I, _P, _P, _P, _P, _P, _P, _I, _I, _I, _I, _F, _I, _P]),
     "dm_relpos_bias_gather": (_I, [_P, _P, _P, _P, _I, _I, _I, _P]),
     "dm_relpos_bias_reduce": (_I, [_P, _P, _P, _P, _I, _I, _I, _I, _I, _P]),
     "dm_layernorm_fwd": (_I, [_P, _P, _P, _P, _I, _P, _P, _I, _I, _F, _P]),
@@ -93,6 +100,7 @@
     "dm_layernorm_bwd_partials": (_I, [_P, _I, _P, _P, _P, _P, _P, _P, _P, _P, _I, _I, C.POINTER(C.c_int32), _P]),
     "dm_layernorm_bwd_partials_pair": (_I, [_P, _I, _P, _P, _P, _P, _P, _P, _P, _P, _I, _I, C.POINTER(C.c_int32), _P]),
     "dm_partial_reduce_batch": (_I, [C.POINTER(DmReduceItem), _I, _P]),
+    "dm_reduce_flush": (_I, [C.POINTER(DmReduceItem), _I, C.POINTER(DmRelposItem), _I, _P]),
     "dm_layernorm_bwd_partial_floats": (_L, [_I]),
     "dm_token_pool_fwd": (_I, [_P, _P, _I, _I, _I, _I, _P]),
     "dm_token_pool_bwd": (_I, [_P, _P, _I, _I, _I, _I, _P]),
diff --git a/deepmerge_amd/csrc/dm_attention.hip b/deepmerge_amd/csrc/dm_attention.hip
--- a/deepmerge_amd/csrc/dm_attention.hip
+++ b/deepmerge_amd/csrc/dm_attention.hip
@@ -490,6 +490,7 @@
     if (const char *e = getenv("DM_ATTN_XCD")) v.xcd = atoi(e) != 0;
     if (const char *e = getenv("DM_ATTN_X3")) v.x3 = atoi(e) != 0;
     if (const char *e = getenv("DM_ATTN_X3_W8")) v.x3_w8 = atoi(e) != 0;
+    if (const char *e = getenv("DM_ATTN_Q32_TABBIN")) v.q32_tabbin = atoi(e) != 0;
     return v;
   }();
   return sw;
@@ -588,6 +589,7 @@
       else if (sw.q32_bwd != 3 && !c.dense && !c.slab) pl.dkv = pass32(c, ATTN_Q32, ATTN_BIAS_NONE, w, 32 * w);
     }
     pl.slab_chunks = pl.dkv.chunks;
+    if (pl.dkv.family == ATTN_Q32_TABKV && sw.q32_tabbin) pl.bin_rows = pl.dkv.chunks * pl.dkv.nblk;
   }
   if (table_only && pl.dkv.family != ATTN_Q32_TABKV) pl.refused = ATTN_TABLE_NOT_TAKEN;
   return pl;
@@ -668,8 +670,8 @@
 }
 
 static int attention_bwd(const void *qkv, const float *bias, const float *bias_t, const float *table, int32_t cube_s, const void *out,
-                         const void *dout, const float *lse, void *dqkv, float *delta, float *dbias_slab, int32_t B, int32_t N, int32_t H,
-                         int32_t D, float scale, int32_t dtype, void *stream) {
+                         const void *dout, const float *lse, void *dqkv, float *delta, float *dbias_slab, float *dtable_part, int32_t B,
+                         int32_t N, int32_t H, int32_t D, float scale, int32_t dtype, void *stream) {
   if (dm_attn_generic_shape(N, D)) {
     DM_REQUIRE(B > 0 && H > 0 && H <= 65535 && B <= 65535 && (dtype == DM_F32 || dtype == DM_BF16) && qkv && out && dout && lse && dqkv && delta,
                DM_ERR_BAD_SHAPE, "dm_attention_bwd: bad arguments (B=%d H=%d dtype=%d)", B, H, dtype);
@@ -684,7 +686,9 @@
   DM_REQUIRE(dm_aligned16(qkv) && dm_aligned16(out) && dm_aligned16(dout) && dm_aligned16(dqkv) && dm_aligned16(bias) &&
              dm_aligned16(bias_t) && dm_aligned16(lse) && dm_aligned16(delta) && dm_aligned16(dbias_slab), DM_ERR_BAD_ALIGN,
              "dm_attention_bwd: tensors must be 16-byte aligned");
-  const AttnBwdPlan pl = attn_plan_bwd(AttnCall{B, N, H, D, dtype, bias != nullptr, table != nullptr, cube_s, dbias_slab != nullptr, false}, attn_switches());
+  const AttnBwdPlan pl = attn_plan_bwd(AttnCall{B, N, H, D, dtype, bias != nullptr, table != nullptr, cube_s,
+                                                dbias_slab != nullptr || dtable_part != nullptr, false}, attn_switches());
+  DM_REQUIRE(!dtable_part || pl.bin_rows > 0, DM_ERR_UNSUPPORTED, "dm_attention_bwd_relpos_binned: the plan has no binned form for this call");
   DM_REQUIRE(pl.refused != ATTN_TABLE_NEEDS_BF16, DM_ERR_UNSUPPORTED, "dm_attention_bwd_relpos: the table-reading kernels are bf16 only");
   DM_REQUIRE(!pl.refused, DM_ERR_UNSUPPORTED,
              "dm_attention_bwd_relpos: the table-reading backward kernels do not take this call (B=%d N=%d H=%d, switches "
@@ -705,6 +709,7 @@
       AttnPipeBwdParams pp{qkv, bias, out, dout, lse, delta, dqkv, dbias_slab, B, N, H, scale};
       pp.table = table;
       pp.cube_s = cube_s;
+      pp.tab_part = dtable_part;
       DM_REQUIRE(pl.dq.family != ATTN_Q32 || dm_attn_bwd_dq_q32(pl, pp, s), DM_ERR_HIP, "dm_attention_bwd: the dQ kernel could not be configured");
       if (pl.dkv.family == ATTN_PIPE16) dm_attn_bwd_pipe(pl, pp, s);
       else DM_REQUIRE(dm_attn_bwd_dkv_q32(pl, pp, s), DM_ERR_HIP, "dm_attention_bwd: the dK / dV kernel could not be configured");
@@ -717,7 +722,7 @@
 extern "C" int dm_attention_bwd(const void *qkv, const float *bias, const float *bias_t, const void *out, const void *dout,
                                 const float *lse, void *dqkv, float *delta, float *dbias_slab, int32_t B, int32_t N, int32_t H, int32_t D, float scale, int32_t dtype,
                                 void *stream) {
-  return attention_bwd(qkv, bias, bias_t, nullptr, 0, out, dout, lse, dqkv, delta, dbias_slab, B, N, H, D, scale, dtype, stream);
+  return attention_bwd(qkv, bias, bias_t, nullptr, 0, out, dout, lse, dqkv, delta, dbias_slab, nullptr, B, N, H, D, scale, dtype, stream);
 }
 
 extern "C" int dm_attention_bwd_relpos(const void *qkv, const float *table, int32_t cube_s, int32_t cube_h, int32_t cube_w, const float *bias,
@@ -727,7 +732,24 @@
   DM_REQUIRE(bias || dm_attention_relpos_inkernel(B, N, H, D, cube_s, cube_h, cube_w, dtype), DM_ERR_UNSUPPORTED,
              "dm_attention_bwd_relpos: shape not taken (B=%d N=%d H=%d D=%d cube=%dx%dx%d dtype=%d); call dm_attention_bwd", B, N, H, D, cube_s,
              cube_h, cube_w, dtype);
-  return attention_bwd(qkv, bias, bias_t, table, cube_s, out, dout, lse, dqkv, delta, dbias_slab, B, N, H, D, scale, dtype, stream);
+  return attention_bwd(qkv, bias, bias_t, table, cube_s, out, dout, lse, dqkv, delta, dbias_slab, nullptr, B, N, H, D, scale, dtype, stream);
+}
+
+extern "C" int32_t dm_attention_bwd_bin_rows(int32_t B, int32_t N, int32_t H, int32_t D, int32_t cube_s, int32_t cube_h, int32_t cube_w,
+                                             int32_t dtype) {
+  if (!dm_attention_relpos_inkernel(B, N, H, D, cube_s, cube_h, cube_w, dtype)) return 0;
+  return attn_plan_bwd(table_call(B, N, H, D, cube_s, cube_h, cube_w, dtype, false), attn_switches()).bin_rows;
+}
+
+extern "C" int dm_attention_bwd_relpos_binned(const void *qkv, const float *table, int32_t cube_s, int32_t cube_h, int32_t cube_w,
+                                              const void *out, const void *dout, const float *lse, void *dqkv, float *delta,
+                                              float *dtable_part, int32_t B, int32_t N, int32_t H, int32_t D, float scale, int32_t dtype,
+                                              void *stream) {
+  DM_REQUIRE(table && dtable_part, DM_ERR_BAD_SHAPE, "dm_attention_bwd_relpos_binned: null table or partial rows");
+  DM_REQUIRE(dm_attention_bwd_bin_rows(B, N, H, D, cube_s, cube_h, cube_w, dtype) > 0, DM_ERR_UNSUPPORTED,
+             "dm_attention_bwd_relpos_binned: shape or switches not taken (B=%d N=%d H=%d D=%d cube=%dx%dx%d dtype=%d); use dm_attention_bwd_relpos",
+             B, N, H, D, cube_s, cube_h, cube_w, dtype);
+  return attention_bwd(qkv, nullptr, nullptr, table, cube_s, out, dout, lse, dqkv, delta, nullptr, dtable_part, B, N, H, D, scale, dtype, stream);
 }
 
 static AttnCall split_call(int32_t B, int32_t N, int32_t H, int32_t D, bool has_table, int32_t cube_s, int32_t cube_h, int32_t cube_w, bool slab) {
diff --git a/deepmerge_amd/csrc/dm_attention_pipe.h b/deepmerge_amd/csrc/dm_attention_pipe.h
--- a/deepmerge_amd/csrc/dm_attention_pipe.h
+++ b/deepmerge_amd/csrc/dm_attention_pipe.h
@@ -30,6 +30,7 @@
   float scale;
   const float *table = nullptr;
   int cube_s = 0;
+  float *tab_part = nullptr;
 };
 
 void dm_attn_bwd_pipe(const AttnBwdPlan &pl, const AttnPipeBwdParams &p, hipStream_t s);
diff --git a/deepmerge_amd/csrc/dm_attention_plan.h b/deepmerge_amd/csrc/dm_attention_plan.h
--- a/deepmerge_amd/csrc/dm_attention_plan.h
+++ b/deepmerge_amd/csrc/dm_attention_plan.h
@@ -11,6 +11,7 @@
   bool xcd = true;
   bool x3 = true;
   bool x3_w8 = true;
+  bool q32_tabbin = true;
 };
 const AttnSwitches &attn_switches();
 
@@ -52,6 +53,7 @@
   AttnPass dq, dkv;
   bool xcd;
   int slab_chunks;
+  int bin_rows;
 };
 AttnFwdPlan attn_plan_fwd(const AttnCall &c, const AttnSwitches &sw);
 AttnBwdPlan attn_plan_bwd(const AttnCall &c, const AttnSwitches &sw);
diff --git a/deepmerge_amd/csrc/dm_attention_q32_bwd.hip b/deepmerge_amd/csrc/dm_attention_q32_bwd.hip
--- a/deepmerge_amd/csrc/dm_attention_q32_bwd.hip
+++ b/deepmerge_amd/csrc/dm_attention_q32_bwd.hip
@@ -937,7 +937,76 @@
       load_rows(b + 1, kld, vld, lse_ld, dl_ld);
     }
   }
-  if (wave_live && p.slab) {
+  if (p.tab_part) {
+    constexpr int S = NKT / 2, PP = 129;
+    static_assert(NP * PP * 4 <= 4 * IMG + 2 * STAT, "the plane fits the image and stat regions");
+    float *plane = reinterpret_cast<float *>(smem);
+    __syncthreads();
+    if (wave_live) {
+#pragma unroll
+      for (int j = 0; j < NKT; ++j) {
+        asm volatile("s_nop 15\n\ts_nop 7" : "+a"(hacc[j]));
+#pragma unroll
+        for (int i = 0; i < 16; ++i) plane[(32 * j + 8 * (i >> 2) + 4 * hh + (i & 3)) * PP + wave * 32 + r] = hacc[j][i];
+      }
+    }
+    __syncthreads();
+    constexpr int NQR = NP / 8, XU = NQR * 16 * 8 / 256;
+    float xs[XU][2];
+    {
+      const int k = t & 7, krow = (t >> 3) & 15;
+#pragma unroll
+      for (int m = 0; m < XU; ++m) {
+        const int qrow = (t >> 7) + 2 * m;
+        float v[8];
+#pragma unroll
+        for (int s = 0; s < 8; ++s) v[s] = plane[(qrow * 8 + ((s + k) & 7)) * PP + krow * 8 + s];
+        float a = 0.f, b = 0.f;
+#pragma unroll
+        for (int s = 0; s < 8; ++s) {
+          if (s < 8 - k) a += v[s]; else b += v[s];
+        }
+        xs[m][0] = a;
+        xs[m][1] = b;
+      }
+    }
+    __syncthreads();
+    float *A = plane, *Bs = plane + 8192;
+    {
+      const int k = t & 7, krow = (t >> 3) & 15;
+#pragma unroll
+      for (int m = 0; m < XU; ++m) {
+        const int qrow = (t >> 7) + 2 * m;
+        A[(qrow * 16 + krow) * 15 + k + 7] = xs[m][0];
+        if (k > 0) A[(qrow * 16 + krow) * 15 + k - 1] = xs[m][1];
+      }
+    }
+    __syncthreads();
+    for (int u = t; u < S * 2 * 15 * 8; u += 256) {
+      const int k = u & 7, dxi = (u >> 3) % 15, zz = (u >> 3) / 15, kzl = zz & 1, qz = zz >> 1;
+      float a = 0.f, b = 0.f;
+#pragma unroll
+      for (int s = 0; s < 8; ++s) {
+        const float v = A[((qz * 8 + ((s + k) & 7)) * 16 + kzl * 8 + s) * 15 + dxi];
+        if (s < 8 - k) a += v; else b += v;
+      }
+      float *o = Bs + (qz * 2 + kzl) * 225 + dxi;
+      o[(k + 7) * 15] = a;
+      if (k > 0) o[(k - 1) * 15] = b;
+    }
+    __syncthreads();
+    float *row = p.tab_part + (long long)(chunk * nblk + rb) * TAB_N * H + h;
+    for (int bin = t; bin < TAB_N; bin += 256) {
+      const int bz = bin / 225, dyx = bin - bz * 225, dz = bz - (S - 1);
+      float acc = 0.f;
+#pragma unroll
+      for (int kzl = 0; kzl < 2; ++kzl) {
+        const int kz = 2 * rb + kzl, qz = kz + dz;
+        if (kz < S && qz >= 0 && qz < S) acc += Bs[(qz * 2 + kzl) * 225 + dyx];
+      }
+      row[(long long)bin * H] = acc;
+    }
+  } else if (wave_live && p.slab) {
     float *sl = p.slab + ((long long)(chunk * H + h) * N) * N + key;
 #pragma unroll
     for (int j = 0; j < NKT; ++j) {
diff --git a/deepmerge_amd/csrc/dm_rows.hip b/deepmerge_amd/csrc/dm_rows.hip
--- a/deepmerge_amd/csrc/dm_rows.hip
+++ b/deepmerge_amd/csrc/dm_rows.hip
@@ -207,9 +207,47 @@
   DmReduceItem it[32];
   int start[33];
   int n;
+  DmRelposItem rp[8];
+  int rstart[9];
+  int nr;
 };
+__device__ void relpos_batch_job(const DmRelposItem &it, int blk) {
+  const int lane = threadIdx.x & 63, wave = threadIdx.x >> 6;
+  const int hq = (it.H + 3) / 4, bin = blk / hq, h = (blk - bin * hq) * 4 + wave;
+  if (h >= it.H) return;
+  const int beg = it.offsets[bin], cnt = it.offsets[bin + 1] - beg;
+  const long long plane = (long long)it.N * it.N, cstride = (long long)it.H * plane;
+  const float *__restrict__ pl = it.slab + h * plane;
+  float acc = 0.f;
+  for (int j = lane; j < cnt; j += 64) {
+    const long long e = it.positions[beg + j];
+    float v = pl[e];
+    int c = 1;
+    for (; c + 8 <= it.chunks; c += 8) {
+      float w[8];
+#pragma unroll
+      for (int i = 0; i < 8; ++i) w[i] = pl[(c + i) * cstride + e];
+#pragma unroll
+      for (int i = 0; i < 8; ++i) v += w[i];
+    }
+    for (; c < it.chunks; ++c) v += pl[c * cstride + e];
+    acc += v;
+  }
+  acc = dm_wave_sum(acc);
+  if (lane == 0) {
+    float *o = it.dtable + (long long)bin * it.H + h;
+    *o = it.accumulate ? *o + acc : acc;
+  }
+}
 __global__ __launch_bounds__(256) void partial_reduce_batch_kernel(const ReduceBatch rb) {
   __shared__ float red[16][17];
+  if ((int)blockIdx.x >= rb.start[rb.n]) {
+    const int blk = (int)blockIdx.x - rb.start[rb.n];
+    int r = 0;
+    while (r + 1 < rb.nr && blk >= rb.rstart[r + 1]) ++r;
+    relpos_batch_job(rb.rp[r], blk - rb.rstart[r]);
+    return;
+  }
   int job = 0;
   while (job + 1 < rb.n && (int)blockIdx.x >= rb.start[job + 1]) ++job;
   const DmReduceItem &it = rb.it[job];
@@ -680,26 +718,47 @@
                      "dm_layernorm_bwd_partials_pair", true);
 }
 
+extern "C" int dm_reduce_flush(const DmReduceItem *items, int32_t n, const DmRelposItem *slabs, int32_t ns, void *stream) {
+  DM_REQUIRE(n >= 0 && ns >= 0 && n + ns > 0 && (items || n == 0) && (slabs || ns == 0), DM_ERR_BAD_SHAPE, "dm_reduce_flush: no items");
+  for (int32_t i = 0; i < n; ++i) {
+    const DmReduceItem &it = items[i];
+    DM_REQUIRE(it.partial && it.out0 && it.out1 && it.nrows > 0 && it.width > 0 && it.split >= 0 && it.split <= it.width, DM_ERR_BAD_SHAPE,
+               "dm_partial_reduce_batch: item %d: nrows=%d width=%d split=%d", i, it.nrows, it.width, it.split);
+  }
+  for (int32_t i = 0; i < ns; ++i) {
+    const DmRelposItem &it = slabs[i];
+    DM_REQUIRE(it.slab && it.positions && it.offsets && it.dtable && it.chunks > 0 && it.H > 0 && it.N > 0 && it.n_bins > 0 &&
+               (long long)it.n_bins * ((it.H + 3) / 4) < (1LL << 30), DM_ERR_BAD_SHAPE,
+               "dm_reduce_flush: slab %d: chunks=%d H=%d N=%d n_bins=%d", i, it.chunks, it.H, it.N, it.n_bins);
+  }
+  hipStream_t s = reinterpret_cast<hipStream_t>(stream);
+  for (int32_t base = 0, rbase = 0; base < n || rbase < ns; base += 32, rbase += 8) {
+    ReduceBatch rb;
+    rb.n = base >= n ? 0 : (n - base < 32) ? n - base : 32;
+    rb.nr = rbase >= ns ? 0 : (ns - rbase < 8) ? ns - rbase : 8;
+    int total = 0;
+    for (int i = 0; i < rb.n; ++i) {
+      rb.it[i] = items[base + i];
+      rb.start[i] = total;
+      total += (rb.it[i].width + 15) / 16;
+    }
+    for (int i = rb.n; i <= 32; ++i) rb.start[i] = total;
+    int rtotal = 0;
+    for (int i = 0; i < rb.nr; ++i) {
+      rb.rp[i] = slabs[rbase + i];
+      rb.rstart[i] = rtotal;
+      rtotal += rb.rp[i].n_bins * ((rb.rp[i].H + 3) / 4);
+    }
+    for (int i = rb.nr; i <= 8; ++i) rb.rstart[i] = rtotal;
+    hipLaunchKernelGGL(partial_reduce_batch_kernel, dim3(total + rtotal), dim3(256), 0, s, rb);
+    DM_LAUNCH_CHECK("dm_reduce_flush");
+  }
+  return DM_OK;
+}
+
 extern "C" int dm_partial_reduce_batch(const DmReduceItem *items, int32_t n, void *stream) {
   DM_REQUIRE(items && n > 0, DM_ERR_BAD_SHAPE, "dm_partial_reduce_batch: no items");
-  hipStream_t s = reinterpret_cast<hipStream_t>(stream);
-  for (int32_t base = 0; base < n; base += 32) {
-    ReduceBatch rb;
-    rb.n = (n - base < 32) ? n - base : 32;
-    int total = 0;
-    for (int i = 0; i < rb.n; ++i) {
-      const DmReduceItem &it = items[base + i];
-      DM_REQUIRE(it.partial && it.out0 && it.out1 && it.nrows > 0 && it.width > 0 && it.split >= 0 && it.split <= it.width, DM_ERR_BAD_SHAPE,
-                 "dm_partial_reduce_batch: item %d: nrows=%d width=%d split=%d", base + i, it.nrows, it.width, it.split);
-      rb.it[i] = it;
-      rb.start[i] = total;
-      total += (it.width + 15) / 16;
-    }
-    for (int i = rb.n; i <= 32; ++i) rb.start[i] = total;
-    hipLaunchKernelGGL(partial_reduce_batch_kernel, dim3(total), dim3(256), 0, s, rb);
-    DM_LAUNCH_CHECK("dm_partial_reduce_batch");
-  }
-  return DM_OK;
+  return dm_reduce_flush(items, n, nullptr, 0, stream);
 }
 
 extern "C" int dm_token_pool_fwd(const float *x, float *y, int32_t B, int32_t S, int32_t side, int32_t C, void *stream) {
diff --git a/deepmerge_amd/ops.py b/deepmerge_amd/ops.py
--- a/deepmerge_amd/ops.py
+++ b/deepmerge_amd/ops.py
@@ -363,6 +363,7 @@
 
 
 _pending_reduce = []
+_pending_slab = []
 _pending_out = set()
 _flush_queued = False
 _flush_task = -1
@@ -375,35 +376,48 @@
 def flush_reductions() -> None:
     global _flush_queued
     _flush_queued = False
-    if not _pending_reduce:
+    if not _pending_reduce and not _pending_slab:
         return
-    items = (_lib.DmReduceItem * len(_pending_reduce))()
+    n, ns = len(_pending_reduce), len(_pending_slab)
+    items = (_lib.DmReduceItem * max(n, 1))()
     for i, (f, _keep) in enumerate(_pending_reduce):
         items[i].partial, items[i].out0, items[i].out1, items[i].nrows, items[i].width, items[i].split, items[i].accumulate = f
-    n = len(_pending_reduce)
-    keep = list(_pending_reduce)
+    slabs = (_lib.DmRelposItem * max(ns, 1))()
+    for i, (f, _keep) in enumerate(_pending_slab):
+        (slabs[i].slab, slabs[i].positions, slabs[i].offsets, slabs[i].dtable, slabs[i].chunks, slabs[i].H, slabs[i].N, slabs[i].n_bins,
+         slabs[i].accumulate) = f
+    keep = list(_pending_reduce) + list(_pending_slab)
     _pending_reduce.clear()
+    _pending_slab.clear()
     _pending_out.clear()
-    check(_lib.lib().dm_partial_reduce_batch(items, n, _stream()), "dm_partial_reduce_batch")
+    if ns:
+        check(_lib.lib().dm_reduce_flush(items, n, slabs, ns, _stream()), "dm_reduce_flush")
+    else:
+        check(_lib.lib().dm_partial_reduce_batch(items, n, _stream()), "dm_partial_reduce_batch")
     del keep
 
 
-def _queue_reduce(part, out0, out1, nrows, width, split, accumulate) -> None:
+def _queue(pending, fields, keep, keys) -> None:
     global _flush_queued, _flush_task
     task = torch._C._current_graph_task_id()
     if task != _flush_task:
         _pending_reduce.clear()
+        _pending_slab.clear()
         _pending_out.clear()
         _flush_queued = False
         _flush_task = task
-    keys = (out0.data_ptr(), out1.data_ptr())
-    if keys[0] in _pending_out or keys[1] in _pending_out:
+    if any(k in _pending_out for k in keys):
         flush_reductions()
-    _pending_reduce.append(((part.data_ptr(), keys[0], keys[1], int(nrows), int(width), int(split), int(bool(accumulate))), (part, out0, out1)))
+    pending.append((fields, keep))
     _pending_out.update(keys)
     if not _flush_queued:
         torch.autograd.Variable._execution_engine.queue_callback(flush_reductions)
         _flush_queued = True
+
+
+def _queue_reduce(part, out0, out1, nrows, width, split, accumulate) -> None:
+    keys = (out0.data_ptr(), out1.data_ptr())
+    _queue(_pending_reduce, (part.data_ptr(), keys[0], keys[1], int(nrows), int(width), int(split), int(bool(accumulate))), (part, out0, out1), keys)
 
 
 def layernorm_bwd(dy, x, gamma, mean, rstd, dres=None, dgamma=None, dbeta=None, accumulate=False, want_lp=False, defer=False, want_pair=False):
@@ -581,11 +595,20 @@
     return hit[1], hit[2]
 
 
-def attention_bwd(qkv, bias, out, dout, lse, B, N, H, D, scale, index32=None, n_bins=0, bias_t=None, table=None, cube=None):
+def attention_bwd(qkv, bias, out, dout, lse, B, N, H, D, scale, index32=None, n_bins=0, bias_t=None, table=None, cube=None, binned=False):
     _need_cuda(qkv, bias, out, dout, lse, index32, bias_t, table)
     dqkv = torch.empty_like(qkv)
     delta = torch.empty((B, H, N), dtype=torch.float32, device=qkv.device)
     slab, info = None, None
+    if binned and index32 is not None and table is not None and cube is not None and bias is None and n_bins == (2 * int(cube[0]) - 1) * 225:
+        c = tuple(int(v) for v in cube)
+        rows = _lib.lib().dm_attention_bwd_bin_rows(B, N, H, D, c[0], c[1], c[2], _dt(qkv))
+        if rows > 0:
+            part = torch.empty((rows, n_bins, H), dtype=torch.float32, device=qkv.device)
+            check(_lib.lib().dm_attention_bwd_relpos_binned(qkv.data_ptr(), table.data_ptr(), c[0], c[1], c[2], out.data_ptr(), dout.data_ptr(),
+                                                            lse.data_ptr(), dqkv.data_ptr(), delta.data_ptr(), part.data_ptr(), B, N, H, D,
+                                                            scale, _dt(qkv), _stream()), "dm_attention_bwd_relpos_binned")
+            return dqkv, part, ("bins", rows, n_bins * H)
     if index32 is not None:
         if D != 64 or N > 256:
             raise ValueError(f"the relative-position bias gradient needs head dim 64 and N <= 256 (got D={D}, N={N})")
@@ -602,6 +625,33 @@
                                       delta.data_ptr(), _ptr(slab), B, N, H, D, scale, _dt(qkv), _stream()),
           "dm_attention_bwd")
     return dqkv, slab, info
+
+
+def table_grad_fold(slab, info, dtable, accumulate=False, defer=False):
+    _need_cuda(slab, dtable)
+    deferred = defer and _DEFER_REDUCTIONS and _in_backward()
+    acc = int(bool(accumulate))
+    if info[0] == "bins":
+        _, rows, width = info
+        if deferred:
+            _queue_reduce(slab, dtable, dtable, rows, width, width, accumulate)
+            return dtable
+        item = (_lib.DmReduceItem * 1)()
+        item[0].partial, item[0].out0, item[0].out1 = slab.data_ptr(), dtable.data_ptr(), dtable.data_ptr()
+        item[0].nrows, item[0].width, item[0].split, item[0].accumulate = rows, width, width, acc
+        check(_lib.lib().dm_partial_reduce_batch(item, 1, _stream()), "dm_partial_reduce_batch")
+        return dtable
+    chunks, N, (positions, offsets) = info
+    fields = (slab.data_ptr(), positions.data_ptr(), offsets.data_ptr(), dtable.data_ptr(), int(chunks), int(slab.shape[1]), int(N),
+              int(dtable.shape[0]), acc)
+    if deferred:
+        _queue(_pending_slab, fields, (slab, positions, offsets, dtable), (dtable.data_ptr(),))
+        return dtable
+    item = (_lib.DmRelposItem * 1)()
+    (item[0].slab, item[0].positions, item[0].offsets, item[0].dtable, item[0].chunks, item[0].H, item[0].N, item[0].n_bins,
+     item[0].accumulate) = fields
+    check(_lib.lib().dm_reduce_flush(None, 0, item, 1, _stream()), "dm_reduce_flush")
+    return dtable
 
 
 def relpos_bias_scatter(slab, dtable, B, H, info, n_bins, accumulate=False):
@@ -1546,11 +1596,11 @@
                 tab, cube = P_table.detach().contiguous(), index32._dm_cube
             want_table = bias is not None or tab is not None
             dqkv, slab, rows = attention_bwd(qkv, bias, o, do, lse, B, N, heads, D, scale,
-                                             index32 if want_table else None, n_bins or 0, bias_t=bias_t, table=tab, cube=cube)
+                                             index32 if want_table else None, n_bins or 0, bias_t=bias_t, table=tab, cube=cube, binned=True)
         dtable, k_t = None, False
         if want_table:
             dtable, k_t = _grad_out(P_table, (n_bins, heads), dev)
-            relpos_bias_scatter(slab, dtable, B, heads, rows, n_bins, accumulate=_acc(P_table, k_t))
+            table_grad_fold(slab, rows, dtable, accumulate=_acc(P_table, k_t), defer=k_t)
         dqkv2 = dqkv if isinstance(dqkv, Planes) else dqkv.view(M, 3 * Cc)
         dwq, k_wq = _grad_out(P_qkv_w, (3 * Cc, Cc), dev)
         dbq, k_bq = _grad_out(P_qkv_b, (3 * Cc,), dev)
diff --git a/include/deepmerge_hip.h b/include/deepmerge_hip.h
--- a/include/deepmerge_hip.h
+++ b/include/deepmerge_hip.h
@@ -89,6 +89,11 @@
                                 const float *lse, void *dqkv_pair, float *delta, float *dbias_slab, int32_t B, int32_t N,
                                 int32_t H, int32_t D, float scale, void *stream);
 int32_t dm_attention_bwd_batch_chunks(int32_t B, int32_t N, int32_t H, int32_t dtype);
+int32_t dm_attention_bwd_bin_rows(int32_t B, int32_t N, int32_t H, int32_t D, int32_t cube_s, int32_t cube_h, int32_t cube_w,
+                                  int32_t dtype);
+int dm_attention_bwd_relpos_binned(const void *qkv, const float *table, int32_t cube_s, int32_t cube_h, int32_t cube_w,
+                                   const void *out, const void *dout, const float *lse, void *dqkv, float *delta, float *dtable_part,
+                                   int32_t B, int32_t N, int32_t H, int32_t D, float scale, int32_t dtype, void *stream);
 
 int dm_relpos_bias_gather(const float *table, const int32_t *index, float *bias, float *bias_t,
                           int32_t N, int32_t H, int32_t n_bins, void *stream);
@@ -114,6 +119,13 @@
   int32_t nrows, width, split, accumulate;
 } DmReduceItem;
 int dm_partial_reduce_batch(const DmReduceItem *items, int32_t n, void *stream);
+typedef struct DmRelposItem {
+  const float *slab;
+  const int32_t *positions, *offsets;
+  float *dtable;
+  int32_t chunks, H, N, n_bins, accumulate;
+} DmRelposItem;
+int dm_reduce_flush(const DmReduceItem *items, int32_t n, const DmRelposItem *slabs, int32_t ns, void *stream);
 
 int dm_token_pool_fwd(const float *x, float *y, int32_t B, int32_t S, int32_t side, int32_t C, void *stream);
 int dm_token_pool_bwd(const float *dy, float *dx, int32_t B, int32_t S, int32_t side, int32_t C, void *stream);
```

Result: no change. 6312 pairs/s, median of 6 (+1.0%).
